# joesharratt1229/DT4Image_Restoration

Measured on AMD Instinct MI355X. Metric: pnp_admm_iterations_per_sec, higher is better.
Workload: dtype f32

## Files before the change

### dt4image_restoration_amd/_lib.py

```python
from __future__ import annotations

import ctypes as C
import os

_HERE = os.path.dirname(os.path.abspath(__file__))
LIB_PATH = os.environ.get("PNP_LIB_PATH") or os.path.join(_HERE, "csrc", "libpnpadmm.so")

PNP_FLAG_PROFILE = 1
PNP_FLAG_NO_DENOISER = 2
PNP_FLAG_KEEP_STAGES = 4
PNP_FLAG_BF16_CONVS = 8
PNP_FLAG_PROFILE_LAYERS = 16
PNP_SSIM_CLAMP_X = 1
PNP_RES_COLS = 6
PNP_RES_DELTA = 1
PNP_RES_DC = 2
RESIDUAL_COLUMNS = ("primal", "dx", "dz", "du", "delta", "dc")
PNP_MC_MAX_COILS = 32
PNP_MC_MAX_CG = 64
PNP_CC_MAX_COILS = 64
PNP_PW_MAX_COILS = 64
PNP_ESPIRIT_MAX_COILS = 16
PNP_ESPIRIT_MAX_KSIZE = 8
PNP_ESPIRIT_MAX_N = 512
PNP_GRAPPA_MAX_COILS = 32
PNP_GRAPPA_MAX_ACCEL = 8
PNP_GRAPPA_MAX_SRC = 512
PNP_TV_MAX_ITERS = 64
PNP_PRIOR_UNET = 0
PNP_PRIOR_TV = 1
PRIORS = {"unet": PNP_PRIOR_UNET, "tv": PNP_PRIOR_TV}
PNP_PRIOR_HAAR = 2
PRIOR_NAMES = {PNP_PRIOR_UNET: "unet", PNP_PRIOR_TV: "tv", PNP_PRIOR_HAAR: "haar"}
PNP_HAAR_TI = 0
PNP_HAAR_ORTHO = 1
PNP_HAAR_MAX_LEVELS = 4
HAAR_MODES = {"ti": PNP_HAAR_TI, "ortho": PNP_HAAR_ORTHO}
PNP_SENS_BOX = 0
PNP_SENS_HANN = 1
SENS_WINDOWS = {"box": PNP_SENS_BOX, "hann": PNP_SENS_HANN}
PROFILE_CLASSES = 6
PROFILE_CLASS_NAMES = ("conv3x3_mfma", "conv_first", "conv_last", "fft_rows", "fft_cols_prox", "other")
N_LAYERS = 28


class pnp_config(C.Structure):
    _fields_ = [("n", C.c_int32), ("h", C.c_int32), ("w", C.c_int32), ("device", C.c_int32), ("flags", C.c_int32)]


_vp, _fp, _u8p = C.c_void_p, C.c_void_p, C.c_void_p

SIGNATURES = {
    "pnp_create": (C.c_int, [C.POINTER(pnp_config), C.POINTER(C.c_void_p)]),
    "pnp_destroy": (C.c_int, [C.c_void_p]),
    "pnp_last_error": (C.c_char_p, []),
    "pnp_version": (C.c_char_p, []),
    "pnp_load_unet_weights": (C.c_int, [C.c_void_p, C.c_void_p, C.c_size_t]),
    "pnp_reset": (C.c_int, [C.c_void_p, _fp, _fp, _u8p, C.c_int, _fp, _fp, _fp, _vp]),
    "pnp_set_kspace": (C.c_int, [C.c_void_p, _fp, _u8p, C.c_int, _vp]),
    "pnp_step": (C.c_int, [C.c_void_p, _fp, _fp, _fp, _fp, _fp, _fp, _fp, _u8p, _vp]),
    "pnp_denoise": (C.c_int, [C.c_void_p, _fp, _fp, _fp, _vp]),
    "pnp_tv_denoise": (C.c_int, [C.c_void_p, _fp, _fp, C.c_int, _fp, _vp]),
    "pnp_set_prior": (C.c_int, [C.c_void_p, C.c_int, C.c_double, C.c_int]),
    "pnp_get_prior": (C.c_int, [C.c_void_p, C.POINTER(C.c_int), C.POINTER(C.c_double), C.POINTER(C.c_int)]),
    "pnp_haar_denoise": (C.c_int, [C.c_void_p, _fp, _fp, C.c_int, C.c_int, _fp, _vp]),
    "pnp_set_prior_haar": (C.c_int, [C.c_void_p, C.c_double, C.c_int, C.c_int]),
    "pnp_get_prior_haar": (C.c_int, [C.c_void_p, C.POINTER(C.c_double), C.POINTER(C.c_int), C.POINTER(C.c_int)]),
    "pnp_fft2c": (C.c_int, [C.c_void_p, _fp, _fp, C.c_int, C.c_int, C.c_int, C.c_int, _vp]),
    "pnp_prox_dual": (C.c_int, [C.c_void_p, _fp, _fp, _fp, _fp, _fp, _vp]),
    "pnp_psnr": (C.c_int, [C.c_void_p, _fp, _fp, _fp, _vp]),
    "pnp_ssim": (C.c_int, [C.c_void_p, _fp, _fp, C.c_float, C.c_float, C.c_float, C.c_int, C.c_int, _fp, _fp, _vp]),
    "pnp_residuals": (C.c_int, [C.c_void_p, _fp, _fp, _fp, _vp, C.c_int, _fp, _vp]),
    "pnp_acquire": (C.c_int, [C.c_void_p, _fp, _u8p, C.c_int, C.c_double, C.c_uint64, C.c_int, _fp, _fp, _fp, _vp]),
    "pnp_set_kspace_mc": (C.c_int, [C.c_void_p, _fp, _fp, C.c_int, C.c_int, _u8p, C.c_int, C.c_int, _vp]),
    "pnp_reset_mc": (C.c_int, [C.c_void_p, _fp, _fp, _fp, C.c_int, C.c_int, _u8p, C.c_int, C.c_int, _fp, _fp, _fp, _vp]),
    "pnp_mc_coils": (C.c_int, [C.c_void_p]),
    "pnp_mc_cg_residual": (C.c_int, [C.c_void_p, _fp, _vp]),
    "pnp_mc_normal": (C.c_int, [C.c_void_p, _fp, _fp, _fp, _vp]),
    "pnp_acquire_mc": (C.c_int, [C.c_void_p, _fp, _fp, C.c_int, C.c_int, _u8p, C.c_int, C.c_double, C.c_uint64, C.c_int, _fp, _fp, _fp, _vp]),
    "pnp_nufft_plan": (C.c_int, [C.c_void_p, C.c_void_p, C.c_int64, C.c_int, C.c_int, C.c_int, C.c_int]),
    "pnp_nufft_samples": (C.c_int64, [C.c_void_p]),
    "pnp_nufft_grid": (C.c_int, [C.c_void_p, C.POINTER(C.c_int), C.POINTER(C.c_int)]),
    "pnp_nufft_forward": (C.c_int, [C.c_void_p, _fp, C.c_int, _fp, _vp]),
    "pnp_nufft_adjoint": (C.c_int, [C.c_void_p, _fp, _fp, C.c_int, _fp, _vp]),
    "pnp_set_kspace_nc": (C.c_int, [C.c_void_p, _fp, _fp, C.c_int, _vp]),
    "pnp_reset_nc": (C.c_int, [C.c_void_p, _fp, _fp, _fp, C.c_int, _fp, _fp, _fp, _vp]),
    "pnp_nc_cg_residual": (C.c_int, [C.c_void_p, _fp, _vp]),
    "pnp_nc_normal": (C.c_int, [C.c_void_p, _fp, _fp, _fp, _vp]),
    "pnp_acquire_nc": (C.c_int, [C.c_void_p, _fp, _fp, C.c_double, C.c_uint64, C.c_int, _fp, _fp, _fp, _vp]),
    "pnp_estimate_sens": (C.c_int, [C.c_void_p, _fp, C.c_int, C.c_int, C.c_int, C.c_int, C.c_double, C.c_int, _fp, _fp, _vp]),
    "pnp_coil_compress_matrix": (C.c_int, [C.c_void_p, _fp, C.c_int, C.c_int, C.c_int, C.c_int, _fp, _fp, _fp, _vp]),
    "pnp_coil_compress_apply": (C.c_int, [C.c_void_p, _fp, C.c_int, _fp, C.c_int, C.c_int, _fp, _vp]),
    "pnp_noise_cov": (C.c_int, [C.c_void_p, _fp, C.c_int, C.c_int, C.c_int, C.c_int, _fp, _vp]),
    "pnp_whiten_matrix": (C.c_int, [C.c_void_p, _fp, C.c_int, C.c_int, C.c_int, _fp, _fp, _fp, _vp]),
    "pnp_whiten_apply": (C.c_int, [C.c_void_p, _fp, C.c_int, _fp, C.c_int, _fp, _vp]),
    "pnp_espirit_sens": (C.c_int, [C.c_void_p, _fp, C.c_int, C.c_int, C.c_int, C.c_int, C.c_double, C.c_double, C.c_int, C.c_int, C.c_double,
                                  C.c_int, _fp, _fp, _fp, _vp, _vp]),
    "pnp_grappa_weights": (C.c_int, [C.c_void_p, _fp, C.c_int, C.c_int, C.c_int, C.c_int, C.c_int, C.c_int, C.c_double, C.c_int, _fp, _vp, _fp,
                                    _vp]),
    "pnp_grappa_apply": (C.c_int, [C.c_void_p, _fp, C.c_int, _u8p, C.c_int, C.c_int, C.c_int, C.c_int, C.c_int, _fp, C.c_int, _fp, _vp]),
    "pnp_snapshot_bytes": (C.c_size_t, [C.c_void_p]),
    "pnp_snapshot": (C.c_int, [C.c_void_p, _fp, _fp, _fp, _fp, _vp, _vp]),
    "pnp_restore": (C.c_int, [C.c_void_p, _vp, _fp, _fp, _fp, _fp, _vp]),
    "pnp_unet_read_stage": (C.c_int, [C.c_void_p, C.c_int, _fp, C.POINTER(C.c_int), C.POINTER(C.c_int),
                                      C.POINTER(C.c_int), _vp]),
    "pnp_profile_reset": (C.c_int, [C.c_void_p]),
    "pnp_profile_collect": (C.c_int, [C.c_void_p, C.POINTER(C.c_double), C.POINTER(C.c_int64)]),
    "pnp_profile_layers": (C.c_int, [C.c_void_p, C.POINTER(C.c_double), C.POINTER(C.c_int64)]),
    "pnp_conv_algorithms": (C.c_int, [C.c_void_p, C.POINTER(C.c_int32)]),
    "pnp_conv_schedules": (C.c_int, [C.c_void_p, C.POINTER(C.c_int32)]),
    "pnp_bf16_weight_terms": (C.c_int, [C.c_void_p]),
    "pnp_workspace_bytes": (C.c_size_t, [C.c_void_p]),
}

SIGNATURES_NCSENSE = {
    "pnp_nufft_forward_mc": (C.c_int, [C.c_void_p, _fp, _fp, C.c_int, C.c_int, C.c_int, _fp, _vp]),
    "pnp_nufft_adjoint_mc": (C.c_int, [C.c_void_p, _fp, _fp, _fp, C.c_int, C.c_int, C.c_int, _fp, _vp]),
    "pnp_set_kspace_ncsense": (C.c_int, [C.c_void_p, _fp, _fp, C.c_int, C.c_int, _fp, C.c_int, _vp]),
    "pnp_reset_ncsense": (C.c_int, [C.c_void_p, _fp, _fp, _fp, C.c_int, C.c_int, _fp, C.c_int, _fp, _fp, _fp, _vp]),
    "pnp_ncsense_coils": (C.c_int, [C.c_void_p]),
    "pnp_ncsense_cg_residual": (C.c_int, [C.c_void_p, _fp, _vp]),
    "pnp_ncsense_normal": (C.c_int, [C.c_void_p, _fp, _fp, _fp, _vp]),
    "pnp_acquire_ncsense": (C.c_int, [C.c_void_p, _fp, _fp, C.c_int, C.c_int, _fp, C.c_double, C.c_uint64, C.c_int, _fp, _fp, _fp, _vp]),
}

SIGNATURES_TOEPLITZ = {
    "pnp_toeplitz_plan": (C.c_int, [C.c_void_p, _fp, C.c_int, _vp]),
    "pnp_toeplitz_planned": (C.c_int, [C.c_void_p]),
    "pnp_toeplitz_live": (C.c_int, [C.c_void_p]),
    "pnp_toeplitz_spectrum": (C.c_int, [C.c_void_p, _fp, _vp]),
    "pnp_toeplitz_apply": (C.c_int, [C.c_void_p, _fp, C.c_int, _fp, _vp]),
    "pnp_toeplitz_apply_mc": (C.c_int, [C.c_void_p, _fp, _fp, C.c_int, C.c_int, C.c_int, _fp, _vp]),
    "pnp_set_kspace_nc_tz": (C.c_int, [C.c_void_p, _fp, C.c_int, _vp]),
    "pnp_reset_nc_tz": (C.c_int, [C.c_void_p, _fp, _fp, C.c_int, _fp, _fp, _fp, _vp]),
    "pnp_set_kspace_ncsense_tz": (C.c_int, [C.c_void_p, _fp, _fp, C.c_int, C.c_int, C.c_int, _vp]),
    "pnp_reset_ncsense_tz": (C.c_int, [C.c_void_p, _fp, _fp, _fp, C.c_int, C.c_int, C.c_int, _fp, _fp, _fp, _vp]),
}
PNP_TOEPLITZ_MAX_SIDE = 512

SIGNATURES_DCF = {
    "pnp_nufft_psi": (C.c_int, [C.c_void_p, _fp, _fp, _vp]),
    "pnp_nufft_dcf": (C.c_int, [C.c_void_p, _fp, C.c_int, C.c_int, _fp, _fp, _vp]),
}
PNP_DCF_MAX_ITERS = 256

SIGNATURES_OFFRES = {
    "pnp_offres_plan": (C.c_int, [C.c_void_p, C.c_void_p, C.c_int, C.c_int]),
    "pnp_offres_segments": (C.c_int, [C.c_void_p]),
    "pnp_offres_maps": (C.c_int, [C.c_void_p, _fp, C.c_int, _fp, _vp]),
    "pnp_offres_forward": (C.c_int, [C.c_void_p, _fp, _fp, C.c_int, C.c_int, _fp, _vp]),
    "pnp_offres_adjoint": (C.c_int, [C.c_void_p, _fp, _fp, _fp, C.c_int, C.c_int, _fp, _vp]),
    "pnp_set_kspace_offres": (C.c_int, [C.c_void_p, _fp, _fp, C.c_int, _fp, C.c_int, _vp]),
    "pnp_reset_offres": (C.c_int, [C.c_void_p, _fp, _fp, _fp, C.c_int, _fp, C.c_int, _fp, _fp, _fp, _vp]),
    "pnp_offres_live": (C.c_int, [C.c_void_p]),
    "pnp_offres_cg_residual": (C.c_int, [C.c_void_p, _fp, _vp]),
    "pnp_offres_normal": (C.c_int, [C.c_void_p, _fp, _fp, _fp, _vp]),
    "pnp_acquire_offres": (C.c_int, [C.c_void_p, _fp, _fp, C.c_int, _fp, C.c_double, C.c_uint64, C.c_int, _fp, _fp, _fp, _vp]),
}


def toeplitz_size_error(fn: str, h: int, w: int):
    if h <= PNP_TOEPLITZ_MAX_SIDE and w <= PNP_TOEPLITZ_MAX_SIDE:
        return None
    return f"{fn}: the Toeplitz operator transforms a 2h x 2w grid, so it takes h, w up to {PNP_TOEPLITZ_MAX_SIDE} (got {int(h)}x{int(w)})"

_lib = None


class PnPError(RuntimeError):
    pass


def load() -> C.CDLL:
    global _lib
    if _lib is not None:
        return _lib
    if not os.path.exists(LIB_PATH):
        raise PnPError(f"{LIB_PATH} not found: build it with `python -c 'import __graft_entry__ as g; g.build()'` "
                       f"or `make -C {os.path.dirname(LIB_PATH)}`; there is no CPU fallback")
    lib = C.CDLL(LIB_PATH)
    for name, (res, args) in {**SIGNATURES, **SIGNATURES_NCSENSE, **SIGNATURES_TOEPLITZ, **SIGNATURES_DCF, **SIGNATURES_OFFRES}.items():
        fn = getattr(lib, name)
        fn.restype = res
        fn.argtypes = args
    _lib = lib
    return lib


def check(rc: int, what: str) -> None:
    if rc != 0:
        msg = load().pnp_last_error()
        raise PnPError(f"{what} failed ({rc}): {msg.decode() if msg else '?'}")
```

### dt4image_restoration_amd/csrc/conv_kernels.hip

```cpp
#include "pnp_internal.h"
#include "conv_staging.h"
#include <cstring>
#include <cstdlib>

namespace pnp {



const LayerSpec kLayers[N_LAYERS] = {
    {2, 32, 3, 0, SRC_SIGMA, 0},    {32, 32, 3, 0, SRC_PLAIN, 0},   {32, 32, 3, 0, SRC_PLAIN, 0},
    {32, 64, 3, 1, SRC_POOL, 0},    {64, 64, 3, 1, SRC_PLAIN, 0},   {64, 64, 3, 1, SRC_PLAIN, 0},
    {64, 128, 3, 2, SRC_POOL, 0},   {128, 128, 3, 2, SRC_PLAIN, 0}, {128, 128, 3, 2, SRC_PLAIN, 0},
    {128, 256, 3, 3, SRC_POOL, 0},  {256, 256, 3, 3, SRC_PLAIN, 0}, {256, 256, 3, 3, SRC_PLAIN, 0},
    {256, 512, 3, 4, SRC_POOL, 0},  {512, 512, 3, 4, SRC_PLAIN, 0}, {512, 512, 3, 4, SRC_PLAIN, 0},
    {768, 256, 3, 3, SRC_UPCAT, 256}, {256, 256, 3, 3, SRC_PLAIN, 0}, {256, 256, 3, 3, SRC_PLAIN, 0},
    {384, 128, 3, 2, SRC_UPCAT, 128}, {128, 128, 3, 2, SRC_PLAIN, 0}, {128, 128, 3, 2, SRC_PLAIN, 0},
    {192, 64, 3, 1, SRC_UPCAT, 64},  {64, 64, 3, 1, SRC_PLAIN, 0},   {64, 64, 3, 1, SRC_PLAIN, 0},
    {96, 32, 3, 0, SRC_UPCAT, 32},   {32, 32, 3, 0, SRC_PLAIN, 0},   {32, 32, 3, 0, SRC_PLAIN, 0},
    {32, 1, 1, 0, SRC_PLAIN, 0},
};

ConvPlan conv3x3_plan(int N, int H, int W, int Cin, int Cout, bool bf16, int src_mode, bool allow_ws) {
    ConvPlan p{};
    p.tw = W >= 32 ? 32 : (W >= 16 ? 16 : 8);
// ... 493 lines not shown
                    const float* o = &patch[((2 * qy) * TW + 2 * qx) * OSTR + 4 * c4];
                    const float4 m = f4max(f4max(*reinterpret_cast<const float4*>(o), *reinterpret_cast<const float4*>(o + OSTR)),
                                           f4max(*reinterpret_cast<const float4*>(o + TW * OSTR), *reinterpret_cast<const float4*>(o + TW * OSTR + OSTR)));
                    *reinterpret_cast<float4*>(a.pooled + (((size_t)n * Hp + gy) * Wp + gx) * a.Cout + cbase + 4 * c4) = m;
                }
            }
        }
    } else {
        const size_t plane = (size_t)a.N * a.H * a.W * a.Cout;
        float* const obuf = SPLITK ? a.partial + (size_t)blockIdx.z * plane : a.dst;
        const __amdgpu_buffer_rsrc_t orsrc = __builtin_amdgcn_make_buffer_rsrc((void*)obuf, 0, (int)(plane * sizeof(float)), 0x00020000);
#pragma unroll
        for (int nt = 0; nt < NT; ++nt) {
            const int co = (cbt * (WN * NT) + wn * NT + nt) * 32 + li;
            const unsigned obase = ((unsigned)(((size_t)n * a.H + ty0) * a.W + tx0 + 4 * hh) * (unsigned)a.Cout + (unsigned)co) * 4u;
#pragma unroll
            for (int mt = 0; mt < MT; ++mt)
#pragma unroll
                for (int r = 0; r < 16; ++r) {
                    const int qc = (wm * MT + mt) * 32 + (r & 3) + 8 * (r >> 2);
                    const int gy = ty0 + qc / TW, gx = tx0 + qc % TW + 4 * hh;
                    const int soff = __builtin_amdgcn_readfirstlane(((qc / TW) * a.W + qc % TW) * a.Cout * 4);
                    const float v = SPLITK ? acc[mt][nt][r] : fmaxf(acc[mt][nt][r], kLeaky * acc[mt][nt][r]);
                    if (gy < a.H && gx < a.W) __builtin_amdgcn_raw_buffer_store_b32(__builtin_bit_cast(unsigned, v), orsrc, obase, soff, 0);
                }
        }
    }
}

__global__ __launch_bounds__(256) void splitk_reduce_kernel(const float* __restrict__ partial, const float* __restrict__ bias,
                                                            float* __restrict__ dst, const float* __restrict__ tact,
                                                            size_t plane4, int splitk, int cout4, size_t slice4) {
    for (size_t i = (size_t)blockIdx.x * 256 + threadIdx.x; i < plane4; i += (size_t)gridDim.x * 256) {
        if (tact != nullptr && tact[i / slice4] > 0.5f) continue;
        float4 s = reinterpret_cast<const float4*>(bias)[i % cout4];
        for (int z0 = 0; z0 < splitk; z0 += 8) {
            float4 p[8];
#pragma unroll
            for (int k = 0; k < 8; ++k) p[k] = reinterpret_cast<const float4*>(partial)[(size_t)(z0 + k < splitk ? z0 + k : splitk - 1) * plane4 + i];
#pragma unroll
            for (int k = 0; k < 8; ++k)
                if (z0 + k < splitk) { s.x += p[k].x; s.y += p[k].y; s.z += p[k].z; s.w += p[k].w; }
        }
        s.x = fmaxf(s.x, kLeaky * s.x); s.y = fmaxf(s.y, kLeaky * s.y);
        s.z = fmaxf(s.z, kLeaky * s.z); s.w = fmaxf(s.w, kLeaky * s.w);
        reinterpret_cast<float4*>(dst)[i] = s;
    }
}

template <int TW, int MT, int NT, int WM, int WN, int CK, int SRC, bool SPLITK, int BF16>
static hipError_t launch_inst(const ConvArgs& a, const ConvPlan& p, hipStream_t s) {
    constexpr int WPS = (MT * NT <= 2 && SRC != SRC_UPCAT) ? 3 : (MT * NT <= 8 ? 2 : 1);
    constexpr int WPS16 = (MT * NT <= 2 && BF16 == 2) ? 3 : WPS;
    dim3 grid((unsigned)(p.tiles_x * p.tiles_y * a.N), (unsigned)(a.Cout / p.bn), (unsigned)p.splitk);
    constexpr bool CAN16 = BF16 != 0 && !SPLITK && MT == 2 && NT == 1 && WM == 4 && CK == 32 && SRC != SRC_POOL;
    if constexpr (CAN16) {
        if (a.act16 & 1) {
            hipLaunchKernelGGL((conv3x3_mfma_kernel<TW, MT, NT, WM, WN, CK, SRC, WPS16, SPLITK, BF16, true>), grid, dim3(256), 0, s, a);
            return hipGetLastError();
        }
    }
    if (a.act16 != 0) return hipErrorInvalidValue;
    hipLaunchKernelGGL((conv3x3_mfma_kernel<TW, MT, NT, WM, WN, CK, SRC, WPS, SPLITK, BF16, false>), grid, dim3(256), 0, s, a);
    return hipGetLastError();
}

template <int TW, int MT, int NT, int WM, int WN, int CK, bool SPLITK, int BF16>
static hipError_t launch_cfg(const ConvArgs& a, const ConvPlan& p, int src_mode, hipStream_t s) {
    switch (src_mode) {
        case SRC_PLAIN: return launch_inst<TW, MT, NT, WM, WN, CK, SRC_PLAIN, SPLITK, BF16>(a, p, s);
        case SRC_POOL:  return launch_inst<TW, MT, NT, WM, WN, CK, SRC_POOL, SPLITK, BF16>(a, p, s);
        case SRC_UPCAT: return launch_inst<TW, MT, NT, WM, WN, CK, SRC_UPCAT, SPLITK, BF16>(a, p, s);
        default: return hipErrorInvalidValue;
    }
}

template <int TW, int BF16>
static hipError_t launch_tw(const ConvArgs& a, const ConvPlan& p, int src_mode, hipStream_t s) {
    if constexpr (BF16 == 0) {
        if (p.mt == 1 && p.wn == 4) return launch_cfg<TW, 1, 1, 1, 4, 16, true, 0>(a, p, src_mode, s);
        if (p.mt == 1 && p.wn == 2) return launch_cfg<TW, 1, 1, 2, 2, 16, true, 0>(a, p, src_mode, s);
    }
    if (p.mt == 2 && p.wn == 4) return launch_cfg<TW, 2, 1, 1, 4, 32, true, BF16>(a, p, src_mode, s);
    if (p.mt == 2 && p.wn == 2) return launch_cfg<TW, 2, 1, 2, 2, 32, true, BF16>(a, p, src_mode, s);
    if constexpr (BF16 == 0) {
        if (p.nt == 1 && p.mt == 1) return launch_cfg<TW, 1, 1, 4, 1, 32, false, 0>(a, p, src_mode, s);
    }
    if (p.nt == 1) return launch_cfg<TW, 2, 1, 4, 1, 32, false, BF16>(a, p, src_mode, s);
    if (p.nt == 2 && p.wn == 1) return launch_cfg<TW, 4, 2, 4, 1, 16, false, BF16>(a, p, src_mode, s);
    if (p.nt == 2) return launch_cfg<TW, 4, 2, 2, 2, 32, false, BF16>(a, p, src_mode, s);
    if constexpr (BF16 != 0) return hipErrorInvalidValue;
    else return launch_cfg<TW, 4, 4, 2, 2, 32, false, 0>(a, p, src_mode, s);
}

hipError_t launch_conv3x3(const ConvArgs& a0, const ConvPlan& p, int src_mode, hipStream_t s) {
    if (a0.Cin % 32 != 0 || a0.Cout % 32 != 0 || (a0.Cout > 64 && a0.Cout % 128 != 0)) return hipErrorInvalidValue;
    if (!conv3x3_tensor_fits(a0.N, a0.H, a0.W, a0.Cin, a0.Cout)) return hipErrorInvalidValue;
    if (p.ws) return launch_conv3x3_bf16ws(a0, p, src_mode, s);
    ConvArgs a = a0;
    a.tilesX = p.tiles_x;
    a.tilesY = p.tiles_y;
    const bool split = p.mt <= 2 && p.wn >= 2;
    if (split && a.partial == nullptr) return hipErrorInvalidValue;
    hipError_t e;
    if (a.bf16 == 2) {
        if (p.tw == 32) e = launch_tw<32, 2>(a, p, src_mode, s);
        else if (p.tw == 16) e = launch_tw<16, 2>(a, p, src_mode, s);
        else e = launch_tw<8, 2>(a, p, src_mode, s);
    } else if (a.bf16 == 1) {
        if (p.tw == 32) e = launch_tw<32, 1>(a, p, src_mode, s);
        else if (p.tw == 16) e = launch_tw<16, 1>(a, p, src_mode, s);
        else e = launch_tw<8, 1>(a, p, src_mode, s);
    } else {
        if (p.tw == 32) e = launch_tw<32, 0>(a, p, src_mode, s);
        else if (p.tw == 16) e = launch_tw<16, 0>(a, p, src_mode, s);
        else e = launch_tw<8, 0>(a, p, src_mode, s);
    }
    if (e != hipSuccess || !split) return e;
    const size_t plane4 = (size_t)a.N * a.H * a.W * a.Cout / 4;
    unsigned blocks = (unsigned)((plane4 + 255) / 256);
    if (blocks > 2048u) blocks = 2048u;
    hipLaunchKernelGGL(splitk_reduce_kernel, dim3(blocks), dim3(256), 0, s, a.partial, a.bias, a.dst, a.tact, plane4,
                       p.splitk, a.Cout / 4, (size_t)a.H * a.W * a.Cout / 4);
    return hipGetLastError();
}

bool conv3x3_tensor_fits(int N, int H, int W, int Cin, int Cout) {
    (void)Cin;
    return (size_t)N * H * W * (size_t)Cout * 4 < ((size_t)1 << 31);
}

bool conv3x3_pooled_output_ok(const ConvPlan& p) {
    return p.splitk == 1 && p.mt <= 2 && p.nt == 1 && p.wm == 4;
}

size_t conv3x3_partial_floats(const ConvPlan& p, int N, int H, int W, int Cout) {
    return (p.mt <= 2 && p.wn >= 2) ? (size_t)p.splitk * N * H * W * Cout : 0;
}

Tuning tuning_from_env() {
    Tuning t;
    if (const char* v = getenv("PNP_WINO_MIN_CIN")) t.wino_min_cin = atoi(v);
    if (const char* v = getenv("PNP_WINO_MIN_BLOCKS")) t.wino_min_blocks = atol(v);
    t.wino_big = getenv("PNP_WINO_BIG_GROUPS") != nullptr;
    t.wino_small = getenv("PNP_WINO_SMALL_GROUPS") != nullptr;
    t.no_wino = getenv("PNP_NO_WINOGRAD") != nullptr;
    if (const char* v = getenv("PNP_WINO_F4_MIN_CIN")) t.f4_min_cin = atoi(v);
    t.no_f4 = getenv("PNP_NO_WINO_F4") != nullptr;
    t.no_f4_phased = getenv("PNP_NO_WINO_F4_PHASED") != nullptr;
    t.no_f4_fused_last = getenv("PNP_NO_F4_FUSED_LAST") != nullptr;
    t.no_f4_fused_first = getenv("PNP_NO_F4_FUSED_FIRST") != nullptr;
    if (const char* v = getenv("PNP_WINO_F4_MT16")) t.f4_mt16 = atoi(v);
    if (const char* v = getenv("PNP_WINO_F4_CS")) t.f4_cs = atoi(v);
    if (const char* v = getenv("PNP_WINO_F4_ORDER")) t.f4_order = atoi(v) != 0;
    t.bf16_f32_acts = getenv("PNP_BF16_F32_ACTS") != nullptr;
    t.bf16_no_ws = getenv("PNP_BF16_NO_WS") != nullptr;
    t.bf16_w1 = getenv("PNP_BF16_W1") != nullptr;
    t.bf16_no_holdhi = getenv("PNP_BF16_NO_HOLDHI") != nullptr;
    if (const char* v = getenv("PNP_SLICE128_MIN_N")) t.slice128_min_n = atoi(v);
    if (const char* v = getenv("PNP_TV_NAIVE")) t.tv_naive = atoi(v) != 0;
    if (const char* v = getenv("PNP_HAAR_NAIVE")) t.haar_naive = atoi(v) != 0;
    if (const char* v = getenv("PNP_NCSENSE_COIL_BLOCK")) t.ncsense_block = atoi(v);
    if (const char* v = getenv("PNP_NCSENSE_NAIVE")) t.ncsense_naive = atoi(v) != 0 ? 1 : 0;
    if (const char* v = getenv("PNP_TOEPLITZ_NAIVE")) t.toeplitz_naive = atoi(v) != 0;
    if (const char* v = getenv("PNP_OFFRES_SEG_BLOCK")) t.offres_block = atoi(v);
    if (const char* v = getenv("PNP_OFFRES_GRID_FILTER")) t.offres_grid_filter = atoi(v) != 0;
    if (const char* v = getenv("PNP_OFFRES_NAIVE")) t.offres_naive = atoi(v) != 0 ? 1 : 0;
    return t;
}

hipError_t raise_lds_cap(const void* fn, int bytes, DeviceOnce& once) {
    int dev = 0;
    hipError_t e = hipGetDevice(&dev);
    if (e != hipSuccess) return e;
    const uint64_t bit = 1ull << (dev & 63);
    if (once.mask.load(std::memory_order_relaxed) & bit) return hipSuccess;
    e = hipFuncSetAttribute(fn, hipFuncAttributeMaxDynamicSharedMemorySize, bytes);
    if (e != hipSuccess) return e;
    once.mask.fetch_or(bit, std::memory_order_relaxed);
    return hipSuccess;
}

__global__ __launch_bounds__(256) void conv_first_kernel(const float* __restrict__ ximg, const float2* __restrict__ z,
                                                         const float2* __restrict__ u, const float* __restrict__ sigma,
                                                         const float* __restrict__ tact, const float* __restrict__ w,
                                                         const float* __restrict__ bias, float* __restrict__ dst,
                                                         int N, int H, int W, int tilesX, int tilesY, int TYG, int dst16) {
    constexpr int TH = 8, TW = 32, PW = TW + 2, PH = TH + 2;
    __shared__ float dt[2][PH][PW + 1];
    __shared__ float mt[2][PH][PW + 1];
    const int groupsY = (tilesY + TYG - 1) / TYG;
    int bt = blockIdx.x;
    const int tx0 = (bt % tilesX) * TW;
    bt /= tilesX;
    const int tyg = bt % groupsY;
    const int n = bt / groupsY;
    if (tact != nullptr && tact[n] > 0.5f) return;
    auto stage = [&](int buf, int ty0) {
        for (int i = threadIdx.x; i < PH * PW; i += 256) {
            const int py = i / PW, px = i % PW;
            const int gy = ty0 + py - 1, gx = tx0 + px - 1;
            float d = 0.f, m = 0.f;
            if (gy >= 0 && gy < H && gx >= 0 && gx < W) {
                const size_t q = ((size_t)n * H + gy) * W + gx;
                d = ximg != nullptr ? ximg[q] : (z[q].x - u[q].x);
                m = 1.f;
            }
            dt[buf][py][px] = d;
            mt[buf][py][px] = m;
        }
    };
    const int t_first = tyg * TYG, t_last = min(t_first + TYG, tilesY);
    stage(0, t_first * TH);
    const int cg = threadIdx.x & 7, col = threadIdx.x >> 3;
    float wd[4][9], ws[4][9], br[4], brs[4];
    const float sg = sigma[n];
#pragma unroll
    for (int j = 0; j < 4; ++j) {
        br[j] = bias[cg * 4 + j];
        brs[j] = br[j];
#pragma unroll
        for (int k = 0; k < 9; ++k) {
            wd[j][k] = w[(cg * 4 + j) * 18 + k];
            ws[j][k] = w[(cg * 4 + j) * 18 + 9 + k] * sg;
            brs[j] += ws[j][k];
        }
    }
    const int gx = tx0 + col;
    for (int t = t_first; t < t_last; ++t) {
        const int buf = (t - t_first) & 1, ty0 = t * TH;
        const bool interior = tx0 > 0 && tx0 + TW < W && ty0 > 0 && ty0 + TH < H;
        __syncthreads();
        if (t + 1 < t_last) stage(buf ^ 1, ty0 + TH);
        float d[3][3], m[3][3];
#pragma unroll
        for (int r = 0; r < 2; ++r)
#pragma unroll
            for (int c = 0; c < 3; ++c) { d[r + 1][c] = dt[buf][r][col + c]; m[r + 1][c] = mt[buf][r][col + c]; }
#pragma unroll
        for (int row = 0; row < TH; ++row) {
#pragma unroll
            for (int c = 0; c < 3; ++c) {
                d[0][c] = d[1][c]; d[1][c] = d[2][c]; d[2][c] = dt[buf][row + 2][col + c];
                m[0][c] = m[1][c]; m[1][c] = m[2][c]; m[2][c] = mt[buf][row + 2][col + c];
            }
            float acc[4];
            if (interior) {
#pragma unroll
                for (int j = 0; j < 4; ++j) acc[j] = brs[j];
#pragma unroll
                for (int ky = 0; ky < 3; ++ky)
#pragma unroll
                    for (int kx = 0; kx < 3; ++kx)
#pragma unroll
                        for (int j = 0; j < 4; ++j) acc[j] = fmaf(wd[j][ky * 3 + kx], d[ky][kx], acc[j]);
            } else {
#pragma unroll
                for (int j = 0; j < 4; ++j) acc[j] = br[j];
#pragma unroll
                for (int ky = 0; ky < 3; ++ky)
#pragma unroll
                    for (int kx = 0; kx < 3; ++kx)
#pragma unroll
                        for (int j = 0; j < 4; ++j) {
                            acc[j] = fmaf(wd[j][ky * 3 + kx], d[ky][kx], acc[j]);
                            acc[j] = fmaf(ws[j][ky * 3 + kx], m[ky][kx], acc[j]);
                        }
            }
            const int gy = ty0 + row;
            if (gy < H && gx < W) {
                float4 o;
                o.x = fmaxf(acc[0], kLeaky * acc[0]);
                o.y = fmaxf(acc[1], kLeaky * acc[1]);
                o.z = fmaxf(acc[2], kLeaky * acc[2]);
                o.w = fmaxf(acc[3], kLeaky * acc[3]);
                if (dst16) {
                    uint2 o16;
                    o16.x = __builtin_bit_cast(unsigned, __builtin_convertvector((f32x2){o.x, o.y}, bf16x2));
                    o16.y = __builtin_bit_cast(unsigned, __builtin_convertvector((f32x2){o.z, o.w}, bf16x2));
                    *reinterpret_cast<uint2*>(reinterpret_cast<uint16_t*>(dst) + (((size_t)n * H + gy) * W + gx) * 32 + cg * 4) = o16;
                } else {
                    *reinterpret_cast<float4*>(dst + (((size_t)n * H + gy) * W + gx) * 32 + cg * 4) = o;
                }
            }
        }
    }
}

hipError_t launch_conv_first(const float* ximg, const float2* z, const float2* u, const float* sigma,
                             const float* tact, const float* w, const float* bias, float* dst, int N, int H, int W,
                             hipStream_t s, bool dst_bf16) {
    const int tilesX = (W + 31) / 32, tilesY = (H + 7) / 8;
    int tyg = 8;
    while (tyg > 1 && (long)tilesX * ((tilesY + tyg - 1) / tyg) * N < 512) tyg >>= 1;
    const int groupsY = (tilesY + tyg - 1) / tyg;
    hipLaunchKernelGGL(conv_first_kernel, dim3((unsigned)(tilesX * groupsY * N)), dim3(256), 0, s, ximg, z, u, sigma, tact, w,
                       bias, dst, N, H, W, tilesX, tilesY, tyg, dst_bf16 ? 1 : 0);
    return hipGetLastError();
}

__global__ __launch_bounds__(256) void conv_last_kernel(const float* __restrict__ act, const float* __restrict__ ximg,
                                                        const float2* __restrict__ z, const float2* __restrict__ u,
                                                        const float* __restrict__ tact, const float* __restrict__ w,
                                                        const float* __restrict__ bias, float* __restrict__ out,
                                                        int N, int H, int W) {
    const int cg = threadIdx.x & 7;
// ... 51 lines not shown
```

### dt4image_restoration_amd/csrc/pnp_capi.hip

```cpp
#include "../../include/pnpadmm.h"
#include "../../include/pnpadmm_ncsense.h"
#include "../../include/pnpadmm_toeplitz.h"
#include "../../include/pnpadmm_dcf.h"
#include "../../include/pnpadmm_offres.h"
#include "pnp_internal.h"
#include "denoiser_plan.h"
#include "nufft_plan.h"
#include "offres_plan.h"
#include "block_reduce.h"

#include <cmath>
#include <cstdarg>
#include <cstdio>
#include <cstring>
#include <cstdlib>
#include <initializer_list>
#include <new>
#include <string>
#include <vector>

using namespace pnp;

namespace {

thread_local std::string g_err;

int fail(int code, const char* fmt, ...) {
    char buf[512];
    va_list ap;
    va_start(ap, fmt);
    vsnprintf(buf, sizeof buf, fmt, ap);
    va_end(ap);
    g_err = buf;
    return code;
}

#define HIP_TRY(expr)                                                                              \
    do {                                                                                           \
        hipError_t e_ = (expr);                                                                    \
        if (e_ != hipSuccess) return fail(PNP_ERR_HIP, "%s failed: %s", #expr, hipGetErrorString(e_)); \
    } while (0)

#define PNP_API_BEGIN try {
#define PNP_API_END(name)                                                                          \
    } catch (const std::bad_alloc&) { return fail(PNP_ERR_NOMEM, name ": out of host memory");     \
    } catch (const std::exception& ex_) { return fail(PNP_ERR_INTERNAL, name ": %s", ex_.what());  \
    } catch (...) { return fail(PNP_ERR_INTERNAL, name ": unknown C++ exception"); }

struct DeviceGuard {
    int prev = -1;
    bool switched = false;
    hipError_t err = hipSuccess;
    explicit DeviceGuard(int dev) {
        err = hipGetDevice(&prev);
        if (err == hipSuccess && prev != dev) { err = hipSetDevice(dev); switched = err == hipSuccess; }
    }
    ~DeviceGuard() { if (switched) (void)hipSetDevice(prev); }
};
#define PNP_ON_DEVICE(e)                                                                                  \
    DeviceGuard dev_guard_((e)->cfg.device);                                                              \
    if (dev_guard_.err != hipSuccess) return fail(PNP_ERR_HIP, "hipSetDevice(%d): %s", (e)->cfg.device, hipGetErrorString(dev_guard_.err))

constexpr size_t kNParams = 11773857;

enum ProfClass : int { PROF_CONV3X3 = 0, PROF_CONV_FIRST = 1, PROF_CONV_LAST = 2, PROF_FFT_ROWS = 3, PROF_FFT_COLS = 4, PROF_OTHER = 5 };
static_assert(PROF_OTHER + 1 == PNP_PROFILE_CLASSES, "one enumerator per profile class");

struct EventPair {
    hipEvent_t a, b;
    int cls, layer;
    int count;
};

enum StageKind { STAGE_NONE, STAGE_CART, STAGE_MC, STAGE_NC, STAGE_NS, STAGE_OR };
struct LiveStage {
    StageKind kind = STAGE_NONE;
    bool toeplitz = false;
    int coils = 0;
    int sens_n = 1;
    int cg = 0;
    bool has_w = false;
};

}

struct pnp_engine {
    pnp_config cfg;
    bool weights_loaded = false;
    LiveStage stage;
    float* d_wpack[N_LAYERS] = {};
    float* d_bias[N_LAYERS] = {};
    float* plane[N_LEVELS][N_SLOTS] = {};
    float* d_partial = nullptr;
    Tuning tune;
    DenoiserPlan dplan;
    ConvArgs largs[N_LAYERS] = {};
    FftPlan plan = {};
    float2* d_work = nullptr;
    float2* d_y0s = nullptr;
    uint8_t* d_masks = nullptr;
    double* d_ssim_part = nullptr;
    double* d_res_part = nullptr;
    int mask_n = 1;
    size_t ws_bytes = 0;
    float2* mc_y = nullptr;
    float2* mc_work = nullptr;
    float2* mc_sens = nullptr;
    size_t mc_y_cap = 0, mc_work_cap = 0, mc_sens_cap = 0;
    float2* mc_vec = nullptr;
    double* mc_part = nullptr;
    double* mc_sc = nullptr;
    float* cm_max = nullptr;
    float* cm_rss = nullptr;
    double2* cc_part = nullptr;
    double2* cc_gram = nullptr;
    size_t cc_part_cap = 0, cc_gram_cap = 0;
    double2* pw_part = nullptr;
    size_t pw_part_cap = 0;
    void* es_ws = nullptr;
    size_t es_cap = 0;
    double2* gr_ws = nullptr;
    size_t gr_cap = 0;
    NufftDev nc;
    size_t nc_i0_cap = 0, nc_wts_cap = 0, nc_cy_cap = 0, nc_cx_cap = 0, nc_off_cap = 0, nc_idx_cap = 0, nc_twh_cap = 0, nc_tww_cap = 0;
    float2* nc_grid = nullptr;
    float2* nc_samp = nullptr;
    float2* nc_y = nullptr;
    float* nc_w = nullptr;
    double* nc_mpart = nullptr;
    size_t nc_grid_cap = 0, nc_samp_cap = 0, nc_y_cap = 0, nc_w_cap = 0, nc_mpart_cap = 0;
    int ns_block = kNcsenseBlock;
    int ns_naive = kNcsenseNaiveSteps;
    float2* ns_img = nullptr;
    size_t ns_img_cap = 0;
    float2* ns_grid = nullptr;
    float2* ns_samp = nullptr;
    float2* ns_y = nullptr;
    float2* ns_sens = nullptr;
    float* ns_w = nullptr;
    double* ns_mpart = nullptr;
    size_t ns_grid_cap = 0, ns_samp_cap = 0, ns_y_cap = 0, ns_sens_cap = 0, ns_w_cap = 0, ns_mpart_cap = 0;
    std::vector<int32_t> nc_bin_off_h, nc_bin_idx_h;
    OffresDev orp;
    size_t or_tau_cap = 0, or_seg_cap = 0, or_b0_cap = 0, or_b1_cap = 0, or_loff_cap = 0, or_lidx_cap = 0;
    int or_block = kOffresBlock;
    int or_naive = kOffresNaiveSteps;
    float2* or_maps = nullptr;
    float2* or_y = nullptr;
    float* or_w = nullptr;
    double* or_mpart = nullptr;
    float2* or_amaps = nullptr;
    size_t or_maps_cap = 0, or_y_cap = 0, or_w_cap = 0, or_mpart_cap = 0, or_amaps_cap = 0;
    std::vector<double> nc_traj;
    double* tz_traj = nullptr;
    float* tz_k = nullptr;
    float* tz_w = nullptr;
    float2* tz_tw_h = nullptr;
// ... 2383 lines not shown
                       float* wts, int32_t* info, double* gram, void* stream) {
    PNP_API_BEGIN
    const char* fn = "pnp_grappa_weights";
    if (flags != 0) return fail(PNP_ERR_INVALID, "%s: flags must be 0 (got 0x%x)", fn, (unsigned)flags);
    if (!(lam >= 0.0) || !(lam <= 1.0)) return fail(PNP_ERR_INVALID, "%s: lam must be finite and in [0, 1] (got %g)", fn, lam);
    if (int rc = grappa_check_kernel(fn, coils, accel, by, bx)) return rc;
    const int span = (bx - 1) * accel + 1;
    if (acs_h < by || (acs_h & 1)) return fail(PNP_ERR_INVALID, "%s: acs_h must be even and >= by=%d (got %d)", fn, by, acs_h);
    if (acs_w < span || (acs_w & 1)) return fail(PNP_ERR_INVALID, "%s: acs_w must be even and >= (bx - 1) accel + 1 = %d (got %d)", fn, span, acs_w);
    if (!y0) return fail(PNP_ERR_INVALID, "%s: null y0", fn);
    if (!wts) return fail(PNP_ERR_INVALID, "%s: null wts", fn);
    if (!info) return fail(PNP_ERR_INVALID, "%s: null info", fn);
    {
        const void* q[4] = {y0, wts, info, gram};
        for (int i = 0; i < 4; ++i)
            for (int j = i + 1; j < 4; ++j)
                if (q[j] && q[i] == q[j]) return fail(PNP_ERR_INVALID, "%s: y0, wts, info and gram must not alias", fn);
    }
    if (!e) return fail(PNP_ERR_INVALID, "%s: null handle", fn);
    const int N = e->cfg.n, H = e->cfg.h, W = e->cfg.w;
    if (W % accel) return fail(PNP_ERR_INVALID, "%s: accel must divide w=%d (got %d)", fn, W, accel);
    if (acs_h > H) return fail(PNP_ERR_INVALID, "%s: acs_h must be <= h=%d (got %d)", fn, H, acs_h);
    if (acs_w > W) return fail(PNP_ERR_INVALID, "%s: acs_w must be <= w=%d (got %d)", fn, W, acs_w);
    if ((long long)N * coils > 65535) return fail(PNP_ERR_INVALID, "%s: n * coils must be <= 65535 (got %d * %d)", fn, N, coils);
    const int ns = coils * by * bx, nt = coils * (accel - 1);
    {
        const void* q[4] = {y0, wts, info, gram};
        const size_t len[4] = {(size_t)N * coils * H * W * sizeof(float2), (size_t)N * nt * ns * sizeof(float2), (size_t)N * sizeof(int32_t),
                               (size_t)N * ns * (ns + nt) * sizeof(double2)};
        for (int i = 0; i < 4; ++i)
            for (int j = i + 1; j < 4; ++j)
                if (q[j] && ranges_overlap(q[i], len[i], q[j], len[j])) return fail(PNP_ERR_INVALID, "%s: y0, wts, info and gram must not alias", fn);
    }
    PNP_ON_DEVICE(e);
    hipStream_t s = (hipStream_t)stream;
    if (int rc = gr_ensure(e, (size_t)N * ns * (ns + nt))) return rc;
    Prof p(e, s, PROF_OTHER, -1);
    HIP_TRY(launch_grappa_gram((const float2*)y0, coils, acs_h, acs_w, accel, by, bx, e->gr_ws, (double2*)gram, N, H, W, s));
    HIP_TRY(launch_grappa_solve(e->gr_ws, ns, nt, lam, (float2*)wts, (int*)info, N, s));
    p.end(2);
    return PNP_OK;
    PNP_API_END("pnp_grappa_weights")
}

int pnp_grappa_apply(pnp_handle e, const float* y0, int coils, const uint8_t* mask, int mask_n, int accel, int offset, int by, int bx,
                     const float* wts, int wts_n, float* out, void* stream) {
    PNP_API_BEGIN
    const char* fn = "pnp_grappa_apply";
    if (int rc = grappa_check_kernel(fn, coils, accel, by, bx)) return rc;
    if (offset < 0 || offset >= accel) return fail(PNP_ERR_INVALID, "%s: offset must be 0..accel-1 = %d (got %d)", fn, accel - 1, offset);
    if (mask_n < 1) return fail(PNP_ERR_INVALID, "%s: mask_n must be 1 or the handle's n (got %d)", fn, mask_n);
    if (wts_n < 1) return fail(PNP_ERR_INVALID, "%s: wts_n must be 1 or the handle's n (got %d)", fn, wts_n);
    if (!y0) return fail(PNP_ERR_INVALID, "%s: null y0", fn);
    if (!mask) return fail(PNP_ERR_INVALID, "%s: null mask", fn);
    if (!wts) return fail(PNP_ERR_INVALID, "%s: null wts", fn);
    if (!out) return fail(PNP_ERR_INVALID, "%s: null out", fn);
    if (out == wts || (const void*)out == (const void*)mask || ranges_overlap(out, (size_t)2048 * coils, y0, (size_t)2048 * coils))
        return fail(PNP_ERR_INVALID, "%s: out must not overlap y0, wts or mask", fn);
    if (!e) return fail(PNP_ERR_INVALID, "%s: null handle", fn);
    const int N = e->cfg.n, H = e->cfg.h, W = e->cfg.w;
    if (W % accel) return fail(PNP_ERR_INVALID, "%s: accel must divide w=%d (got %d)", fn, W, accel);
    if (mask_n != 1 && mask_n != N) return fail(PNP_ERR_INVALID, "%s: mask_n must be 1 or the handle's n=%d (got %d)", fn, N, mask_n);
    if (wts_n != 1 && wts_n != N) return fail(PNP_ERR_INVALID, "%s: wts_n must be 1 or the handle's n=%d (got %d)", fn, N, wts_n);
    if ((long long)N * coils > 65535) return fail(PNP_ERR_INVALID, "%s: n * coils must be <= 65535 (got %d * %d)", fn, N, coils);
    const size_t ns = (size_t)coils * by * bx, nt = (size_t)coils * (accel - 1);
    const size_t bytes = (size_t)N * coils * H * W * sizeof(float2), wbytes = (size_t)wts_n * nt * ns * sizeof(float2), mbytes = (size_t)mask_n * H * W;
    if (ranges_overlap(out, bytes, y0, bytes) || ranges_overlap(out, bytes, wts, wbytes) || ranges_overlap(out, bytes, mask, mbytes))
        return fail(PNP_ERR_INVALID, "%s: out must not overlap y0, wts or mask", fn);
    PNP_ON_DEVICE(e);
    hipStream_t s = (hipStream_t)stream;
    Prof p(e, s, PROF_OTHER, -1);
    HIP_TRY(launch_grappa_apply((const float2*)y0, mask, mask_n, (const float2*)wts, wts_n, (float2*)out, coils, accel, offset, by, bx, N, H, W, s));
    return PNP_OK;
    PNP_API_END("pnp_grappa_apply")
}

size_t pnp_snapshot_bytes(pnp_handle e) {
    return e ? SnapLayout(e).bytes() : 0;
}

int pnp_snapshot(pnp_handle e, const float* x, const float* z, const float* u, const float* t_state, void* dst,
                 void* stream) {
    PNP_API_BEGIN
    if (!e || !x || !z || !u || !dst) return fail(PNP_ERR_INVALID, "pnp_snapshot: null argument");
    PNP_ON_DEVICE(e);
    const SnapLayout snap(e);
    char* d = static_cast<char*>(dst);
    hipStream_t s = (hipStream_t)stream;
    HIP_TRY(hipMemcpyAsync(d, x, snap.x_bytes(), hipMemcpyDeviceToDevice, s));
    HIP_TRY(hipMemcpyAsync(d + snap.z_off(), z, snap.zu_bytes(), hipMemcpyDeviceToDevice, s));
    HIP_TRY(hipMemcpyAsync(d + snap.u_off(), u, snap.zu_bytes(), hipMemcpyDeviceToDevice, s));
    if (t_state) HIP_TRY(hipMemcpyAsync(d + snap.t_off(), t_state, snap.t_bytes(), hipMemcpyDeviceToDevice, s));
    else HIP_TRY(hipMemsetAsync(d + snap.t_off(), 0, snap.t_bytes(), s));
    return PNP_OK;
    PNP_API_END("pnp_snapshot")
}

int pnp_restore(pnp_handle e, const void* src, float* x, float* z, float* u, float* t_state, void* stream) {
    PNP_API_BEGIN
    if (!e || !x || !z || !u || !src) return fail(PNP_ERR_INVALID, "pnp_restore: null argument");
    PNP_ON_DEVICE(e);
    const SnapLayout snap(e);
    const char* d = static_cast<const char*>(src);
    hipStream_t s = (hipStream_t)stream;
    HIP_TRY(hipMemcpyAsync(x, d, snap.x_bytes(), hipMemcpyDeviceToDevice, s));
    HIP_TRY(hipMemcpyAsync(z, d + snap.z_off(), snap.zu_bytes(), hipMemcpyDeviceToDevice, s));
    HIP_TRY(hipMemcpyAsync(u, d + snap.u_off(), snap.zu_bytes(), hipMemcpyDeviceToDevice, s));
    if (t_state) HIP_TRY(hipMemcpyAsync(t_state, d + snap.t_off(), snap.t_bytes(), hipMemcpyDeviceToDevice, s));
    return PNP_OK;
    PNP_API_END("pnp_restore")
}

int pnp_unet_read_stage(pnp_handle e, int which, float* dst, int* c, int* hh, int* ww, void* stream) {
    PNP_API_BEGIN
    if (!e || which < 0 || which > 8) return fail(PNP_ERR_INVALID, "pnp_unet_read_stage: which must be 0..8");
    if (e->cfg.flags & PNP_FLAG_NO_DENOISER) return fail(PNP_ERR_STATE, "pnp_unet_read_stage: handle has no denoiser");
    const StagePlan& st = e->dplan.stage[which];
    if (st.fused_away) return fail(PNP_ERR_STATE, "pnp_unet_read_stage: stage 8 is fused away; create the handle with PNP_FLAG_KEEP_STAGES");
    if (st.bf16) return fail(PNP_ERR_STATE, "pnp_unet_read_stage: this stage is held as bf16 on this handle; create it with PNP_FLAG_KEEP_STAGES");
    PNP_ON_DEVICE(e);
    const float* src = e->plane[st.plane.level][st.plane.slot];
    if (c) *c = st.c;
    if (hh) *hh = st.h;
    if (ww) *ww = st.w;
    if (dst) HIP_TRY(launch_nhwc_to_nchw(src, dst, e->cfg.n, st.c, st.h, st.w, (hipStream_t)stream));
    return PNP_OK;
    PNP_API_END("pnp_unet_read_stage")
}

int pnp_conv_algorithms(pnp_handle e, int32_t* algo28) {
    PNP_API_BEGIN
    if (!e || !algo28) return fail(PNP_ERR_INVALID, "pnp_conv_algorithms: null argument");
    if (e->cfg.flags & PNP_FLAG_NO_DENOISER) return fail(PNP_ERR_STATE, "pnp_conv_algorithms: handle has no denoiser");
    for (int i = 0; i < N_LAYERS; ++i) algo28[i] = e->dplan.family[i];
    return PNP_OK;
    PNP_API_END("pnp_conv_algorithms")
}

int pnp_conv_schedules(pnp_handle e, int32_t* sched28) {
    PNP_API_BEGIN
    if (!e || !sched28) return fail(PNP_ERR_INVALID, "pnp_conv_schedules: null argument");
    if (e->cfg.flags & PNP_FLAG_NO_DENOISER) return fail(PNP_ERR_STATE, "pnp_conv_schedules: handle has no denoiser");
    for (int i = 0; i < N_LAYERS; ++i) {
        const int at = e->dplan.launch_of[i];
        sched28[i] = 0;
        if (at < 0 || e->dplan.family[i] != FAM_WINO4) continue;
        const WinoPlan& w = e->dplan.launch[at].wino;
        sched28[i] = w.cs ? 4 : (w.mt == 16 ? 3 : (w.phased ? 2 : 1));
    }
    return PNP_OK;
    PNP_API_END("pnp_conv_schedules")
}

int pnp_profile_reset(pnp_handle e) {
    PNP_API_BEGIN
    if (!e) return fail(PNP_ERR_INVALID, "null handle");
    e->ev_used = 0;
    memset(e->cls_ms, 0, sizeof e->cls_ms); memset(e->cls_n, 0, sizeof e->cls_n);
    memset(e->layer_ms, 0, sizeof e->layer_ms); memset(e->layer_n, 0, sizeof e->layer_n);
    return PNP_OK;
    PNP_API_END("pnp_profile_reset")
}

int pnp_profile_collect(pnp_handle e, double* total_ms, int64_t* launches) {
    PNP_API_BEGIN
    if (!e) return fail(PNP_ERR_INVALID, "null handle");
    PNP_ON_DEVICE(e);
    for (size_t i = 0; i < e->ev_used; ++i) {
        float ms = 0.f;
        HIP_TRY(hipEventElapsedTime(&ms, e->events[i].a, e->events[i].b));
        const EventPair& p = e->events[i];
        e->cls_ms[p.cls] += ms; e->cls_n[p.cls] += p.count;
        if (p.layer >= 0) { e->layer_ms[p.layer] += ms; e->layer_n[p.layer] += 1; }
    }
    e->ev_used = 0;
    for (int i = 0; i < PNP_PROFILE_CLASSES; ++i) {
        if (total_ms) total_ms[i] = e->cls_ms[i];
        if (launches) launches[i] = e->cls_n[i];
    }
    return PNP_OK;
    PNP_API_END("pnp_profile_collect")
}

int pnp_profile_layers(pnp_handle e, double* layer_ms, int64_t* layer_launches) {
    PNP_API_BEGIN
    if (!e) return fail(PNP_ERR_INVALID, "null handle");
    for (int i = 0; i < N_LAYERS; ++i) {
        if (layer_ms) layer_ms[i] = e->layer_ms[i];
        if (layer_launches) layer_launches[i] = e->layer_n[i];
    }
    return PNP_OK;
    PNP_API_END("pnp_profile_layers")
}

}
```

### dt4image_restoration_amd/csrc/pnp_internal.h

```cpp
#pragma once
#include <hip/hip_runtime.h>
#include <stdint.h>
#include <stddef.h>
#include <atomic>
#include <vector>

namespace pnp {

struct Tuning {
    int wino_min_cin = 32;
    long wino_min_blocks = 192;
    bool wino_big = false;
    bool wino_small = false;
    bool no_wino = false;
    int f4_min_cin = 32;
    bool no_f4 = false;
    bool no_f4_fused_first = false;
    bool no_f4_fused_last = false;
    bool no_f4_phased = false;
    int f4_mt16 = 0;
    bool bf16_no_ws = false;
    bool bf16_f32_acts = false;
    bool bf16_no_holdhi = false;
    bool bf16_w1 = false;
    int f4_cs = 1;
    int f4_order = 1;
    int slice128_min_n = 192;
    bool tv_naive = false;
    bool haar_naive = false;
    int ncsense_block = 0;
    int ncsense_naive = -1;
    bool toeplitz_naive = false;
    int offres_block = 0;
    bool offres_grid_filter = false;
    int offres_naive = -1;
};
Tuning tuning_from_env();

struct DeviceOnce { std::atomic<uint64_t> mask{0}; };
hipError_t raise_lds_cap(const void* fn, int bytes, DeviceOnce& once);

enum SrcMode : int { SRC_PLAIN = 0, SRC_SIGMA = 1, SRC_POOL = 2, SRC_UPCAT = 3, SRC_FIRST = 4 };

struct LayerSpec {
    int cin, cout, ksize, level, src, cskip;
};
static constexpr int N_LAYERS = 28;
extern const LayerSpec kLayers[N_LAYERS];

struct ConvArgs {
    const float* src0;
    const float* src1;
    const float* wpack;
    const float* bias;
    float* dst;
    float* pooled;
    const float* last_w; const float* last_b; const float* last_ximg; const float2* last_z; const float2* last_u; float* last_out;
    const float* first_w; const float* first_b; const float* first_sigma;
    float* partial;
    const float* tact;
    int N, H, W;
    int Cin, Cskip, Cout;
    int tilesX, tilesY;
    float rh, rw;
    int bf16;
    int act16;
    int order;
#ifdef PNP_STAMPS
    int stamp_slot;
#endif
#ifdef PNP_DIAG
    int diag;
#endif
};

struct ConvPlan {
    int tw, th;
    int bm, bn;
    int mt, nt, wm, wn;
    int ck;
    int splitk;
    int ws;
    int holdhi = 1;
    int tiles_x, tiles_y;
};
ConvPlan conv3x3_plan(int N, int H, int W, int Cin, int Cout, bool bf16 = false, int src_mode = SRC_PLAIN, bool allow_ws = true);
hipError_t launch_conv3x3_bf16ws(const ConvArgs& a, const ConvPlan& p, int src_mode, hipStream_t s);
size_t conv3x3_partial_floats(const ConvPlan& p, int N, int H, int W, int Cout);
bool conv3x3_pooled_output_ok(const ConvPlan& p);
bool conv3x3_tensor_fits(int N, int H, int W, int Cin, int Cout);
hipError_t launch_conv3x3(const ConvArgs& a, const ConvPlan& p, int src_mode, hipStream_t s);

size_t conv3x3_pack_floats(int cin, int cout);
void pack_conv3x3_weights(const float* oihw, int cin, int cout, int ck, float* dst);
size_t conv3x3_pack_floats_bf16(int cin, int cout, int terms);
void pack_conv3x3_weights_bf16(const float* oihw, int cin, int cout, int ck, int terms, float* dst);

struct WinoPlan {
    bool use;
    int algo;
    int tw, th, bn, wm, wn, ck, tiles_x, tiles_y;
    int stack;
    int mt;
    int phased;
    int cs;
    int order;
};
WinoPlan winograd_plan(int N, int H, int W, int Cin, int Cout, int src_mode, const Tuning& t, int Cskip = 0);
bool upsample_lines_regular(int H);
size_t winograd4_pack_floats(int cin, int cout);
void pack_winograd4_weights(const float* oihw, int cin, int cout, int ck, float* dst);
hipError_t launch_conv3x3_winograd4(const ConvArgs& a, const WinoPlan& p, int src_mode, hipStream_t s);
size_t winograd_pack_floats(int cin, int cout);
void pack_winograd_weights(const float* oihw, int cin, int cout, int ck, float* dst);
hipError_t launch_conv3x3_winograd(const ConvArgs& a, const WinoPlan& p, int src_mode, hipStream_t s);

hipError_t launch_conv_first(const float* ximg, const float2* z, const float2* u, const float* sigma,
                             const float* tact, const float* w, const float* bias, float* dst,
                             int N, int H, int W, hipStream_t s, bool dst_bf16 = false);
hipError_t launch_conv_last(const float* act, const float* ximg, const float2* z, const float2* u,
                            const float* tact, const float* w, const float* bias, float* out,
                            int N, int H, int W, hipStream_t s);
hipError_t launch_nhwc_to_nchw(const float* src, float* dst, int N, int C, int H, int W, hipStream_t s);

struct FftPlan {
    int h, w;
    float2* tw_h;
    float2* tw_w;
};

bool kspace_len_ok(int L);
hipError_t launch_fft_rows(const float2* in, float2* out, const float2* tw, int batch, int H, int W, int inverse, int shift, hipStream_t s);
hipError_t launch_fft_cols(float2* data, const float2* tw, int batch, int H, int W, int inverse, int shift, hipStream_t s);
hipError_t launch_fft_rows_real(const float* x, float2* work, const float2* tw, int N, int H, int W, hipStream_t s);
hipError_t launch_fft_rows_fwd_admm(const float* x, const float2* u, float2* work, const float2* tw, const float* tact, int N, int H, int W,
                                    hipStream_t s);
hipError_t launch_fft_cols_prox(float2* work, const float2* tw, const float2* y0s, const uint8_t* masks, int mask_n, const float* mu,
                                const float* tact, int N, int H, int W, hipStream_t s);
hipError_t launch_fft_rows_inv_admm(const float2* work, const float* x, float2* z, float2* u, const float2* tw, const float* tact, int N,
                                    int H, int W, hipStream_t s);
namespace mixed {
hipError_t launch_fft_rows(const float2* in, float2* out, const float2* tw, int batch, int H, int W, int inverse, int shift, hipStream_t s);
hipError_t launch_fft_cols(float2* data, const float2* tw, int batch, int H, int W, int inverse, int shift, hipStream_t s);
hipError_t launch_fft_rows_real(const float* x, float2* work, const float2* tw, int N, int H, int W, hipStream_t s);
hipError_t launch_fft_rows_fwd_admm(const float* x, const float2* u, float2* work, const float2* tw, const float* tact, int N, int H, int W,
                                    hipStream_t s);
hipError_t launch_fft_cols_prox(float2* work, const float2* tw, const float2* y0s, const uint8_t* masks, int mask_n, const float* mu,
                                const float* tact, int N, int H, int W, hipStream_t s);
hipError_t launch_fft_rows_inv_admm(const float2* work, const float* x, float2* z, float2* u, const float2* tw, const float* tact, int N,
                                    int H, int W, hipStream_t s);
}

hipError_t launch_admm_slice128(const float* x, float2* z, float2* u, const float2* tw, const float2* y0s,
                                const uint8_t* masks, int mask_n, const float* mu, const float* tact, int N, hipStream_t s);

hipError_t launch_reset(const float2* x0, const float2* y0, const uint8_t* mask, int mask_n, float* x, float2* z,
                        float2* u, float2* y0s, uint8_t* masks, int N, int H, int W, hipStream_t s);
hipError_t launch_finish(const float* tact, float* tstate, uint8_t* done, int N, hipStream_t s);
hipError_t launch_psnr(const float* x, const float* gt, float* out, int N, int HW, hipStream_t s);

static constexpr int kSsimMaxRadius = 16;
struct SsimArgs {
    const float* x;
    const float* gt;
    float* map;
    double* partial;
    float* out;
    int H, W;
    int radius;
    int clamp_x;
    float c1, c2;
    float w[2 * kSsimMaxRadius + 1];
};
int ssim_tiles(int H, int W);
hipError_t launch_ssim(const SsimArgs& a, int N, hipStream_t s);

hipError_t launch_residual_tiles(const float* x, const float2* z, const float2* u, const float* xp, const float2* zp, const float2* up,
                                 double* partial, int N, int H, int W, hipStream_t s);
hipError_t launch_misfit_tiles(const float2* fx, const float2* y0s, const uint8_t* masks, int mask_n, double* dcpartial, int N, int H, int W,
                               hipStream_t s);
hipError_t launch_residual_reduce(const double* partial, const double* dcpartial, int has_delta, int has_dc, float* out, int N, int H, int W,
                                  hipStream_t s);

hipError_t launch_acquire_epilogue(float2* work, const uint8_t* mask, int mask_n, float2* y0, double sigma, uint64_t seed, int N, int H, int W,
                                   hipStream_t s, int coils = 1);
hipError_t launch_acquire_clamp(const float2* aty0, float2* x0, int N, int H, int W, hipStream_t s);

hipError_t launch_sense_expand(const float2* src, const float* src_real, const float2* sens, int sens_n, int C, const float* tact, float2* work,
                               int N, int H, int W, hipStream_t s);
hipError_t launch_sense_mask(float2* work, const uint8_t* masks, int mask_n, int C, int N, int H, int W, hipStream_t s);
hipError_t launch_sense_combine(const float2* work, const float2* sens, int sens_n, int C, const float2* pv, const float* mu, const float* tact,
                                float2* q, double* partial, int N, int H, int W, hipStream_t s);
hipError_t launch_sense_cg_init(const float2* aty, const float* x, const float2* u, const float2* q, const float* mu, const float* tact, float2* r,
                                float2* pv, double* partial, int N, int H, int W, hipStream_t s);
hipError_t launch_sense_scalar(const double* partial, int mode, const float* tact, double* sc, int N, int H, int W, hipStream_t s);
hipError_t launch_sense_cg_update(float2* z, float2* r, const float2* pv, const float2* q, const double* sc, const float* tact, double* partial,
                                  int N, int H, int W, hipStream_t s);
hipError_t launch_sense_cg_dir(const float2* r, float2* pv, const double* sc, const float* tact, int N, int H, int W, hipStream_t s);
hipError_t launch_sense_dual(const float* x, const float2* z, float2* u, const float* tact, int N, int H, int W, hipStream_t s);
hipError_t launch_sense_cgres(const double* sc, float* out, int N, hipStream_t s);
hipError_t launch_sense_misfit(const float2* fx, const float2* ys, const uint8_t* masks, int mask_n, int C, double* dcpartial, int N, int H, int W,
                               hipStream_t s);
hipError_t launch_sense_install(const float2* y, const uint8_t* mask, int mask_n, int C, float2* ys, float2* work, uint8_t* masks, int N, int H,
                                int W, hipStream_t s);
hipError_t launch_sense_iterate(const float2* x0, float* x, float2* z, float2* u, int N, int H, int W, hipStream_t s);

hipError_t launch_coilmap_window(const float2* y, float2* sens, int acs_h, int acs_w, int hann, int N, int C, int H, int W, hipStream_t s);
hipError_t launch_coilmap_rss(const float2* l, int C, float* rss, float* partial, int N, int H, int W, hipStream_t s);
hipError_t launch_coilmap_max(const float* partial, float* smax, int N, int H, int W, hipStream_t s);
hipError_t launch_coilmap_normalise(float2* l, int C, const float* rss, const float* smax, float thresh, int N, int H, int W, hipStream_t s);

static constexpr int kGramMinBins = 1024, kGramMaxChunks = 64;
inline int gram_chunk_len(long long count) {
    const long long per = ((count + kGramMaxChunks - 1) / kGramMaxChunks + 31) / 32 * 32;
    return per < kGramMinBins ? kGramMinBins : (int)per;
}
inline int gram_chunks(long long count) { return (int)((count + gram_chunk_len(count) - 1) / gram_chunk_len(count)); }
hipError_t launch_coilcomp_gram(const float2* y, int C, int acs_h, int acs_w, double2* partial, double2* gram, int N, int H, int W, hipStream_t s);
hipError_t launch_coilcomp_eig(const double2* gram, int C, float2* cmat, float* eig, int N, hipStream_t s);
hipError_t launch_coilcomp_apply(const float2* in, const float2* cmat, int cmat_n, int C, int V, float2* out, int N, int H, int W, hipStream_t s);

hipError_t launch_prewhiten_cov(const float2* noise, int noise_n, int C, int S, double2* partial, double2* psi, hipStream_t s);
hipError_t launch_prewhiten_chol(const double2* psi, int psi_n, int C, float2* wmat, float2* lmat, int* info, hipStream_t s);
hipError_t launch_prewhiten_apply(const float2* in, const float2* wmat, int wmat_n, int C, float2* out, int N, int H, int W, hipStream_t s);

hipError_t launch_grappa_gram(const float2* y, int C, int acs_h, int acs_w, int R, int by, int bx, double2* ws, double2* gram, int N, int H, int W,
                              hipStream_t s);
hipError_t launch_grappa_solve(double2* ws, int ns, int nt, double lam, float2* wts, int* info, int N, hipStream_t s);
hipError_t launch_grappa_apply(const float2* y0, const uint8_t* mask, int mask_n, const float2* wts, int wts_n, float2* out, int C, int R,
                               int offset, int by, int bx, int N, int H, int W, hipStream_t s);

inline int espirit_padded(int C, int k) { return (C * k * k + 1) & ~1; }
hipError_t launch_espirit_gram(const float2* y, int C, int acs_h, int acs_w, int k, double2* ws, int N, int H, int W, hipStream_t s);
hipError_t launch_espirit_eig(double2* ws, int C, int k, int N, hipStream_t s);
hipError_t launch_espirit_kern(const double2* ws, int C, int k, double sv_thresh, float2* kern, int* nkept, int N, hipStream_t s);
hipError_t launch_espirit_pixels(float2* sens, const float2* kern, const float* rss, const float* smax, int C, int k, int iters, float crop,
                                 float thresh, float* eval, int N, int H, int W, hipStream_t s);

static constexpr int kTvT = 10, kTvRegion = 128, kTvTile = kTvRegion - 2 * kTvT - 1;
struct TvArgs {
    const float* v;
    const float2* z;
    const float2* u;
    const float* lam;
    float scale;
    const float* tact;
    const float2* p_in;
    float2* p_out;
    float* out;
    int H, W;
    int iters;
    int tiles_x, tiles_y;
};
hipError_t launch_tv_fused(TvArgs a, int N, hipStream_t s);
hipError_t launch_tv_iter(TvArgs a, int N, hipStream_t s);
hipError_t launch_tv_close(TvArgs a, int N, hipStream_t s);

static constexpr int kHaarRegion = 128, kHaarMaxLevels = 4;
inline int haar_tile(int levels) { return kHaarRegion - 2 * ((1 << levels) - 1); }
struct HaarArgs {
// ... 103 lines not shown
```

### dt4image_restoration_amd/csrc/winograd4_kernels.hip

```cpp
#include "pnp_internal.h"
#include "conv_staging.h"
#include <type_traits>

namespace pnp {

#ifdef PNP_STAMPS
#define W4_SLOTS 32
#define W4_WGS 1024
#define W4_N 16
__device__ unsigned long long g_w4_stamps[W4_SLOTS * W4_WGS * W4_N];
static int g_w4_slot = 0;
#define W4T() __builtin_amdgcn_s_memtime()
#endif

namespace {
constexpr double kA = 0.75, kB = 1.5;
constexpr float fA = 0.75f, fB = 1.5f, fA2 = 0.5625f, fB2 = 2.25f, fA3 = 0.421875f, fB3 = 3.375f;
constexpr float fK0 = 1.265625f;
constexpr float fK1 = 2.8125f;

__device__ __forceinline__ float4 f4add(float4 a, float4 b) { return make_float4(a.x + b.x, a.y + b.y, a.z + b.z, a.w + b.w); }
typedef float v2f __attribute__((ext_vector_type(2)));
typedef float f32x4 __attribute__((ext_vector_type(4)));

template <int G>
__device__ __forceinline__ void bt3(const v2f* d, v2f* o) {
    if constexpr (G == 0) {
        o[0] = fK0 * d[0] + (d[4] - fK1 * d[2]);
        const v2f e = d[4] - fB2 * d[2];
        const v2f od = fA * (d[3] - fB2 * d[1]);
        o[1] = e + od;
        o[2] = e - od;
    } else {
        const v2f e = d[4] - fA2 * d[2];
        const v2f od = fB * (d[3] - fA2 * d[1]);
        o[0] = e + od;
        o[1] = e - od;
        o[2] = fK0 * d[1] + (d[5] - fK1 * d[3]);
    }
}

template <int QJ, int PW, int CKP, int PLANE>
__device__ __forceinline__ void wino4_input_transform(const float* w, float* v) {
    constexpr int X0 = QJ == 0 ? 0 : 1;
    v2f c[6][3];
#pragma unroll
    for (int y = 0; y < 6; ++y) {
        v2f d[6];
        __builtin_amdgcn_sched_barrier(0);
#pragma unroll
        for (int x = 0; x < 5; ++x) d[X0 + x] = *reinterpret_cast<const v2f*>(w + (y * PW + X0 + x) * CKP);
        bt3<QJ>(d, c[y]);
    }
#pragma unroll
    for (int j = 0; j < 3; ++j) {
        const v2f r0 = c[0][j], r1 = c[1][j], r2 = c[2][j], r3 = c[3][j], r4 = c[4][j], r5 = c[5][j];
        float* vj = v + (3 * QJ + j) * PLANE;
        *reinterpret_cast<v2f*>(vj + 0 * 6 * PLANE) = fK0 * r0 + (r4 - fK1 * r2);
        const v2f e1 = r4 - fB2 * r2, o1 = fA * (r3 - fB2 * r1);
        *reinterpret_cast<v2f*>(vj + 1 * 6 * PLANE) = e1 + o1;
        *reinterpret_cast<v2f*>(vj + 2 * 6 * PLANE) = e1 - o1;
        const v2f e2 = r4 - fA2 * r2, o2 = fB * (r3 - fA2 * r1);
        *reinterpret_cast<v2f*>(vj + 3 * 6 * PLANE) = e2 + o2;
        *reinterpret_cast<v2f*>(vj + 4 * 6 * PLANE) = e2 - o2;
        *reinterpret_cast<v2f*>(vj + 5 * 6 * PLANE) = fK0 * r1 + (r5 - fK1 * r3);
    }
}
}

constexpr int kW4Tail = 8 * 64 * 4;
size_t winograd4_pack_floats(int cin, int cout) { return (size_t)cout * cin * 36 + (size_t)(cout / 16) * kW4Tail; }

void pack_winograd4_weights(const float* oihw, int cin, int cout, int ck, float* dst) {
    const int CK = ck, S = CK / 4;
    const double pts[5] = {0.0, kA, -kA, kB, -kB};
    double G[6][3];
    for (int j = 0; j < 5; ++j) {
        double nrm = 1.0;
        for (int l = 0; l < 5; ++l) if (l != j) nrm *= pts[j] - pts[l];
        G[j][0] = 1.0 / nrm; G[j][1] = pts[j] / nrm; G[j][2] = pts[j] * pts[j] / nrm;
    }
    G[5][0] = 0.0; G[5][1] = 0.0; G[5][2] = 1.0;
    std::vector<float> U((size_t)cout * cin * 36);
    for (int co = 0; co < cout; ++co)
        for (int ci = 0; ci < cin; ++ci) {
            const float* g = oihw + ((size_t)co * cin + ci) * 9;
            double t[6][3];
            for (int i = 0; i < 6; ++i)
                for (int kx = 0; kx < 3; ++kx) t[i][kx] = G[i][0] * g[kx] + G[i][1] * g[3 + kx] + G[i][2] * g[6 + kx];
            for (int i = 0; i < 6; ++i)
                for (int j = 0; j < 6; ++j)
                    U[((size_t)co * cin + ci) * 36 + 6 * i + j] = (float)(t[i][0] * G[j][0] + t[i][1] * G[j][1] + t[i][2] * G[j][2]);
        }
    size_t o = 0;
    for (int cb = 0; cb < cout / 16; ++cb) {
        for (int ch = 0; ch < cin / CK; ++ch)
            for (int xi = 0; xi < 36; ++xi)
                for (int l = 0; l < 64; ++l)
                    for (int sidx = 0; sidx < S; ++sidx) {
                        const int co = 16 * cb + (l & 15);
                        const int ci = CK * ch + S * (l >> 4) + sidx;
                        dst[o++] = U[((size_t)co * cin + ci) * 36 + xi];
                    }
        for (int i = 0; i < kW4Tail; ++i) dst[o++] = 0.f;
    }
}

bool upsample_lines_regular(int H) {
    if (H < 2 || H % 2) return false;
    const int Hs = H / 2;
    const float rh = (float)(Hs - 1) / (float)(H - 1);
    for (int g = 0; g < H; ++g) {
        const float sc = rh * (float)g;
        const int i0 = (int)sc;
        const int i1 = i0 + (i0 < Hs - 1 ? 1 : 0);
        const float l = sc - (float)i0;
        const int s0 = g >= 1 ? (g - 1) / 2 : -1;
        if (l < 1.f && i0 != s0 && i0 != s0 + 1) return false;
        if (l > 0.f && i1 != s0 && i1 != s0 + 1) return false;
    }
    return true;
}

__device__ __forceinline__ void wino4_decode(int bid, int ny, int ntiles, int order, int& cby, int& bt) {
    if (order == 0) {
        const int grp = bid / (8 * ny), rem = bid % (8 * ny);
        cby = rem >> 3;
        bt = grp * 8 + (rem & 7);
    } else {
        const int xcd = bid & 7, slot = bid >> 3;
        const int tpx = (ntiles + 7) >> 3;
        const int lt = slot / ny;
        cby = slot - lt * ny;
        bt = lt < tpx ? xcd * tpx + lt : ntiles;
    }
}

template <int PH, int PW, int PPP, int NW>
struct Wino4Interp {
    static constexpr int IPAIRS = PW * PPP, IWPG = (IPAIRS + 63) / 64, ING = NW / IWPG;
    static constexpr int IRG = (((PH + (ING > 0 ? ING : 1) - 1) / (ING > 0 ? ING : 1)) + 1) & ~1;
    static constexpr int IK = IRG / 2 + 1;
};
template <int PH, int PW, int PPP, int LH, int LW, int LP, int NW, int ROWSTEP, class Slot, class Put>
__device__ __forceinline__ void wino4_interpolate(const float* lowres, const float* rowT, const float* colT, int w, int t, Slot slot, Put put) {
    typedef Wino4Interp<PH, PW, PPP, NW> G;
    constexpr int IPAIRS = G::IPAIRS, IWPG = G::IWPG, ING = G::ING, IRG = G::IRG, IK = G::IK;
    const int ig = w / IWPG;
    const int it = t - ig * (IWPG * 64);
    if (ig >= ING || it >= IPAIRS) return;
    const int x = it / PPP, part = it % PPP;
    const int yb = ig * IRG;
    const float4 ct = *reinterpret_cast<const float4*>(&colT[4 * x]);
    const float* const l0 = &lowres[__float_as_int(ct.x) + part * 4 + (yb / 2) * (LW * LP)];
    const float* const l1 = &lowres[__float_as_int(ct.y) + part * 4 + (yb / 2) * (LW * LP)];
    const v2f wx0 = v2f{ct.z, ct.z}, wx1 = v2f{ct.w, ct.w};
    v2f tl[IK], th_[IK];
#pragma unroll
    for (int k = 0; k < IK; ++k) {
        if ((yb / 2 + k) < LH) {
            const float4 pa = *reinterpret_cast<const float4*>(l0 + k * (LW * LP)), pb = *reinterpret_cast<const float4*>(l1 + k * (LW * LP));
            tl[k] = __builtin_elementwise_fma(wx0, v2f{pa.x, pa.y}, wx1 * v2f{pb.x, pb.y});
            th_[k] = __builtin_elementwise_fma(wx0, v2f{pa.z, pa.w}, wx1 * v2f{pb.z, pb.w});
        } else { tl[k] = v2f{0.f, 0.f}; th_[k] = v2f{0.f, 0.f}; }
    }
    const int pdst = slot(yb, x, part);
#pragma unroll
    for (int j = 0; j < IRG; ++j) {
        if (yb + j < PH) {
            const float4 rw = *reinterpret_cast<const float4*>(&rowT[4 * (yb + j)]);
            const v2f wa = v2f{rw.x, rw.x}, wb = v2f{rw.y, rw.y};
            const int k = j >> 1;
            const v2f olo = __builtin_elementwise_fma(wa, tl[k], wb * tl[k + 1]);
            const v2f ohi = __builtin_elementwise_fma(wa, th_[k], wb * th_[k + 1]);
            put(pdst + j * ROWSTEP, make_float4(olo.x, olo.y, ohi.x, ohi.y));
        }
    }
}
template <int PH, int PW, int LP>
__device__ __forceinline__ void wino4_upsample_tables(const ConvArgs& a, int tid, int ty0, int tx0, int ylo, int xlo, float* rowT, float* colT) {
    if (tid >= PH + PW) return;
    const int Hs = a.H >> 1, Ws = a.W >> 1;
    const bool isrow = tid < PH;
    const int pq = isrow ? tid : tid - PH;
    const int g = (isrow ? ty0 : tx0) + pq - 1;
    float4 e = make_float4(0.f, 0.f, 0.f, 0.f);
    if (g >= 0 && g < (isrow ? a.H : a.W)) {
        const float sc = (isrow ? a.rh : a.rw) * (float)g;
        const int i0 = (int)sc;
        const int i1 = i0 + (i0 < (isrow ? Hs : Ws) - 1 ? 1 : 0);
        const float l = fminf(fmaxf(sc - (float)i0, 0.f), 1.f);
        if (isrow) {
            const int s0 = ylo + (pq >> 1);
            const float w0 = 1.f - l, w1 = l;
            e.x = (i0 == s0 ? w0 : 0.f) + (i1 == s0 ? w1 : 0.f);
            e.y = (i0 == s0 + 1 ? w0 : 0.f) + (i1 == s0 + 1 ? w1 : 0.f);
        } else {
            e = make_float4(__int_as_float((i0 - xlo) * LP), __int_as_float((i1 - xlo) * LP), 1.f - l, l);
        }
    }
    *reinterpret_cast<float4*>(&(isrow ? rowT : colT)[4 * pq]) = e;
}

template <int CTRL>
__device__ __forceinline__ float dpp_xchg(float v) {
    return __builtin_bit_cast(float, __builtin_amdgcn_update_dpp(0, __builtin_bit_cast(int, v), CTRL, 0xF, 0xF, false));
}
template <int H, int CTRL>
__device__ __forceinline__ void row_reduce_scatter_step(v2f* P, bool bit) {
#pragma unroll
    for (int i = 0; i < H; ++i) {
        const v2f lo = P[i], hi = P[i + H];
        const v2f keep = bit ? hi : lo, send = bit ? lo : hi;
        P[i] = v2f{keep.x + dpp_xchg<CTRL>(send.x), keep.y + dpp_xchg<CTRL>(send.y)};
    }
}

template <int TW, bool STK, int MT = 32, bool FUSE = false>
__device__ __forceinline__ void wino4_epilogue(const ConvArgs& a, const f32x4 (&acc)[36], int n, int th, int tg, int cl, int cb,
                                               int tx0, int ty0, bool live, float* xch = nullptr) {
    constexpr int TC = TW / 4, TR = MT / TC;
    constexpr unsigned OOB = 0x80000000u;
    const int cout0 = cb * 16 + cl;
    const float bias = a.bias[cout0];
    const int Hp = a.H >> 1, Wp = a.W >> 1;
    auto at6 = [&](v2f m0, v2f m1, v2f m2, v2f m3, v2f m4, v2f m5, v2f* t) {
        const v2f s1 = m1 + m2, d1 = m1 - m2, s2 = m3 + m4, d2 = m3 - m4;
        t[0] = m0 + s1 + s2;
        t[1] = fA * d1 + fB * d2;
        t[2] = fA2 * s1 + fB2 * s2;
        t[3] = fA3 * d1 + fB3 * d2 + m5;
    };
    if (!live) return;
    const bool fused = FUSE && a.last_w != nullptr;
#ifdef PNP_DIAG
    const bool nostore = (a.diag & 1) != 0;
#else
    constexpr bool nostore = false;
#endif
    v2f part[2];
    const __amdgpu_buffer_rsrc_t rdst = __builtin_amdgcn_make_buffer_rsrc(
        (void*)(a.dst + (size_t)(n + (STK ? th : 0)) * a.H * a.W * a.Cout), 0, nostore ? 0 : a.H * a.W * a.Cout * 4, 0x00020000);
    const __amdgpu_buffer_rsrc_t rpool = __builtin_amdgcn_make_buffer_rsrc(
        (void*)(a.pooled != nullptr ? a.pooled + (size_t)(n + (STK ? th : 0)) * Hp * Wp * a.Cout : a.dst), 0,
        (a.pooled != nullptr && !nostore) ? Hp * Wp * a.Cout * 4 : 0, 0x00020000);
#pragma unroll
    for (int rp = 0; rp < 2; ++rp) {
        v2f T[4][6];
#pragma unroll
        for (int j = 0; j < 6; ++j) {
            v2f m[6];
#pragma unroll
            for (int i = 0; i < 6; ++i) m[i] = v2f{acc[6 * i + j][2 * rp], acc[6 * i + j][2 * rp + 1]};
            v2f t[4];
            at6(m[0], m[1], m[2], m[3], m[4], m[5], t);
#pragma unroll
            for (int ay = 0; ay < 4; ++ay) T[ay][j] = t[ay];
        }
        v2f Y[4][4];
#pragma unroll
        for (int ay = 0; ay < 4; ++ay) {
            at6(T[ay][0], T[ay][1], T[ay][2], T[ay][3], T[ay][4], T[ay][5], Y[ay]);
#pragma unroll
            for (int ax = 0; ax < 4; ++ax) {
                const v2f sv = Y[ay][ax] + bias;
                Y[ay][ax] = v2f{fmaxf(sv.x, kLeaky * sv.x), fmaxf(sv.y, kLeaky * sv.y)};
            }
        }
        if constexpr (FUSE) {
            if (fused) {
                const float wl = a.last_w[cout0];
                v2f P[16];
#pragma unroll
                for (int i = 0; i < 16; ++i) P[i] = Y[i >> 2][i & 3] * wl;
                row_reduce_scatter_step<8, 0x140>(P, (cl & 8) != 0);
                row_reduce_scatter_step<4, 0x141>(P, (cl & 4) != 0);
                row_reduce_scatter_step<2, 0x1B>(P, (cl & 2) != 0);
                row_reduce_scatter_step<1, 0xB1>(P, (cl & 1) != 0);
                part[rp] = P[0];
                continue;
            }
        }
#pragma unroll
        for (int e = 0; e < 2; ++e) {
            const int t = 16 * th + 4 * tg + 2 * rp + e;
            const int tr = t / TC;
            const int py = STK ? 4 * (tr % (TR / 2)) : 4 * tr, px = 4 * (t % TC);
            const int gy = ty0 + py, gx = tx0 + px;
            const unsigned base = (gx < a.W) ? (unsigned)(((gy * a.W + gx) * a.Cout + cout0) * 4) : OOB;
            const unsigned rowb = (unsigned)(a.W * a.Cout * 4);
#pragma unroll
            for (int ay = 0; ay < 4; ++ay)
#pragma unroll
                for (int ax = 0; ax < 4; ++ax) {
                    const float val = e == 0 ? Y[ay][ax].x : Y[ay][ax].y;
                    __builtin_amdgcn_raw_buffer_store_b32(__builtin_bit_cast(unsigned, val), rdst, base + ay * rowb, ax * a.Cout * 4, 0);
                }
            if (a.pooled != nullptr) {
                const int qy = gy >> 1, qx = gx >> 1;
                const unsigned pbase = (qx < Wp) ? (unsigned)(((qy * Wp + qx) * a.Cout + cout0) * 4) : OOB;
                const unsigned prowb = (unsigned)(Wp * a.Cout * 4);
#pragma unroll
                for (int wy = 0; wy < 2; ++wy)
#pragma unroll
                    for (int wx = 0; wx < 2; ++wx) {
                        const v2f mx = __builtin_elementwise_max(__builtin_elementwise_max(Y[2 * wy][2 * wx], Y[2 * wy][2 * wx + 1]),
                                                                 __builtin_elementwise_max(Y[2 * wy + 1][2 * wx], Y[2 * wy + 1][2 * wx + 1]));
                        const float val = e == 0 ? mx.x : mx.y;
                        __builtin_amdgcn_raw_buffer_store_b32(__builtin_bit_cast(unsigned, val), rpool, pbase + wy * prowb, wx * a.Cout * 4, 0);
                    }
            }
        }
    }
    if constexpr (FUSE) {
        if (fused) {
            const int cq = cb & 1, lane = 16 * tg + cl;
            float4* const x4 = reinterpret_cast<float4*>(xch) + th * 64 + lane;
            if (cq == 1) *x4 = make_float4(part[0].x, part[0].y, part[1].x, part[1].y);
            __syncthreads();
            if (cq == 0) {
                const float4 o = *x4;
                const float sum[4] = {part[0].x + o.x, part[0].y + o.y, part[1].x + o.z, part[1].y + o.w};
                const float lb = a.last_b[0];
#pragma unroll
                for (int r = 0; r < 4; ++r) {
                    const int t = 16 * th + 4 * tg + r;
                    const int gy = ty0 + 4 * (t / TC) + (cl >> 2), gx = tx0 + 4 * (t % TC) + (cl & 3);
                    if (gy < a.H && gx < a.W && !nostore) {
                        const size_t qx = ((size_t)n * a.H + gy) * a.W + gx;
                        const float img = a.last_ximg != nullptr ? a.last_ximg[qx] : (a.last_z[qx].x - a.last_u[qx].x);
                        a.last_out[qx] = fminf(fmaxf(img + sum[r] + lb, 0.f), 1.f);
                    }
                }
            }
        }
    }
}

template <int TW, int SRC, bool STK = false, int WN = 2, int MT = 32>
__global__ __launch_bounds__(8 * MT * WN, 2) void conv3x3_wino4_kernel(const ConvArgs a) {
    constexpr int CK = 8 * WN, CKP = CK, LP = CK, PPP = CK / 4, NT_ = 8 * MT * WN;
    constexpr int CKQ = WN == 2 ? CK + 4 : CK + 2;
    constexpr int HCN = CK / 2;
    constexpr int TC = TW / 4, TR = MT / TC;
    constexpr int TH = 4 * TR;
    constexpr int SUBH = STK ? TH / 2 + 2 : 0;
    constexpr int PH = STK ? 2 * SUBH : TH + 2, PW = TW + 2;
    constexpr int ITEMS = PH * PW * PPP;
    static_assert(!STK || (TW == 16 && SRC == SRC_PLAIN && WN == 2 && MT == 32), "stacked slices: 16-wide tiles, plain source");
    static_assert(MT == 32 || (MT == 16 && WN == 2), "16-tile M-blocks: 64-channel workgroups only");
    constexpr int NIT = (ITEMS + NT_ - 1) / NT_;
    constexpr bool UP2 = SRC == SRC_UPCAT;
    constexpr bool FIRST = SRC == SRC_FIRST;
    constexpr int LH = TH / 2 + 3, LW = TW / 2 + 3;
    constexpr int LITEMS = LH * LW * PPP;
    constexpr int NITL = (LITEMS + NT_ - 1) / NT_;
    constexpr bool SPLIT = UP2 && WN == 2;
    constexpr int NH0 = SPLIT ? (NIT + 1) / 2 : NIT;
    constexpr int NRAW = SPLIT ? (NH0 > NITL ? NH0 : NITL) : ((UP2 && NITL > NIT) ? NITL : NIT);
    constexpr int S = CK / 4;
    constexpr int PF = WN == 2 ? 9 : 12;
    constexpr int KEEP = WN == 1 ? 6 : 3;
    constexpr int PLANE = MT * CKP;
    static_assert(SRC == SRC_PLAIN || SRC == SRC_UPCAT || SRC == SRC_FIRST, "pooled sources go through the pooled copy");
    static_assert(!FIRST || (WN == 1 && MT == 32), "fused first layer: the 32-channel variant");
    static_assert(36 % PF == 0 && MT * HCN * 2 == NT_, "one (tile, 2-channel, column group) transform item per thread");

    extern __shared__ __attribute__((aligned(16))) float smem[];
    float* const patch = smem;
    float* const V = smem + ((PH * PW * CKQ + 3) & ~3);
    float* const lowres = V + 36 * PLANE;
    float* const rowT = lowres + LH * LW * LP;
    float* const colT = rowT + 4 * PH;
    constexpr int IW = PW + 3;
    float* const dimg = V + 36 * PLANE;
    float* const mimg = dimg + (PH + 2) * IW;
    float* const wl = mimg + (PH + 2) * IW;
    float* const bl = wl + 18 * 32;
#ifdef PNP_STAMPS
    unsigned long long st_t0 = W4T(), st_setup = 0, st_loop0 = 0, st_commit = 0, st_trans = 0, st_mfma = 0, st_loop1 = 0, st_ew = 0, st_er = 0, st_tmp = 0;
#endif
    const int tid = threadIdx.x, lane = tid & 63;
    const int wid = __builtin_amdgcn_readfirstlane(tid >> 6);
    const int cq = wid / (MT / 16), th = wid % (MT / 16);
    const int tg = lane >> 4, cl = lane & 15;

    const int ny = a.Cout / (32 * WN);
    const int bid = blockIdx.x;
    const int ntl = a.tilesX * a.tilesY * (STK ? (a.N + 1) / 2 : a.N);
    int cby, bt;
    wino4_decode(bid, ny, ntl, a.order, cby, bt);
    if (bt >= ntl) return;
    const int tx0 = (bt % a.tilesX) * TW;
    bt /= a.tilesX;
    const int ty0 = (bt % a.tilesY) * TH;
    const int n = STK ? 2 * (bt / a.tilesY) : bt / a.tilesY;
    const int nsl = STK ? (n + 1 < a.N ? 2 : 1) : 1;
    const bool live0 = !(a.tact != nullptr && a.tact[n] > 0.5f);
    const bool live1 = STK && nsl == 2 && !(a.tact != nullptr && a.tact[n + 1] > 0.5f);
    if (!live0 && !live1) return;
    const int cb = cby * (2 * WN) + cq;
    const int nchunks = a.Cin / CK;

    const int Hs = a.H >> 1, Ws = a.W >> 1;
    const int ylo = UP2 ? ty0 / 2 - 1 : 0;
    const int xlo = UP2 ? (int)(a.rw * (float)(tx0 > 0 ? tx0 - 1 : 0)) : 0;
    const int nskip = UP2 ? a.Cskip / CK : 0;

    constexpr unsigned OOB = 0x80000000u;
    const int cs = UP2 ? a.Cskip : a.Cin;
#ifdef PNP_DIAG
    const bool hot = (a.diag & 2) != 0;
#else
    constexpr bool hot = false;
#endif
    const int ly0 = hot ? 0 : ty0, lx0 = hot ? 0 : tx0, ln = hot ? 0 : n;
    const __amdgpu_buffer_rsrc_t rsrc0 = __builtin_amdgcn_make_buffer_rsrc(
        (void*)(a.src0 + (size_t)ln * a.H * a.W * cs), 0, nsl * a.H * a.W * cs * 4, 0x00020000);
    unsigned voff[NIT];
#pragma unroll
    for (int k = 0; k < NIT; ++k) {
        const int idx = tid + k * NT_;
        const int part = idx % PPP, pp = idx / PPP;
        const int py = pp / PW, px = pp % PW;
        const int sub = STK ? py / SUBH : 0;
        const int gy = STK ? py % SUBH - 1 : ly0 + py - 1, gx = lx0 + px - 1;
        voff[k] = (idx < ITEMS && sub < nsl && gy >= 0 && gy < a.H && gx >= 0 && gx < a.W)
                      ? (unsigned)((((sub * a.H + gy) * a.W + gx) * cs + part * 4) * 4) : OOB;
    }
    const int Cup = a.Cin - a.Cskip;
    const __amdgpu_buffer_rsrc_t rsrc1 = __builtin_amdgcn_make_buffer_rsrc(
        (void*)(UP2 ? a.src1 + (size_t)ln * Hs * Ws * Cup : a.src0), 0, UP2 ? Hs * Ws * Cup * 4 : 0, 0x00020000);
    unsigned voffL[UP2 ? NITL : 1];
    if constexpr (UP2) {
#pragma unroll
        for (int k = 0; k < NITL; ++k) {
            const int idx = tid + k * NT_;
            const int part = idx % PPP, pp = idx / PPP;
            const int sy = (hot ? -1 : ylo) + pp / LW, sx = (hot ? 0 : xlo) + pp % LW;
            voffL[k] = (idx < LITEMS && sy >= 0 && sy < Hs && sx < Ws) ? (unsigned)(((sy * Ws + sx) * Cup + part * 4) * 4) : OOB;
        }
    }
    const int ldst = ((tid / PPP) * CKQ + (tid % PPP) * 4);
    const int ldstL = ((tid / PPP) * LP + (tid % PPP) * 4);
    auto put_patch = [&](int off, float4 v) {
        if constexpr (CKQ % 4 == 0) *reinterpret_cast<float4*>(&patch[off]) = v;
        else { *reinterpret_cast<float2*>(&patch[off]) = make_float2(v.x, v.y); *reinterpret_cast<float2*>(&patch[off + 2]) = make_float2(v.z, v.w); }
    };

    float4 raw[NRAW];
    auto issue = [&](int c, int half = 0) {
        if (UP2 && c >= nskip) {
            if (half != 0) return;
            const int soff = (c * CK - a.Cskip) * 4;
#pragma unroll
            for (int k = 0; k < NITL; ++k)
                raw[k] = __builtin_bit_cast(float4, __builtin_amdgcn_raw_buffer_load_b128(rsrc1, voffL[k], soff, 0));
            return;
        }
        const int soff = c * CK * 4;
        if (half == 0) {
#pragma unroll
            for (int k = 0; k < NH0; ++k)
                raw[k] = __builtin_bit_cast(float4, __builtin_amdgcn_raw_buffer_load_b128(rsrc0, voff[k], soff, 0));
        } else {
#pragma unroll
            for (int k = NH0; k < NIT; ++k)
                raw[k - NH0] = __builtin_bit_cast(float4, __builtin_amdgcn_raw_buffer_load_b128(rsrc0, voff[k], soff, 0));
        }
    };
    auto park = [&](int c, int half = 0) {
        if (UP2 && c >= nskip) {
            if (half != 0) return;
#pragma unroll
            for (int k = 0; k < NITL; ++k) {
                const int idx = tid + k * NT_;
                if (idx < LITEMS) *reinterpret_cast<float4*>(&lowres[ldstL + k * (NT_ / PPP) * LP]) = raw[k];
            }
            return;
        }
        if (half == 0) {
#pragma unroll
            for (int k = 0; k < NH0; ++k) {
                const int idx = tid + k * NT_;
                if (idx < ITEMS) put_patch(ldst + k * (NT_ / PPP) * CKQ, raw[k]);
            }
        } else {
#pragma unroll
            for (int k = NH0; k < NIT; ++k) {
                const int idx = tid + k * NT_;
                if (idx < ITEMS) put_patch(ldst + k * (NT_ / PPP) * CKQ, raw[k - NH0]);
            }
        }
    };
    typedef Wino4Interp<PH, PW, PPP, NT_ / 64> IG;
    static_assert(!UP2 || (IG::ING >= 1 && (PPP & (PPP - 1)) == 0 && TH % 2 == 0), "row groups of whole waves; even tile origin");
    static_assert(!UP2 || ((PH - 1) / 2 + 1 < LH), "the parked region holds every candidate line");
    auto interpolate = [&]() {
        wino4_interpolate<PH, PW, PPP, LH, LW, LP, NT_ / 64, PW * CKQ>(lowres, rowT, colT, wid, tid,
            [](int y, int x, int part) { return ((y * PW + x) * CKQ) + part * 4; }, [&](int off, float4 v) { put_patch(off, v); });
    };
    bool first_interior = false;
    int fbase[FIRST ? NIT : 1];
    if constexpr (FIRST) {
        first_interior = ty0 >= 2 && ty0 + TH + 2 <= a.H && tx0 >= 2 && tx0 + TW + 2 <= a.W;
        const float sg = a.first_sigma[n];
        for (int i = tid; i < (PH + 2) * (PW + 2); i += NT_) {
            const int r = i / (PW + 2), q = i % (PW + 2);
            const int gy = ty0 - 2 + r, gx = tx0 - 2 + q;
            float d = 0.f, m = 0.f;
            if (gy >= 0 && gy < a.H && gx >= 0 && gx < a.W) {
                const size_t qx = ((size_t)n * a.H + gy) * a.W + gx;
                d = a.last_ximg != nullptr ? a.last_ximg[qx] : (a.last_z[qx].x - a.last_u[qx].x);
                m = 1.f;
            }
            dimg[r * IW + q] = d;
            mimg[r * IW + q] = m;
        }
        for (int i = tid; i < 32 * 18; i += NT_) {
            const int ch = i / 18, t = i % 18;
            wl[t * 32 + ch] = a.first_w[i] * (t >= 9 ? sg : 1.f);
        }
        if (tid < 32) {
            float sc = 0.f;
#pragma unroll
            for (int t = 9; t < 18; ++t) sc += a.first_w[tid * 18 + t] * sg;
            bl[tid] = a.first_b[tid];
            bl[32 + tid] = a.first_b[tid] + sc;
        }
#pragma unroll
        for (int k = 0; k < NIT; ++k) {
            const int pp = (tid + k * NT_) / PPP;
            fbase[k] = (tid + k * NT_ < ITEMS) ? (pp / PW) * IW + pp % PW : 0;
        }
        __syncthreads();
    }
    auto first_patch = [&](int c) {
        if constexpr (FIRST) {
            const int part = tid % PPP;
            const float* const wq = wl + CK * c + 4 * part;
            const f32x4 b4 = *reinterpret_cast<const f32x4*>(bl + (first_interior ? 32 : 0) + CK * c + 4 * part);
            f32x4 acc[NIT];
#pragma unroll
            for (int k = 0; k < NIT; ++k) acc[k] = b4;
#pragma unroll
            for (int t = 0; t < 9; ++t) {
                const f32x4 w4 = *reinterpret_cast<const f32x4*>(wq + t * 32);
#pragma unroll
                for (int k = 0; k < NIT; ++k) acc[k] = __builtin_elementwise_fma(w4, f32x4(dimg[fbase[k] + (t / 3) * IW + t % 3]), acc[k]);
            }
            if (!first_interior) {
#pragma unroll
                for (int t = 0; t < 9; ++t) {
                    const f32x4 w4 = *reinterpret_cast<const f32x4*>(wq + (9 + t) * 32);
#pragma unroll
                    for (int k = 0; k < NIT; ++k) acc[k] = __builtin_elementwise_fma(w4, f32x4(mimg[fbase[k] + (t / 3) * IW + t % 3]), acc[k]);
                }
            }
#pragma unroll
            for (int k = 0; k < NIT; ++k) {
                const int idx = tid + k * NT_;
                if (idx < ITEMS) {
                    const float in = first_interior ? 1.f : mimg[fbase[k] + IW + 1];
                    const f32x4 v = in * __builtin_elementwise_max(acc[k], kLeaky * acc[k]);
                    put_patch((idx / PPP) * CKQ + part * 4, make_float4(v[0], v[1], v[2], v[3]));
                }
            }
        }
    };
    if constexpr (UP2) {
        wino4_upsample_tables<PH, PW, LP>(a, tid, ty0, tx0, ylo, xlo, rowT, colT);
    }
    if constexpr (FIRST) first_patch(0);
    else {
        issue(0); park(0);
        if constexpr (SPLIT) { issue(0, 1); park(0, 1); }
    }

    auto swz = [](int t16, int g) { return WN == 2 ? (g ^ ((4 - (t16 >> 2)) & 3)) : (g ^ ((t16 >> 3) << 1)); };
    const int hc = tid % HCN, tq = (tid / HCN) % MT;
    const int tj = wid / (NT_ / 128);
    const int trow = tq / TC;
    const int wrow = STK ? (trow / (TR / 2)) * SUBH + 4 * (trow % (TR / 2)) : 4 * trow;
    const int win = (wrow * PW + 4 * (tq % TC)) * CKQ + 2 * hc;
    const int vout = WN == 2 ? tq * CKP + 4 * swz(tq & 15, hc >> 1) + 2 * (hc & 1)
                             : tq * CKP + 2 * swz(tq & 15, hc);

    f32x4 acc[36];
#pragma unroll
    for (int k = 0; k < 36; ++k) acc[k] = f32x4{0.f, 0.f, 0.f, 0.f};

    typedef typename std::conditional<WN == 2, float4, float2>::type frag_t;
    const size_t stream = (size_t)nchunks * 36 * 64 + kW4Tail / S;
    const __amdgpu_buffer_rsrc_t rB = __builtin_amdgcn_make_buffer_rsrc(
        (void*)(reinterpret_cast<const frag_t*>(a.wpack) + (size_t)cb * stream), 0, (int)(stream * sizeof(frag_t)), 0x00020000);
    const int boff = lane * (int)sizeof(frag_t);
    const frag_t* const bptr = reinterpret_cast<const frag_t*>(a.wpack) + (size_t)cb * stream + lane;
    auto bfrag = [&](const frag_t* bp, int f0, int i) -> frag_t {
        if constexpr (!UP2) return bp[i * 64];
        else if constexpr (WN == 2) return __builtin_bit_cast(frag_t, __builtin_amdgcn_raw_buffer_load_b128(rB, boff, (f0 + i) * (64 * 16), 0));
        else return __builtin_bit_cast(frag_t, __builtin_amdgcn_raw_buffer_load_b64(rB, boff, (f0 + i) * (64 * 8), 0));
    };
    frag_t bq[PF];
#pragma unroll
    for (int p = 0; p < KEEP; ++p) bq[p] = bfrag(bptr, 0, p);
    const int aoff = (16 * th + cl) * CKP + S * swz(cl, tg);

#ifdef PNP_STAMPS
    st_setup = W4T();
    st_loop0 = st_setup;
#endif
    for (int c = 0; c < nchunks; ++c) {
#ifdef PNP_STAMPS
        st_tmp = W4T();
#endif
        __syncthreads();
        if (UP2 && c >= nskip) {
            if constexpr (NT_ == 256) __builtin_amdgcn_s_setprio(3);
            interpolate();
            if constexpr (NT_ == 256) __builtin_amdgcn_s_setprio(0);
            __syncthreads();
        }
#ifdef PNP_STAMPS
        { const unsigned long long t = W4T(); st_commit += t - st_tmp; st_tmp = t; }
#endif

        if constexpr (WN == 1 && !FIRST) { if (c + 1 < nchunks) issue(c + 1); }
        __builtin_amdgcn_sched_barrier(0);
        if constexpr (NT_ == 256) __builtin_amdgcn_s_setprio(3);
        if (tj == 0) wino4_input_transform<0, PW, CKQ, PLANE>(patch + win, V + vout);
        else wino4_input_transform<1, PW, CKQ, PLANE>(patch + win, V + vout);
        if constexpr (NT_ == 256) __builtin_amdgcn_s_setprio(0);
        __builtin_amdgcn_sched_barrier(0);
        const frag_t* bp = bptr + (size_t)c * 36 * 64;
        const int bf0 = c * 36;
#pragma unroll
        for (int p = KEEP; p < PF; ++p) bq[p] = bfrag(bp, bf0, p);
        if constexpr (WN == 2) { if (c + 1 < nchunks) issue(c + 1); }
        __syncthreads();
#ifdef PNP_STAMPS
        { const unsigned long long t = W4T(); st_trans += t - st_tmp; st_tmp = t; }
#endif

        frag_t ar[3];
        ar[0] = *reinterpret_cast<const frag_t*>(&V[aoff]);
        ar[1] = *reinterpret_cast<const frag_t*>(&V[PLANE + aoff]);
#pragma unroll
        for (int xi = 0; xi < 36; ++xi) {
            if (xi + 2 < 36) ar[(xi + 2) % 3] = *reinterpret_cast<const frag_t*>(&V[(xi + 2) * PLANE + aoff]);
            __builtin_amdgcn_sched_barrier(0);
            const frag_t a0 = ar[xi % 3], b0 = bq[xi % PF];
            acc[xi] = __builtin_amdgcn_mfma_f32_16x16x4f32(a0.x, b0.x, acc[xi], 0, 0, 0);
            acc[xi] = __builtin_amdgcn_mfma_f32_16x16x4f32(a0.y, b0.y, acc[xi], 0, 0, 0);
            if constexpr (WN == 2) {
                acc[xi] = __builtin_amdgcn_mfma_f32_16x16x4f32(a0.z, b0.z, acc[xi], 0, 0, 0);
                acc[xi] = __builtin_amdgcn_mfma_f32_16x16x4f32(a0.w, b0.w, acc[xi], 0, 0, 0);
            }
            __builtin_amdgcn_sched_barrier(0);
            if constexpr (SPLIT) {
                if (xi == 17 && c + 1 < nchunks) { park(c + 1, 0); issue(c + 1, 1); }
            }
#ifdef PNP_DIAG
            if ((a.diag & 4) && (xi & 1)) continue;
#endif
            if (xi + PF < 36 + KEEP) bq[xi % PF] = bfrag(bp, bf0, xi + PF);
        }
#ifdef PNP_STAMPS
        { const unsigned long long t = W4T(); st_mfma += t - st_tmp; }
#endif
        if (c + 1 < nchunks) {
            if constexpr (FIRST) first_patch(c + 1);
            else park(c + 1, SPLIT ? 1 : 0);
        }
    }
#ifdef PNP_STAMPS
    st_loop1 = W4T();
    st_tmp = st_loop1;
#endif

    wino4_epilogue<TW, STK, MT, WN == 1 && MT == 32 && SRC == SRC_PLAIN>(a, acc, n, th, tg, cl, cb, tx0, ty0, STK ? (th == 0 ? live0 : live1) : true, smem);
#ifdef PNP_STAMPS
    {
        const int w = (int)blockIdx.x - (int)(gridDim.x / 2);
        if (tid == 0 && w >= 0 && w < W4_WGS && a.stamp_slot < W4_SLOTS) {
            unsigned long long* o = g_w4_stamps + ((size_t)a.stamp_slot * W4_WGS + w) * W4_N;
            const unsigned long long te = W4T();
            o[0] = 1; o[1] = st_setup - st_t0; o[2] = st_commit; o[3] = st_trans; o[4] = st_mfma; o[5] = st_loop1 - st_loop0;
            o[6] = te - st_tmp; o[7] = 0; o[8] = te - st_loop1; o[9] = te - st_t0; o[10] = (unsigned long long)nchunks;
        }
    }
#endif
}

template <int TW, bool STK>
__global__ __launch_bounds__(512, 2) void conv3x3_wino4p_kernel(const ConvArgs a) {
    constexpr int CK = 16, CKP = 16, PPP = 4, NT_ = 512, S = 4;
    constexpr int TC = TW / 4, TR = 32 / TC;
    constexpr int TH = 4 * TR;
    constexpr int SUBH = STK ? TH / 2 + 2 : 0;
    constexpr int PH = STK ? 2 * SUBH : TH + 2, PW = TW + 2;
    constexpr int NPIX = PH * PW, ITEMS = NPIX * PPP;
    constexpr int NIT = (ITEMS + NT_ - 1) / NT_;
    constexpr int PLSZ = ((NPIX * 4 + 15) / 16) * 16 + 4;
    constexpr int PATCH = 4 * PLSZ;
    constexpr int PF = 12, KEEP = 3;
    constexpr int PLANE = 32 * CKP;
    constexpr unsigned OOB = 0x80000000u;
    static_assert(!STK || TW == 16, "stacked slices: 16-wide tiles");
    static_assert((2 * PATCH + 36 * PLANE) * 4 <= 160 * 1024, "two patch copies + V in one CU's LDS");

    extern __shared__ __attribute__((aligned(16))) float smem[];
    float* const patch = smem;
    float* const V = smem + 2 * PATCH;
#ifdef PNP_STAMPS
    unsigned long long st_t0 = W4T(), st_setup = 0, st_loop0 = 0, st_commit = 0, st_trans = 0, st_mfma = 0, st_loop1 = 0, st_tmp = 0;
#endif
    const int tid = threadIdx.x, lane = tid & 63;
    const int wid = __builtin_amdgcn_readfirstlane(tid >> 6);
    const int grp = wid >> 2, cq = wid & 3;
    const int th = grp;
    const int tg = lane >> 4, cl = lane & 15;

    const int ny = a.Cout / 64;
    const int bid = blockIdx.x;
    const int ntl = a.tilesX * a.tilesY * (STK ? (a.N + 1) / 2 : a.N);
    int cby, bt;
    wino4_decode(bid, ny, ntl, a.order, cby, bt);
    if (bt >= ntl) return;
    const int tx0 = (bt % a.tilesX) * TW;
    bt /= a.tilesX;
    const int ty0 = (bt % a.tilesY) * TH;
    const int n = STK ? 2 * (bt / a.tilesY) : bt / a.tilesY;
    const int nsl = STK ? (n + 1 < a.N ? 2 : 1) : 1;
    const bool live0 = !(a.tact != nullptr && a.tact[n] > 0.5f);
    const bool live1 = STK && nsl == 2 && !(a.tact != nullptr && a.tact[n + 1] > 0.5f);
    if (!live0 && !live1) return;
    const int cb = cby * 4 + cq;
    const int nchunks = a.Cin / CK;

    const __amdgpu_buffer_rsrc_t rsrc0 = __builtin_amdgcn_make_buffer_rsrc(
        (void*)(a.src0 + (size_t)n * a.H * a.W * a.Cin), 0, nsl * a.H * a.W * a.Cin * 4, 0x00020000);
    unsigned voff[NIT];
#pragma unroll
    for (int k = 0; k < NIT; ++k) {
        const int idx = tid + k * NT_;
        const int part = idx % PPP, pp = idx / PPP;
        const int py = pp / PW, px = pp % PW;
        const int sub = STK ? py / SUBH : 0;
        const int gy = STK ? py % SUBH - 1 : ty0 + py - 1, gx = tx0 + px - 1;
        voff[k] = (idx < ITEMS && sub < nsl && gy >= 0 && gy < a.H && gx >= 0 && gx < a.W)
                      ? (unsigned)((((sub * a.H + gy) * a.W + gx) * a.Cin + part * 4) * 4) : OOB;
    }
    const int ldst = (tid & 3) * PLSZ + (tid >> 2) * 4;
    float4 raw[NIT];
    auto issue = [&](int c) {
        const int soff = c * CK * 4;
#pragma unroll
        for (int k = 0; k < NIT; ++k)
            raw[k] = __builtin_bit_cast(float4, __builtin_amdgcn_raw_buffer_load_b128(rsrc0, voff[k], soff, 0));
    };
    auto park = [&](int c) {
        float* const dst = patch + (c & 1) * PATCH + ldst;
#pragma unroll
        for (int k = 0; k < NIT; ++k)
            if (tid + k * NT_ < ITEMS) *reinterpret_cast<float4*>(&dst[k * (NT_ / PPP) * 4]) = raw[k];
    };

    auto swz = [](int t16, int g) { return g ^ ((4 - (t16 >> 2)) & 3); };
    const int tgi = tid & 255;
    const int hc = tgi & 7, t16 = (tgi >> 3) & 15;
    const int tj = (wid >> 1) & 1;
    const int tq = 16 * grp + t16;
    const int trow = tq / TC;
    const int wrow = STK ? (trow / (TR / 2)) * SUBH + 4 * (trow % (TR / 2)) : 4 * trow;
    const int win = (hc >> 1) * PLSZ + (wrow * PW + 4 * (tq % TC)) * 4 + 2 * (hc & 1);
    const int vout = tq * CKP + 4 * swz(t16, hc >> 1) + 2 * (hc & 1);

    f32x4 acc[36];
#pragma unroll
    for (int k = 0; k < 36; ++k) acc[k] = f32x4{0.f, 0.f, 0.f, 0.f};

    const size_t stream = (size_t)nchunks * 36 * 64 + kW4Tail / S;
    const float4* const bptr = reinterpret_cast<const float4*>(a.wpack) + (size_t)cb * stream + lane;
    float4 bq[PF];
#pragma unroll
    for (int p = 0; p < KEEP; ++p) bq[p] = bptr[p * 64];
    const int aoff = (16 * th + cl) * CKP + 4 * swz(cl, tg);

    constexpr bool PARK_T = !STK;
    issue(0);
    park(0);
    if constexpr (!PARK_T) { if (grp == 1 && nchunks > 1) { issue(1); park(1); } }
#ifdef PNP_STAMPS
    st_setup = W4T();
    st_loop0 = st_setup;
#endif
    if (grp == 1) __syncthreads();
    for (int c = 0; c < nchunks; ++c) {
#ifdef PNP_STAMPS
        st_tmp = W4T();
#endif
        __syncthreads();
#ifdef PNP_STAMPS
        { const unsigned long long t = W4T(); st_commit += t - st_tmp; st_tmp = t; }
#endif
        if constexpr (PARK_T) { if (c + 1 < nchunks) issue(c + 1); }
        __builtin_amdgcn_s_setprio(3);
        {
            const float* const w = patch + (c & 1) * PATCH + win;
            if (tj == 0) wino4_input_transform<0, PW, 4, PLANE>(w, V + vout);
            else wino4_input_transform<1, PW, 4, PLANE>(w, V + vout);
        }
        __builtin_amdgcn_s_setprio(0);
        __builtin_amdgcn_sched_barrier(0);
        const float4* bp = bptr + (size_t)c * 36 * 64;
#pragma unroll
        for (int p = KEEP; p < PF; ++p) bq[p] = bp[p * 64];
        const int nx = c + 1 + grp;
        if constexpr (PARK_T) { if (c + 1 < nchunks) park(c + 1); }
        else { if (nx < nchunks) issue(nx); }
        __syncthreads();
#ifdef PNP_STAMPS
        { const unsigned long long t = W4T(); st_trans += t - st_tmp; st_tmp = t; }
#endif

        float4 ar[3];
        ar[0] = *reinterpret_cast<const float4*>(&V[aoff]);
        ar[1] = *reinterpret_cast<const float4*>(&V[PLANE + aoff]);
#pragma unroll
        for (int xi = 0; xi < 36; ++xi) {
            if (xi + 2 < 36) ar[(xi + 2) % 3] = *reinterpret_cast<const float4*>(&V[(xi + 2) * PLANE + aoff]);
            __builtin_amdgcn_sched_barrier(0);
            const float4 a0 = ar[xi % 3], b0 = bq[xi % PF];
            acc[xi] = __builtin_amdgcn_mfma_f32_16x16x4f32(a0.x, b0.x, acc[xi], 0, 0, 0);
            acc[xi] = __builtin_amdgcn_mfma_f32_16x16x4f32(a0.y, b0.y, acc[xi], 0, 0, 0);
            acc[xi] = __builtin_amdgcn_mfma_f32_16x16x4f32(a0.z, b0.z, acc[xi], 0, 0, 0);
            acc[xi] = __builtin_amdgcn_mfma_f32_16x16x4f32(a0.w, b0.w, acc[xi], 0, 0, 0);
            __builtin_amdgcn_sched_barrier(0);
#ifdef PNP_DIAG
            if ((a.diag & 4) && (xi & 1)) continue;
#endif
            if (xi + PF < 36 + KEEP) bq[xi % PF] = bp[(xi + PF) * 64];
        }
#ifdef PNP_STAMPS
        { const unsigned long long t = W4T(); st_mfma += t - st_tmp; }
#endif
        if constexpr (!PARK_T) { if (nx < nchunks) park(nx); }
    }
    if (grp == 0) __syncthreads();
#ifdef PNP_STAMPS
    st_loop1 = W4T();
    st_tmp = st_loop1;
#endif

    wino4_epilogue<TW, STK>(a, acc, n, th, tg, cl, cb, tx0, ty0, STK ? (th == 0 ? live0 : live1) : true);
#ifdef PNP_STAMPS
    {
        const int w = (int)blockIdx.x - (int)(gridDim.x / 2);
        if (tid == 0 && w >= 0 && w < W4_WGS && a.stamp_slot < W4_SLOTS) {
            unsigned long long* o = g_w4_stamps + ((size_t)a.stamp_slot * W4_WGS + w) * W4_N;
            const unsigned long long te = W4T();
            o[0] = 1; o[1] = st_setup - st_t0; o[2] = st_commit; o[3] = st_trans; o[4] = st_mfma; o[5] = st_loop1 - st_loop0;
            o[6] = te - st_tmp; o[7] = 0; o[8] = te - st_loop1; o[9] = te - st_t0; o[10] = (unsigned long long)nchunks;
        }
    }
#endif
}

template <int TW, int SRC>
__global__ __launch_bounds__(512, 2) void conv3x3_wino4c_kernel(const ConvArgs a) {
    constexpr int CK = 16, CKP = 16, PPP = 4, NT_ = 512, S = 4, MT = 16;
    constexpr bool UP2 = SRC == SRC_UPCAT;
    static_assert(SRC == SRC_PLAIN || SRC == SRC_UPCAT, "plain or upsample + concat source");
    constexpr int TC = TW / 4, TR = MT / TC;
    constexpr int TH = 4 * TR;
    constexpr int PH = TH + 2, PW = TW + 2;
    constexpr int NPIX = PH * PW, ITEMS = NPIX * PPP;
    constexpr int NIT = (ITEMS + NT_ - 1) / NT_;
    constexpr int PLSZ = ((NPIX * 4 + 15) / 16) * 16 + 4;
    constexpr int PATCH = 4 * PLSZ;
    constexpr int PF = 12, KEEP = 3;
    constexpr int PLANE = MT * CKP;
    constexpr int VSZ = 36 * PLANE;
    constexpr unsigned OOB = 0x80000000u;
    static_assert(NIT == 3 && ITEMS <= NIT * NT_, "three staging items per thread");
    constexpr int LP = CK;
    constexpr int LH = TH / 2 + 3, LW = TW / 2 + 3;
    constexpr int LITEMS = LH * LW * PPP, NITL = (LITEMS + NT_ - 1) / NT_;
    constexpr int LOWRES = LH * LW * LP;
    static_assert((2 * PATCH + 2 * VSZ + (UP2 ? 2 * LOWRES + 4 * (PH + PW) : 0)) * 4 <= 160 * 1024, "everything in one CU's LDS");

    extern __shared__ __attribute__((aligned(16))) float smem[];
    float* const patch = smem;
    float* const V = smem + 2 * PATCH;
    float* const lowres = V + 2 * VSZ;
    float* const rowT = lowres + 2 * LOWRES;
    float* const colT = rowT + 4 * PH;
#ifdef PNP_STAMPS
    unsigned long long st_t0 = W4T(), st_setup = 0, st_loop0 = 0, st_commit = 0, st_trans = 0, st_mfma = 0, st_loop1 = 0, st_tmp = 0;
#endif
    const int tid = threadIdx.x, lane = tid & 63;
    const int wid = __builtin_amdgcn_readfirstlane(tid >> 6);
    const int half = wid >> 2;
    const int tg = lane >> 4, cl = lane & 15;

    const int ny = a.Cout / 128;
    const int bid = blockIdx.x;
    const int ntl = a.tilesX * a.tilesY * a.N;
    int cby, bt;
    wino4_decode(bid, ny, ntl, a.order, cby, bt);
    if (bt >= ntl) return;
    const int tx0 = (bt % a.tilesX) * TW;
    bt /= a.tilesX;
    const int ty0 = (bt % a.tilesY) * TH;
    const int n = bt / a.tilesY;
    if (a.tact != nullptr && a.tact[n] > 0.5f) return;
    const int cb = cby * 8 + wid;
    const int nchunks = a.Cin / CK;
    const int cs = UP2 ? a.Cskip : a.Cin;
    const int nskip = UP2 ? a.Cskip / CK : nchunks;
    const int Hs = a.H >> 1, Ws = a.W >> 1;
    const int ylo = UP2 ? ty0 / 2 - 1 : 0;
    const int xlo = UP2 ? (int)(a.rw * (float)(tx0 > 0 ? tx0 - 1 : 0)) : 0;

    const __amdgpu_buffer_rsrc_t rsrc0 = __builtin_amdgcn_make_buffer_rsrc(
        (void*)(a.src0 + (size_t)n * a.H * a.W * cs), 0, a.H * a.W * cs * 4, 0x00020000);
    unsigned voff[NIT];
#pragma unroll
    for (int k = 0; k < NIT; ++k) {
        const int idx = tid + k * NT_;
        const int part = idx % PPP, pp = idx / PPP;
        const int gy = ty0 + pp / PW - 1, gx = tx0 + pp % PW - 1;
        voff[k] = (idx < ITEMS && gy >= 0 && gy < a.H && gx >= 0 && gx < a.W) ? (unsigned)(((gy * a.W + gx) * cs + part * 4) * 4) : OOB;
    }
    const int ldst = (tid & 3) * PLSZ + (tid >> 2) * 4;
    float4 raw[NIT];
    const int Cup = a.Cin - a.Cskip;
    const __amdgpu_buffer_rsrc_t rsrc1 = __builtin_amdgcn_make_buffer_rsrc(
        (void*)(UP2 ? a.src1 + (size_t)n * Hs * Ws * Cup : a.src0), 0, UP2 ? Hs * Ws * Cup * 4 : 0, 0x00020000);
    unsigned voffL[UP2 ? NITL : 1];
    float4 rawL[UP2 ? NITL : 1];
    if constexpr (UP2) {
#pragma unroll
        for (int k = 0; k < NITL; ++k) {
            const int idx = tid + k * NT_;
            const int part = idx % PPP, pp = idx / PPP;
            const int sy = ylo + pp / LW, sx = xlo + pp % LW;
            voffL[k] = (idx < LITEMS && sy >= 0 && sy < Hs && sx < Ws) ? (unsigned)(((sy * Ws + sx) * Cup + part * 4) * 4) : OOB;
        }
    }
    const int ldstL = (tid >> 2) * LP + (tid & 3) * 4;
    auto issueL = [&](int c) {
        if constexpr (UP2) {
            const int soff = (c * CK - a.Cskip) * 4;
#pragma unroll
            for (int k = 0; k < NITL; ++k)
                rawL[k] = __builtin_bit_cast(float4, __builtin_amdgcn_raw_buffer_load_b128(rsrc1, voffL[k], soff, 0));
        }
    };
    auto parkL = [&](int c) {
        if constexpr (UP2) {
            float* const dst = lowres + (c & 1) * LOWRES + ldstL;
#pragma unroll
            for (int k = 0; k < NITL; ++k)
                if (tid + k * NT_ < LITEMS) *reinterpret_cast<float4*>(&dst[k * (NT_ / PPP) * LP]) = rawL[k];
        }
    };
    static_assert(Wino4Interp<PH, PW, PPP, 4>::ING >= 1 && TH % 2 == 0 && (PH - 1) / 2 + 1 < LH, "row groups of whole waves; even tile origin; every candidate line parked");
    auto interpolate = [&](int c) {
        if constexpr (UP2) {
            float* const pdst = patch + (c & 1) * PATCH;
            wino4_interpolate<PH, PW, PPP, LH, LW, LP, 4, PW * 4>(lowres + (c & 1) * LOWRES, rowT, colT, wid & 3, tid & 255,
                [](int y, int x, int part) { return part * PLSZ + (y * PW + x) * 4; }, [&](int off, float4 v) { *reinterpret_cast<float4*>(&pdst[off]) = v; });
        }
    };
    if constexpr (UP2) {
        wino4_upsample_tables<PH, PW, LP>(a, tid, ty0, tx0, ylo, xlo, rowT, colT);
    }
    auto issue = [&](int c) {
        const int soff = c * CK * 4;
#pragma unroll
        for (int k = 0; k < NIT; ++k)
            raw[k] = __builtin_bit_cast(float4, __builtin_amdgcn_raw_buffer_load_b128(rsrc0, voff[k], soff, 0));
    };
    auto park = [&](int c) {
        float* const dst = patch + (c & 1) * PATCH + ldst;
#pragma unroll
        for (int k = 0; k < NIT; ++k)
            if (tid + k * NT_ < ITEMS) *reinterpret_cast<float4*>(&dst[k * (NT_ / PPP) * 4]) = raw[k];
    };

    auto swz = [](int t16, int g) { return g ^ ((4 - (t16 >> 2)) & 3); };
    const int tgi = tid & 255;
    const int hc = tgi & 7, t16 = (tgi >> 3) & 15;
    const int tj = (wid >> 1) & 1;
    const int win = (hc >> 1) * PLSZ + (4 * (t16 / TC) * PW + 4 * (t16 % TC)) * 4 + 2 * (hc & 1);
    const int vout = t16 * CKP + 4 * swz(t16, hc >> 1) + 2 * (hc & 1);
    auto transform = [&](int c) {
        const float* const w = patch + (c & 1) * PATCH + win;
        float* const v = V + (c & 1) * VSZ + vout;
        if (tj == 0) wino4_input_transform<0, PW, 4, PLANE>(w, v);
        else wino4_input_transform<1, PW, 4, PLANE>(w, v);
    };

    f32x4 acc[36];
#pragma unroll
    for (int k = 0; k < 36; ++k) acc[k] = f32x4{0.f, 0.f, 0.f, 0.f};

    const size_t stream = (size_t)nchunks * 36 * 64 + kW4Tail / S;
    const __amdgpu_buffer_rsrc_t rB = __builtin_amdgcn_make_buffer_rsrc(
        (void*)(reinterpret_cast<const float4*>(a.wpack) + (size_t)cb * stream), 0, (int)(stream * sizeof(float4)), 0x00020000);
    const int boff = lane * (int)sizeof(float4);
    const float4* const bptr = reinterpret_cast<const float4*>(a.wpack) + (size_t)cb * stream + lane;
    auto bfrag = [&](const float4* bp, int f0, int i) -> float4 {
        if constexpr (!UP2) return bp[i * 64];
        else return __builtin_bit_cast(float4, __builtin_amdgcn_raw_buffer_load_b128(rB, boff, (f0 + i) * (64 * 16), 0));
    };
    float4 bq[PF];
#pragma unroll
    for (int p = 0; p < KEEP; ++p) bq[p] = bfrag(bptr, 0, p);
    const int aoff = cl * CKP + 4 * swz(cl, tg);

    issue(0);
    park(0);
    if (nchunks > 1) issue(1);
    __syncthreads();
    if (half == 1) transform(0);
    if (nchunks > 1) park(1);
#ifdef PNP_STAMPS
    st_setup = W4T();
    st_loop0 = st_setup;
#endif
    for (int c = 0; c < nchunks; ++c) {
#ifdef PNP_STAMPS
        st_tmp = W4T();
#endif
        __syncthreads();
#ifdef PNP_STAMPS
        { const unsigned long long t = W4T(); st_commit += t - st_tmp; st_tmp = t; }
#endif
        if (half == (c & 1)) {
            if (c + 1 < nchunks) {
                __builtin_amdgcn_s_setprio(3);
                transform(c + 1);
                __builtin_amdgcn_s_setprio(0);
            }
        } else if (UP2 && c + 2 >= nskip && c + 2 < nchunks) {
            __builtin_amdgcn_s_setprio(3);
            interpolate(c + 2);
            __builtin_amdgcn_s_setprio(0);
        }
        __builtin_amdgcn_sched_barrier(0);
        const float4* bp = bptr + (size_t)c * 36 * 64;
        const int bf0 = c * 36;
#pragma unroll
        for (int p = KEEP; p < PF; ++p) bq[p] = bfrag(bp, bf0, p);
        if (c + 2 < nskip) issue(c + 2);
        if (UP2 && c + 3 >= nskip && c + 3 < nchunks) issueL(c + 3);
#ifdef PNP_STAMPS
        { const unsigned long long t = W4T(); st_trans += t - st_tmp; st_tmp = t; }
#endif

        const float* const Vc = V + (c & 1) * VSZ + aoff;
        float4 ar[3];
        ar[0] = *reinterpret_cast<const float4*>(&Vc[0]);
        ar[1] = *reinterpret_cast<const float4*>(&Vc[PLANE]);
#pragma unroll
        for (int xi = 0; xi < 36; ++xi) {
            if (xi + 2 < 36) ar[(xi + 2) % 3] = *reinterpret_cast<const float4*>(&Vc[(xi + 2) * PLANE]);
            __builtin_amdgcn_sched_barrier(0);
            const float4 a0 = ar[xi % 3], b0 = bq[xi % PF];
            acc[xi] = __builtin_amdgcn_mfma_f32_16x16x4f32(a0.x, b0.x, acc[xi], 0, 0, 0);
            acc[xi] = __builtin_amdgcn_mfma_f32_16x16x4f32(a0.y, b0.y, acc[xi], 0, 0, 0);
            acc[xi] = __builtin_amdgcn_mfma_f32_16x16x4f32(a0.z, b0.z, acc[xi], 0, 0, 0);
            acc[xi] = __builtin_amdgcn_mfma_f32_16x16x4f32(a0.w, b0.w, acc[xi], 0, 0, 0);
            __builtin_amdgcn_sched_barrier(0);
            if (xi + PF < 36 + KEEP) bq[xi % PF] = bfrag(bp, bf0, xi + PF);
        }
#ifdef PNP_STAMPS
        { const unsigned long long t = W4T(); st_mfma += t - st_tmp; }
#endif
        if (c + 2 < nskip) park(c + 2);
        if (UP2 && c + 3 >= nskip && c + 3 < nchunks) parkL(c + 3);
    }
#ifdef PNP_STAMPS
    st_loop1 = W4T();
    st_tmp = st_loop1;
#endif

    wino4_epilogue<TW, false, 16>(a, acc, n, 0, tg, cl, cb, tx0, ty0, true);
#ifdef PNP_STAMPS
    {
        const int w = (int)blockIdx.x - (int)(gridDim.x / 2);
        if (tid == 0 && w >= 0 && w < W4_WGS && a.stamp_slot < W4_SLOTS) {
            unsigned long long* o = g_w4_stamps + ((size_t)a.stamp_slot * W4_WGS + w) * W4_N;
            const unsigned long long te = W4T();
            o[0] = 1; o[1] = st_setup - st_t0; o[2] = st_commit; o[3] = st_trans; o[4] = st_mfma; o[5] = st_loop1 - st_loop0;
            o[6] = te - st_tmp; o[7] = 0; o[8] = te - st_loop1; o[9] = te - st_t0; o[10] = (unsigned long long)nchunks;
        }
    }
#endif
}

template <int TW, int SRC>
static hipError_t launch_wino4c_inst(const ConvArgs& a, const WinoPlan& p, hipStream_t s) {
    constexpr int TC = TW / 4, TR = 16 / TC, TH = 4 * TR;
    constexpr int NPIX = (TH + 2) * (TW + 2);
    constexpr int PLSZ = ((NPIX * 4 + 15) / 16) * 16 + 4;
    constexpr size_t lowres_f = SRC == SRC_UPCAT ? (size_t)2 * (TH / 2 + 3) * (TW / 2 + 3) * 16 + 4 * (TH + 2 + TW + 2) : 0;
    constexpr size_t lds = ((size_t)2 * 4 * PLSZ + (size_t)2 * 36 * 16 * 16 + lowres_f) * sizeof(float);
    if (p.th != TH || p.tw != TW) return hipErrorInvalidValue;
    if (SRC == SRC_UPCAT && a.Cskip < 3 * 16) return hipErrorInvalidValue;
    auto kern = conv3x3_wino4c_kernel<TW, SRC>;
    static DeviceOnce cap;
    if (hipError_t e = raise_lds_cap((const void*)kern, (int)lds, cap); e != hipSuccess) return e;
    const int ntiles = p.tiles_x * p.tiles_y * a.N, ny = a.Cout / 128;
    dim3 grid((unsigned)(((ntiles + 7) / 8) * 8 * ny));
    hipLaunchKernelGGL(kern, grid, dim3(512), lds, s, a);
    return hipGetLastError();
}

template <int TW, bool STK>
static hipError_t launch_wino4p_inst(const ConvArgs& a, const WinoPlan& p, hipStream_t s) {
    constexpr int TC = TW / 4, TR = 32 / TC, TH = 4 * TR;
    constexpr int NPIX = (STK ? TH + 4 : TH + 2) * (TW + 2);
    constexpr int PLSZ = ((NPIX * 4 + 15) / 16) * 16 + 4;
    constexpr size_t lds = ((size_t)2 * 4 * PLSZ + (size_t)36 * 32 * 16) * sizeof(float);
    auto kern = conv3x3_wino4p_kernel<TW, STK>;
    static DeviceOnce cap;
    if (hipError_t e = raise_lds_cap((const void*)kern, (int)lds, cap); e != hipSuccess) return e;
    const int ntiles = p.tiles_x * p.tiles_y * (STK ? (a.N + 1) / 2 : a.N), ny = a.Cout / 64;
    dim3 grid((unsigned)(((ntiles + 7) / 8) * 8 * ny));
    hipLaunchKernelGGL(kern, grid, dim3(512), lds, s, a);
    return hipGetLastError();
}

template <int TW, int SRC, bool STK = false, int WN = 2, int MT = 32>
static hipError_t launch_wino4_inst(const ConvArgs& a, const WinoPlan& p, hipStream_t s) {
    constexpr int CK = 8 * WN, CKP = CK, CKQ = WN == 2 ? CK + 4 : CK + 2, TC = TW / 4, TR = MT / TC, TH = 4 * TR;
    constexpr size_t patch_f = (((size_t)(STK ? TH + 4 : TH + 2) * (TW + 2) * CKQ + 3) / 4) * 4;
    constexpr size_t lowres_f = SRC == SRC_UPCAT ? (size_t)(TH / 2 + 3) * (TW / 2 + 3) * CK + 4 * (TH + 2 + TW + 2) : 0;
    constexpr size_t first_f = SRC == SRC_FIRST ? (size_t)2 * (TH + 4) * (TW + 5) + 18 * 32 + 64 : 0;
    constexpr size_t lds = (patch_f + (size_t)36 * MT * CKP + lowres_f + first_f) * sizeof(float);
    static_assert(lds <= (WN == 2 && MT == 32 ? 160 : 80) * 1024, "one (8 waves) / two (4 waves) workgroups per CU");
    if (p.th != TH || p.tw != TW) return hipErrorInvalidValue;
    auto kern = conv3x3_wino4_kernel<TW, SRC, STK, WN, MT>;
    static DeviceOnce cap;
    if (hipError_t e = raise_lds_cap((const void*)kern, (int)lds, cap); e != hipSuccess) return e;
    const int ntiles = p.tiles_x * p.tiles_y * (STK ? (a.N + 1) / 2 : a.N), ny = a.Cout / (32 * WN);
    dim3 grid((unsigned)(((ntiles + 7) / 8) * 8 * ny));
    hipLaunchKernelGGL(kern, grid, dim3(8 * MT * WN), lds, s, a);
    return hipGetLastError();
}

hipError_t launch_conv3x3_winograd4(const ConvArgs& a0, const WinoPlan& p, int src_mode, hipStream_t s) {
    if (!p.use || p.algo != 4 || a0.Cout % p.bn || a0.Cin % p.ck || (src_mode == SRC_UPCAT && a0.Cskip % p.ck) || a0.W % 4) return hipErrorInvalidValue;
    if (a0.last_w != nullptr && !(p.bn == 32 && p.mt == 32 && src_mode == SRC_PLAIN)) return hipErrorInvalidValue;
    ConvArgs a = a0;
    a.tilesX = p.tiles_x;
    a.tilesY = p.tiles_y;
    a.order = p.order;
#ifdef PNP_STAMPS
    a.stamp_slot = g_w4_slot++;
#endif
    if (p.bn == 32) {
        if (p.ck != 8 || p.stack) return hipErrorInvalidValue;
        if (p.tw == 32 && src_mode == SRC_PLAIN) return launch_wino4_inst<32, SRC_PLAIN, false, 1>(a, p, s);
        if (p.tw == 32 && src_mode == SRC_UPCAT) return launch_wino4_inst<32, SRC_UPCAT, false, 1>(a, p, s);
        if (p.tw == 32 && src_mode == SRC_FIRST) return launch_wino4_inst<32, SRC_FIRST, false, 1>(a, p, s);
        if (p.tw == 16 && src_mode == SRC_FIRST) return launch_wino4_inst<16, SRC_FIRST, false, 1>(a, p, s);
        if (p.tw == 16 && src_mode == SRC_PLAIN) return launch_wino4_inst<16, SRC_PLAIN, false, 1>(a, p, s);
        if (p.tw == 16 && src_mode == SRC_UPCAT) return launch_wino4_inst<16, SRC_UPCAT, false, 1>(a, p, s);
        return hipErrorInvalidValue;
    }
    if (p.ck != 16) return hipErrorInvalidValue;
    if (p.cs) {
        if (p.bn != 128 || p.mt != 16 || p.stack) return hipErrorInvalidValue;
        if (p.tw == 32 && src_mode == SRC_PLAIN) return launch_wino4c_inst<32, SRC_PLAIN>(a, p, s);
        if (p.tw == 32 && src_mode == SRC_UPCAT) return launch_wino4c_inst<32, SRC_UPCAT>(a, p, s);
        if (p.tw == 16 && src_mode == SRC_PLAIN) return launch_wino4c_inst<16, SRC_PLAIN>(a, p, s);
        if (p.tw == 16 && src_mode == SRC_UPCAT) return launch_wino4c_inst<16, SRC_UPCAT>(a, p, s);
        return hipErrorInvalidValue;
    }
    if (p.mt == 16) {
        if (p.stack) return hipErrorInvalidValue;
        if (p.tw == 32 && src_mode == SRC_PLAIN) return launch_wino4_inst<32, SRC_PLAIN, false, 2, 16>(a, p, s);
        if (p.tw == 32 && src_mode == SRC_UPCAT) return launch_wino4_inst<32, SRC_UPCAT, false, 2, 16>(a, p, s);
        if (p.tw == 16 && src_mode == SRC_PLAIN) return launch_wino4_inst<16, SRC_PLAIN, false, 2, 16>(a, p, s);
        if (p.tw == 16 && src_mode == SRC_UPCAT) return launch_wino4_inst<16, SRC_UPCAT, false, 2, 16>(a, p, s);
        return hipErrorInvalidValue;
    }
    if (p.phased && src_mode == SRC_PLAIN) {
        if (p.tw == 32 && !p.stack) return launch_wino4p_inst<32, false>(a, p, s);
        if (p.tw == 16) {
            if (p.stack) return a.H == 16 && a.W == 16 ? launch_wino4p_inst<16, true>(a, p, s) : hipErrorInvalidValue;
            return launch_wino4p_inst<16, false>(a, p, s);
        }
        return hipErrorInvalidValue;
    }
    if (p.tw == 32) {
        if (src_mode == SRC_PLAIN) return launch_wino4_inst<32, SRC_PLAIN>(a, p, s);
        if (src_mode == SRC_UPCAT) return launch_wino4_inst<32, SRC_UPCAT>(a, p, s);
    } else if (p.tw == 16) {
        if (p.stack) return src_mode == SRC_PLAIN && a.H == 16 && a.W == 16 ? launch_wino4_inst<16, SRC_PLAIN, true>(a, p, s) : hipErrorInvalidValue;
        if (src_mode == SRC_PLAIN) return launch_wino4_inst<16, SRC_PLAIN>(a, p, s);
        if (src_mode == SRC_UPCAT) return launch_wino4_inst<16, SRC_UPCAT>(a, p, s);
    }
    return hipErrorInvalidValue;
}

}

#ifdef PNP_STAMPS
extern "C" int pnp_debug_stamps4_reset(void) { pnp::g_w4_slot = 0; return 0; }
extern "C" int pnp_debug_stamps4_read(unsigned long long* dst, int slots) {
    return (int)hipMemcpyFromSymbol(dst, HIP_SYMBOL(pnp::g_w4_stamps), (size_t)slots * W4_WGS * W4_N * sizeof(unsigned long long));
}
#endif
```

### dt4image_restoration_amd/csrc/winograd_kernels.hip

```cpp
#include "pnp_internal.h"
#include "conv_staging.h"
#include <cstdlib>

namespace pnp {

#ifdef PNP_STAMPS
#define PNP_STAMP_SLOTS 32
#define PNP_STAMP_WGS 1024
#define PNP_STAMP_N 112
__device__ unsigned long long g_wino_stamps[PNP_STAMP_SLOTS * PNP_STAMP_WGS * PNP_STAMP_N];
static int g_stamp_slot = 0;
#define STAMP() do { if (ns < PNP_STAMP_N) st[ns] = __builtin_amdgcn_s_memtime(); ++ns; } while (0)
#else
#define STAMP() do { } while (0)
#endif

size_t winograd_pack_floats(int cin, int cout) { return (size_t)(cout / 32) * ((size_t)(cin / 8) * 16 * 256 + 2 * 4 * 256); }

void pack_winograd_weights(const float* oihw, int cin, int cout, int ck, float* dst) {
    static const double G[4][3] = {{1, 0, 0}, {0.5, 0.5, 0.5}, {0.5, -0.5, 0.5}, {0, 0, 1}};
    std::vector<float> U((size_t)cout * cin * 16);
    for (int co = 0; co < cout; ++co)
        for (int ci = 0; ci < cin; ++ci) {
            const float* g = oihw + ((size_t)co * cin + ci) * 9;
            double t[4][3];
            for (int i = 0; i < 4; ++i)
                for (int kx = 0; kx < 3; ++kx) t[i][kx] = G[i][0] * g[kx] + G[i][1] * g[3 + kx] + G[i][2] * g[6 + kx];
            for (int i = 0; i < 4; ++i)
                for (int j = 0; j < 4; ++j)
                    U[((size_t)co * cin + ci) * 16 + 4 * i + j] = (float)(t[i][0] * G[j][0] + t[i][1] * G[j][1] + t[i][2] * G[j][2]);
        }
    size_t o = 0;
    for (int cb = 0; cb < cout / 32; ++cb)
        for (int half = 0; half < 2; ++half) {
            for (int ch = 0; ch < cin / ck; ++ch)
                for (int ks = 0; ks < ck / 8; ++ks)
                    for (int k = 0; k < 8; ++k)
                        for (int l = 0; l < 64; ++l)
                            for (int j = 0; j < 4; ++j) {
                                const int co = 32 * cb + (l & 31);
                                const int ci = ck * ch + 8 * ks + 4 * (l >> 5) + j;
                                dst[o++] = U[((size_t)co * cin + ci) * 16 + 8 * half + k];
                            }
            for (int i = 0; i < 4 * 256; ++i) dst[o++] = 0.f;
        }
}


WinoPlan winograd_plan(int N, int H, int W, int Cin, int Cout, int src_mode, const Tuning& t, int Cskip) {
    constexpr long kCsMinBlocks = 256;
    WinoPlan p{};
    p.use = false;
    p.algo = 1;
    if (t.no_wino || Cin < t.wino_min_cin || Cin % 32 || Cout % 32) return p;
    if (!t.no_f4 && Cin >= t.f4_min_cin && (Cout % 64 == 0 || Cout == 32) && Cin % 16 == 0 && (src_mode == SRC_PLAIN || src_mode == SRC_UPCAT) &&
        W >= 16 && H >= 16 && (W >= 32 || H >= 32 || (W == 16 && H == 16 && src_mode == SRC_PLAIN && N >= 2)) &&
        W % 4 == 0 &&
        (src_mode != SRC_UPCAT || upsample_lines_regular(H))) {
        WinoPlan f{};
        f.algo = 4;
        f.order = (t.f4_order && (long)H * W >= 32 * 32) ? 1 : 0;
        f.tw = W >= 32 ? 32 : 16;
        f.th = f.tw == 32 ? 16 : 32;
        f.bn = 64; f.wm = 1; f.wn = 2; f.ck = 16;
        if (Cout == 32) { f.bn = 32; f.wn = 1; f.ck = 8; }
        f.tiles_x = (W + f.tw - 1) / f.tw;
        f.tiles_y = (H + f.th - 1) / f.th;
        f.stack = (W == 16 && H == 16) ? 1 : 0;
        if (!(f.stack && Cout == 32)) {
            f.mt = 32;
            const bool mt16 = t.f4_mt16 == 0 ? (src_mode == SRC_UPCAT || Cin <= 64) : (t.f4_mt16 == 1 ? false : (t.f4_mt16 == 2 ? src_mode == SRC_UPCAT : true));
            if (f.bn == 64 && mt16 && (f.tw == 32 ? H >= 8 : H >= 16)) {
                f.mt = 16;
                f.th = f.tw == 32 ? 8 : 16;
                f.tiles_y = (H + f.th - 1) / f.th;
                f.stack = 0;
            }
            f.phased = (f.mt == 32 && f.bn == 64 && src_mode == SRC_PLAIN && !t.no_f4_phased) ? 1 : 0;
            const bool cs_can = f.bn == 64 && Cout % 128 == 0 && (src_mode == SRC_PLAIN || (Cskip % 16 == 0 && Cskip >= 48));
            const int cs_th = f.tw == 32 ? 8 : 16;
            const long cs_blocks = (long)f.tiles_x * ((H + cs_th - 1) / cs_th) * N * (Cout / 128);
            const bool cs_rule = src_mode == SRC_UPCAT && cs_blocks >= kCsMinBlocks;
            if (cs_can && cs_blocks >= t.wino_min_blocks && (t.f4_cs == 2 || (t.f4_cs == 1 && t.f4_mt16 == 0 && !t.no_f4_phased && cs_rule))) {
                f.cs = 1;
                f.bn = 128;
                f.mt = 16;
                f.th = cs_th;
                f.tiles_y = (H + f.th - 1) / f.th;
                f.stack = 0;
                f.phased = 0;
            }
            const long blocks = (long)f.tiles_x * f.tiles_y * (f.stack ? (N + 1) / 2 : N) * (Cout / f.bn);
            f.use = blocks >= t.wino_min_blocks;
            if (f.use) return f;
        }
    }
    p.tw = W >= 32 ? 32 : (W >= 16 ? 16 : 8);
    const bool big = t.wino_big;
    if (Cout % 128 == 0 && !t.wino_small) { p.wm = 1; p.wn = 4; p.ck = 32; }
    else if (Cout % 64 == 0) { if (big) { p.wm = 2; p.wn = 2; } else { p.wm = 1; p.wn = 2; } p.ck = 16; }
    else { if (big) { p.wm = 4; p.wn = 1; } else { p.wm = 2; p.wn = 1; } p.ck = 8; }
    const int tc = p.tw / 2, tr = 32 / tc;
    p.th = p.wm * 2 * tr;
    p.bn = p.wn * 32;
    p.tiles_x = (W + p.tw - 1) / p.tw;
    p.tiles_y = (H + p.th - 1) / p.th;
    const long blocks = (long)p.tiles_x * p.tiles_y * N * (Cout / p.bn);
    p.use = blocks >= t.wino_min_blocks;
    return p;
}

template <int TW, int WM, int WN, int CK, int SRC>
__global__ __launch_bounds__(WM * WN * 128, 2) void conv3x3_winograd_kernel(const ConvArgs a) {
    constexpr int GW = WM * WN;
    constexpr int NT_ = GW * 128;
    constexpr int CKP = CK + 4;
    constexpr int PPP = CK / 4;
    constexpr int TC = TW / 2, TR = 32 / TC;
    constexpr int TH = WM * 2 * TR;
    constexpr int NTILES = WM * 32;
    constexpr int PWL = TW + 2, PH = TH + 2, PW = PWL;
    constexpr int ITEMS = PH * PWL * PPP;
    constexpr int NIT = (ITEMS + NT_ - 1) / NT_;
    constexpr bool UP2 = SRC == SRC_UPCAT;
    constexpr bool PREFETCH = SRC == SRC_PLAIN || UP2;
    constexpr int LH = TH / 2 + 3, LW = TW / 2 + 3;
    constexpr int LITEMS = LH * LW * PPP;
    constexpr int NITL = (LITEMS + NT_ - 1) / NT_;
    constexpr int NRAW = PREFETCH ? (UP2 && NITL > NIT ? NITL : NIT) : (NIT < 3 ? NIT : 3);
    constexpr int LB = PREFETCH ? NIT : (NIT < 3 ? NIT : 3);
    constexpr int KSC = CK / 8;
    constexpr int PAIRS = 8 * KSC;
    constexpr int PF = 4;
    static_assert((GW == 4 || GW == 2) && NTILES * PPP * 2 == NT_, "one (tile, 4-channel, frequency-half) transform item per thread");

#ifdef PNP_STAMPS
    unsigned long long st[PNP_STAMP_N];
    int ns = 0;
    STAMP();
#endif
    extern __shared__ __attribute__((aligned(16))) float smem[];
    float* const patch = smem;
    float* const V = smem + PH * PW * CKP;
    float* const lowres = V + 16 * NTILES * CKP;

    const int tid = threadIdx.x, lane = tid & 63, wid = tid >> 6;
    const int xh = wid / GW;
    const int wm = (wid % GW) / WN, wn = (wid % GW) % WN;
    const int hh = lane >> 5, li = lane & 31;

    int bt = blockIdx.x;
    const int tx0 = (bt % a.tilesX) * TW;
    bt /= a.tilesX;
    const int ty0 = (bt % a.tilesY) * TH;
    const int n = bt / a.tilesY;
    const int cb = blockIdx.y * WN + wn;
    if (a.tact != nullptr && a.tact[n] > 0.5f) return;
    const int nchunks = a.Cin / CK;

    const int Hs = a.H >> 1, Ws = a.W >> 1;
    const int ylo = UP2 ? (int)(a.rh * (float)(ty0 > 0 ? ty0 - 1 : 0)) : 0;
    const int xlo = UP2 ? (int)(a.rw * (float)(tx0 > 0 ? tx0 - 1 : 0)) : 0;
    const int nskip = UP2 ? a.Cskip / CK : 0;

    float4 raw[NRAW][(SRC == SRC_POOL) ? 4 : 1];
    auto issue = [&](int c, int it0, int cnt) {
        if (UP2 && c >= nskip) {
            const int Cup = a.Cin - a.Cskip;
            const float* base = a.src1 + (size_t)n * Hs * Ws * Cup + (c * CK - a.Cskip);
#pragma unroll
            for (int k = 0; k < NITL; ++k) {
                const int idx = tid + k * NT_;
                const int part = idx % PPP, pp = idx / PPP;
                const int sy = ylo + pp / LW, sx = xlo + pp % LW;
                if (idx < LITEMS && sy < Hs && sx < Ws)
                    raw[k][0] = *reinterpret_cast<const float4*>(base + ((size_t)sy * Ws + sx) * Cup + part * 4);
            }
            return;
        }
#pragma unroll
        for (int k = 0; k < cnt; ++k) {
            const int idx = tid + (it0 + k) * NT_;
            const int part = idx % PPP, pp = idx / PPP;
            const int py = pp / PWL, px = pp % PWL;
            const int gy = ty0 + py - 1, gx = tx0 + px - 1;
            if (idx < ITEMS && gy >= 0 && gy < a.H && gx >= 0 && gx < a.W) {
                if constexpr (SRC == SRC_POOL) {
                    RawPiece<SRC_POOL> r;
                    issue_piece<SRC_POOL>(a, n, gy, gx, c * CK + part * 4, r);
                    raw[k][0] = r.v[0]; raw[k][1] = r.v[1]; raw[k][2] = r.v[2]; raw[k][3] = r.v[3];
                } else {
                    const int cs = UP2 ? a.Cskip : a.Cin;
                    raw[k][0] = *reinterpret_cast<const float4*>(a.src0 + (((size_t)n * a.H + gy) * a.W + gx) * cs + c * CK + part * 4);
                }
            }
        }
    };
    auto commit = [&](int c, int it0, int cnt) {
        if (UP2 && c >= nskip) {
#pragma unroll
            for (int k = 0; k < NITL; ++k) {
                const int idx = tid + k * NT_;
                if (idx < LITEMS) *reinterpret_cast<float4*>(&lowres[(idx / PPP) * CKP + (idx % PPP) * 4]) = raw[k][0];
            }
            __syncthreads();
#pragma unroll
            for (int k = 0; k < NIT; ++k) {
                const int idx = tid + k * NT_;
                const int part = idx % PPP, pp = idx / PPP;
                const int py = pp / PWL, px = pp % PWL;
                const int gy = ty0 + py - 1, gx = tx0 + px - 1;
                if (idx < ITEMS) {
                    float4 v = make_float4(0.f, 0.f, 0.f, 0.f);
                    if (gy >= 0 && gy < a.H && gx >= 0 && gx < a.W) {
                        const float sy = a.rh * (float)gy, sx = a.rw * (float)gx;
                        const int y0 = (int)sy, x0 = (int)sx;
                        const int y1 = y0 + (y0 < Hs - 1 ? 1 : 0), x1 = x0 + (x0 < Ws - 1 ? 1 : 0);
                        const float ly = fminf(fmaxf(sy - (float)y0, 0.f), 1.f), lx = fminf(fmaxf(sx - (float)x0, 0.f), 1.f);
                        const float* r0 = &lowres[((y0 - ylo) * LW - xlo) * CKP + part * 4];
                        const float* r1 = &lowres[((y1 - ylo) * LW - xlo) * CKP + part * 4];
                        v = f4lerp2(*reinterpret_cast<const float4*>(r0 + x0 * CKP), *reinterpret_cast<const float4*>(r0 + x1 * CKP),
                                    *reinterpret_cast<const float4*>(r1 + x0 * CKP), *reinterpret_cast<const float4*>(r1 + x1 * CKP),
                                    1.f - lx, lx, 1.f - ly, ly);
                    }
                    *reinterpret_cast<float4*>(&patch[(py * PW + px) * CKP + part * 4]) = v;
                }
            }
            return;
        }
#pragma unroll
        for (int k = 0; k < cnt; ++k) {
            const int idx = tid + (it0 + k) * NT_;
            const int part = idx % PPP, pp = idx / PPP;
            const int py = pp / PWL, px = pp % PWL;
            const int gy = ty0 + py - 1, gx = tx0 + px - 1;
            if (idx < ITEMS) {
                float4 v = make_float4(0.f, 0.f, 0.f, 0.f);
                if (gy >= 0 && gy < a.H && gx >= 0 && gx < a.W) {
                    if constexpr (SRC == SRC_POOL) v = f4max(f4max(raw[k][0], raw[k][1]), f4max(raw[k][2], raw[k][3]));
                    else v = raw[k][0];
                }
                *reinterpret_cast<float4*>(&patch[(py * PW + px) * CKP + part * 4]) = v;
            }
        }
    };
// ... 248 lines not shown
```

### dt4image_restoration_amd/engine.py

```python
from __future__ import annotations

import ctypes as C
from typing import Dict, Mapping, Optional, Tuple

import numpy as np
import torch

from . import _lib
from .weights import flatten_state_dict

RESIDUAL_COLUMNS = _lib.RESIDUAL_COLUMNS


def _ptr(t: Optional[torch.Tensor]) -> Optional[int]:
    return None if t is None else t.data_ptr()


_episode_counter = 0


def _next_episode() -> int:
    global _episode_counter
    _episode_counter += 1
    return _episode_counter
# ... 745 lines not shown
                                                     _ptr(gram), self._stream()), "pnp_coil_compress_matrix")
        return (cmat, eig, gram) if return_gram else (cmat, eig)

    def coil_compress_apply(self, planes: torch.Tensor, cmat: torch.Tensor, out_coils: int) -> torch.Tensor:
        if planes.dim() != 4 or planes.shape[0] != self.n or tuple(planes.shape[-2:]) != (self.h, self.w):
            raise ValueError(f"planes: expected [{self.n},C,{self.h},{self.w}], got {tuple(planes.shape)}")
        coils = int(planes.shape[1])
        planes = self._chk(planes, torch.complex64, self.n * coils * self.h * self.w, "planes")
        if tuple(cmat.shape) not in ((coils, coils), (1, coils, coils), (self.n, coils, coils)):
            raise ValueError(f"cmat: expected [{coils},{coils}] or [{self.n},{coils},{coils}], got {tuple(cmat.shape)}")
        cmat_n = 1 if cmat.numel() == coils * coils else self.n
        cmat = self._chk(cmat, torch.complex64, cmat_n * coils * coils, "cmat")
        out_coils = int(out_coils)
        if not 1 <= out_coils <= min(coils, _lib.PNP_MC_MAX_COILS):
            raise ValueError(f"out_coils must be 1..{min(coils, _lib.PNP_MC_MAX_COILS)}, got {out_coils}")
        out = torch.empty((self.n, out_coils, self.h, self.w), dtype=torch.complex64, device=self.device)
        _lib.check(self.lib.pnp_coil_compress_apply(self._h, planes.data_ptr(), coils, cmat.data_ptr(), cmat_n, out_coils, out.data_ptr(),
                                                    self._stream()), "pnp_coil_compress_apply")
        return out

    def noise_cov(self, noise: torch.Tensor) -> torch.Tensor:
        if noise.dim() not in (2, 3):
            raise ValueError(f"noise: expected [C,S] or [M,C,S], got {tuple(noise.shape)}")
        m = 1 if noise.dim() == 2 else int(noise.shape[0])
        coils, samples = int(noise.shape[-2]), int(noise.shape[-1])
        noise = self._chk(noise, torch.complex64, m * coils * samples, "noise")
        psi = torch.empty((m, coils, coils), dtype=torch.complex128, device=self.device)
        _lib.check(self.lib.pnp_noise_cov(self._h, noise.data_ptr(), m, coils, samples, 0, psi.data_ptr(), self._stream()), "pnp_noise_cov")
        return psi[0] if noise.dim() == 2 else psi

    def whiten_matrix(self, psi: torch.Tensor) -> Tuple[torch.Tensor, torch.Tensor, torch.Tensor]:
        if psi.dim() not in (2, 3) or psi.shape[-1] != psi.shape[-2]:
            raise ValueError(f"psi: expected [C,C] or [M,C,C], got {tuple(psi.shape)}")
        m = 1 if psi.dim() == 2 else int(psi.shape[0])
        coils = int(psi.shape[-1])
        psi = self._chk(psi, torch.complex128, m * coils * coils, "psi")
        wmat = torch.empty(tuple(psi.shape), dtype=torch.complex64, device=self.device)
        lmat = torch.empty_like(wmat)
        info = torch.empty((m,), dtype=torch.int32, device=self.device)
        _lib.check(self.lib.pnp_whiten_matrix(self._h, psi.data_ptr(), m, coils, 0, wmat.data_ptr(), lmat.data_ptr(), info.data_ptr(),
                                              self._stream()), "pnp_whiten_matrix")
        return wmat, lmat, info

    def whiten_apply(self, planes: torch.Tensor, wmat: torch.Tensor, out: Optional[torch.Tensor] = None) -> torch.Tensor:
        if planes.dim() != 4 or planes.shape[0] != self.n or tuple(planes.shape[-2:]) != (self.h, self.w):
            raise ValueError(f"planes: expected [{self.n},C,{self.h},{self.w}], got {tuple(planes.shape)}")
        coils = int(planes.shape[1])
        planes = self._chk(planes, torch.complex64, self.n * coils * self.h * self.w, "planes")
        if tuple(wmat.shape) not in ((coils, coils), (1, coils, coils), (self.n, coils, coils)):
            raise ValueError(f"wmat: expected [{coils},{coils}] or [{self.n},{coils},{coils}], got {tuple(wmat.shape)}")
        wmat_n = 1 if wmat.numel() == coils * coils else self.n
        wmat = self._chk(wmat, torch.complex64, wmat_n * coils * coils, "wmat")
        if out is None:
            out = torch.empty_like(planes)
        elif tuple(out.shape) != tuple(planes.shape):
            raise ValueError(f"out: expected {tuple(planes.shape)}, got {tuple(out.shape)}")
        out = self._chk(out, torch.complex64, planes.numel(), "out")
        _lib.check(self.lib.pnp_whiten_apply(self._h, planes.data_ptr(), coils, wmat.data_ptr(), wmat_n, out.data_ptr(), self._stream()),
                   "pnp_whiten_apply")
        return out

    @staticmethod
    def _grappa_kernel(coils: int, accel: int, kernel) -> Tuple[int, int, int, int]:
        by, bx = (int(v) for v in kernel)
        if not 1 <= coils <= _lib.PNP_GRAPPA_MAX_COILS:
            raise ValueError(f"grappa takes 1..{_lib.PNP_GRAPPA_MAX_COILS} coils, got {coils}: compress the channels first")
        if not 2 <= accel <= _lib.PNP_GRAPPA_MAX_ACCEL:
            raise ValueError(f"accel must be 2..{_lib.PNP_GRAPPA_MAX_ACCEL}, got {accel}")
        if by not in (1, 3, 5, 7) or bx not in (2, 4) or coils * by * bx > _lib.PNP_GRAPPA_MAX_SRC:
            raise ValueError(f"kernel must be (1|3|5|7, 2|4) with coils * by * bx <= {_lib.PNP_GRAPPA_MAX_SRC}, got {(by, bx)} at {coils} coils")
        return by, bx, coils * by * bx, coils * (accel - 1)

    def grappa_weights(self, y0: torch.Tensor, acs: Tuple[int, int], accel: int, kernel: Tuple[int, int] = (5, 4), lam: float = 1e-2,
                       return_gram: bool = False):
        if y0.dim() != 4 or y0.shape[0] != self.n or tuple(y0.shape[-2:]) != (self.h, self.w):
            raise ValueError(f"y0: expected [{self.n},C,{self.h},{self.w}], got {tuple(y0.shape)}")
        coils, accel = int(y0.shape[1]), int(accel)
        y0 = self._chk(y0, torch.complex64, self.n * coils * self.h * self.w, "y0")
        by, bx, ns, nt = self._grappa_kernel(coils, accel, kernel)
        acs_h, acs_w = (int(v) for v in acs)
        wts = torch.empty((self.n, nt, ns), dtype=torch.complex64, device=self.device)
        info = torch.empty((self.n,), dtype=torch.int32, device=self.device)
        gram = torch.empty((self.n, ns, ns + nt), dtype=torch.complex128, device=self.device) if return_gram else None
        _lib.check(self.lib.pnp_grappa_weights(self._h, y0.data_ptr(), coils, acs_h, acs_w, accel, by, bx, float(lam), 0, wts.data_ptr(),
                                               info.data_ptr(), _ptr(gram), self._stream()), "pnp_grappa_weights")
        return (wts, info, gram) if return_gram else (wts, info)

    def grappa_apply(self, y0: torch.Tensor, wts: torch.Tensor, mask: torch.Tensor, accel: int, offset: int, kernel: Tuple[int, int] = (5, 4),
                     out: Optional[torch.Tensor] = None) -> torch.Tensor:
        if y0.dim() != 4 or y0.shape[0] != self.n or tuple(y0.shape[-2:]) != (self.h, self.w):
            raise ValueError(f"y0: expected [{self.n},C,{self.h},{self.w}], got {tuple(y0.shape)}")
        coils, accel, offset = int(y0.shape[1]), int(accel), int(offset)
        y0 = self._chk(y0, torch.complex64, self.n * coils * self.h * self.w, "y0")
        by, bx, ns, nt = self._grappa_kernel(coils, accel, kernel)
        if tuple(wts.shape) not in ((nt, ns), (1, nt, ns), (self.n, nt, ns)):
            raise ValueError(f"wts: expected [{nt},{ns}] or [{self.n},{nt},{ns}], got {tuple(wts.shape)}")
        wts_n = 1 if wts.numel() == nt * ns else self.n
        wts = self._chk(wts, torch.complex64, wts_n * nt * ns, "wts")
        m, mask_n = self._mask(mask)
        if out is None:
            out = torch.empty_like(y0)
        elif tuple(out.shape) != tuple(y0.shape):
            raise ValueError(f"out: expected {tuple(y0.shape)}, got {tuple(out.shape)}")
        out = self._chk(out, torch.complex64, y0.numel(), "out")
        _lib.check(self.lib.pnp_grappa_apply(self._h, y0.data_ptr(), coils, m.data_ptr(), mask_n, accel, offset, by, bx, wts.data_ptr(), wts_n,
                                             out.data_ptr(), self._stream()), "pnp_grappa_apply")
        return out

    def snapshot(self, x: torch.Tensor, z: torch.Tensor, u: torch.Tensor, t_state: Optional[torch.Tensor] = None,
                 out: Optional[torch.Tensor] = None) -> torch.Tensor:
        nhw = self.n * self.h * self.w
        self._chk(x, torch.float32, nhw, "x"); self._chk(z, torch.complex64, nhw, "z"); self._chk(u, torch.complex64, nhw, "u")
        if t_state is not None:
            self._chk(t_state, torch.float32, self.n, "t_state")
        nbytes = self.lib.pnp_snapshot_bytes(self._h)
        if out is None:
            out = torch.empty(nbytes, dtype=torch.uint8, device=self.device)
        elif out.numel() * out.element_size() != nbytes or not out.is_contiguous() or out.device != self.device:
            raise ValueError(f"snapshot buffer must be {nbytes} contiguous bytes on {self.device}")
        _lib.check(self.lib.pnp_snapshot(self._h, x.data_ptr(), z.data_ptr(), u.data_ptr(), _ptr(t_state), out.data_ptr(),
                                         self._stream()), "pnp_snapshot")
        return out

    def restore(self, snap: torch.Tensor, x: torch.Tensor, z: torch.Tensor, u: torch.Tensor,
                t_state: Optional[torch.Tensor] = None) -> None:
        nhw = self.n * self.h * self.w
        self._chk(x, torch.float32, nhw, "x"); self._chk(z, torch.complex64, nhw, "z"); self._chk(u, torch.complex64, nhw, "u")
        if t_state is not None:
            self._chk(t_state, torch.float32, self.n, "t_state")
        if snap.numel() * snap.element_size() != self.lib.pnp_snapshot_bytes(self._h) or not snap.is_contiguous():
            raise ValueError("not a snapshot of this engine")
        _lib.check(self.lib.pnp_restore(self._h, snap.data_ptr(), x.data_ptr(), z.data_ptr(), u.data_ptr(), _ptr(t_state),
                                        self._stream()), "pnp_restore")

    def read_stage(self, which: int) -> torch.Tensor:
        c, hh, ww = C.c_int(), C.c_int(), C.c_int()
        _lib.check(self.lib.pnp_unet_read_stage(self._h, which, None, C.byref(c), C.byref(hh), C.byref(ww), self._stream()),
                   "pnp_unet_read_stage")
        out = torch.empty((self.n, c.value, hh.value, ww.value), dtype=torch.float32, device=self.device)
        _lib.check(self.lib.pnp_unet_read_stage(self._h, which, out.data_ptr(), None, None, None, self._stream()),
                   "pnp_unet_read_stage")
        return out

    def conv_algorithms(self):
        out = (C.c_int32 * _lib.N_LAYERS)()
        _lib.check(self.lib.pnp_conv_algorithms(self._h, out), "pnp_conv_algorithms")
        return list(out)

    def conv_schedules(self):
        out = (C.c_int32 * _lib.N_LAYERS)()
        _lib.check(self.lib.pnp_conv_schedules(self._h, out), "pnp_conv_schedules")
        return list(out)

    def bf16_weight_terms(self) -> int:
        return int(self.lib.pnp_bf16_weight_terms(self._h))

    def profile_reset(self) -> None:
        _lib.check(self.lib.pnp_profile_reset(self._h), "pnp_profile_reset")

    def profile_collect(self) -> Dict[str, Dict[str, float]]:
        ms = (C.c_double * _lib.PROFILE_CLASSES)()
        cnt = (C.c_int64 * _lib.PROFILE_CLASSES)()
        _lib.check(self.lib.pnp_profile_collect(self._h, ms, cnt), "pnp_profile_collect")
        lms = (C.c_double * _lib.N_LAYERS)()
        lcnt = (C.c_int64 * _lib.N_LAYERS)()
        _lib.check(self.lib.pnp_profile_layers(self._h, lms, lcnt), "pnp_profile_layers")
        out = {name: {"ms": ms[i], "launches": int(cnt[i])} for i, name in enumerate(_lib.PROFILE_CLASS_NAMES)}
        out["layers"] = {"ms": list(lms), "launches": [int(v) for v in lcnt]}
        return out
```

Baseline: 132.1.

## Let Winograd F4 workgroups process runs of consecutive tiles per block

Restructures the F4 Winograd conv kernel so that one workgroup can loop over a run of consecutive tiles within its XCD slice instead of handling a single tile. Per-tile staging (buffer descriptors, offsets, halo loads) moves into lambdas that can be re-invoked, and the bias load is hoisted out of the epilogue. The aim is to amortise per-block setup and weight-fragment loads across several tiles with a smaller grid. The planner leaves run length at 1 unless PNP_WINO_F4_RUN=2 is set, because the default rule is hard-coded false. The restructured kernel body, which reads args through the kernarg pointer and adds an LDS exchange buffer, may still change register and LDS usage on the default path.

New measurement: 129.2. 2.2% lower.

```diff
diff --git a/dt4image_restoration_amd/_lib.py b/dt4image_restoration_amd/_lib.py
--- a/dt4image_restoration_amd/_lib.py
+++ b/dt4image_restoration_amd/_lib.py
@@ -159,6 +159,11 @@
 }
 
 
+SIGNATURES_PLAN = {
+    "pnp_conv_tile_runs": (C.c_int, [C.c_void_p, C.POINTER(C.c_int32)]),
+}
+
+
 def toeplitz_size_error(fn: str, h: int, w: int):
     if h <= PNP_TOEPLITZ_MAX_SIDE and w <= PNP_TOEPLITZ_MAX_SIDE:
         return None
@@ -183,6 +188,11 @@
         fn = getattr(lib, name)
         fn.restype = res
         fn.argtypes = args
+    for name, (res, args) in SIGNATURES_PLAN.items():
+        if hasattr(lib, name):
+            fn = getattr(lib, name)
+            fn.restype = res
+            fn.argtypes = args
     _lib = lib
     return lib
 
diff --git a/dt4image_restoration_amd/csrc/conv_kernels.hip b/dt4image_restoration_amd/csrc/conv_kernels.hip
--- a/dt4image_restoration_amd/csrc/conv_kernels.hip
+++ b/dt4image_restoration_amd/csrc/conv_kernels.hip
@@ -669,6 +669,8 @@
     t.no_f4_fused_first = getenv("PNP_NO_F4_FUSED_FIRST") != nullptr;
     if (const char* v = getenv("PNP_WINO_F4_MT16")) t.f4_mt16 = atoi(v);
     if (const char* v = getenv("PNP_WINO_F4_CS")) t.f4_cs = atoi(v);
+    if (const char* v = getenv("PNP_WINO_F4_RUN")) t.f4_run = atoi(v);
+    if (const char* v = getenv("PNP_WINO_F4_RUN_LEN")) t.f4_run_len = atoi(v);
     if (const char* v = getenv("PNP_WINO_F4_ORDER")) t.f4_order = atoi(v) != 0;
     t.bf16_f32_acts = getenv("PNP_BF16_F32_ACTS") != nullptr;
     t.bf16_no_ws = getenv("PNP_BF16_NO_WS") != nullptr;
diff --git a/dt4image_restoration_amd/csrc/pnp_capi.hip b/dt4image_restoration_amd/csrc/pnp_capi.hip
--- a/dt4image_restoration_amd/csrc/pnp_capi.hip
+++ b/dt4image_restoration_amd/csrc/pnp_capi.hip
@@ -3,6 +3,7 @@
 #include "../../include/pnpadmm_toeplitz.h"
 #include "../../include/pnpadmm_dcf.h"
 #include "../../include/pnpadmm_offres.h"
+#include "../../include/pnpadmm_plan.h"
 #include "pnp_internal.h"
 #include "denoiser_plan.h"
 #include "nufft_plan.h"
@@ -2692,6 +2693,21 @@
     PNP_API_END("pnp_conv_schedules")
 }
 
+int pnp_conv_tile_runs(pnp_handle e, int32_t* run28) {
+    PNP_API_BEGIN
+    if (!e || !run28) return fail(PNP_ERR_INVALID, "pnp_conv_tile_runs: null argument");
+    if (e->cfg.flags & PNP_FLAG_NO_DENOISER) return fail(PNP_ERR_STATE, "pnp_conv_tile_runs: handle has no denoiser");
+    for (int i = 0; i < N_LAYERS; ++i) {
+        const int at = e->dplan.launch_of[i];
+        run28[i] = 0;
+        if (at < 0 || e->dplan.family[i] != FAM_WINO4) continue;
+        const WinoPlan& w = e->dplan.launch[at].wino;
+        if (!w.cs && !w.phased) run28[i] = w.run > 1 ? w.run : 1;
+    }
+    return PNP_OK;
+    PNP_API_END("pnp_conv_tile_runs")
+}
+
 int pnp_profile_reset(pnp_handle e) {
     PNP_API_BEGIN
     if (!e) return fail(PNP_ERR_INVALID, "null handle");
diff --git a/dt4image_restoration_amd/csrc/pnp_internal.h b/dt4image_restoration_amd/csrc/pnp_internal.h
--- a/dt4image_restoration_amd/csrc/pnp_internal.h
+++ b/dt4image_restoration_amd/csrc/pnp_internal.h
@@ -24,6 +24,8 @@
     bool bf16_no_holdhi = false;
     bool bf16_w1 = false;
     int f4_cs = 1;
+    int f4_run = 1;
+    int f4_run_len = 0;
     int f4_order = 1;
     int slice128_min_n = 192;
     bool tv_naive = false;
@@ -66,6 +68,7 @@
     int bf16;
     int act16;
     int order;
+    int run;
 #ifdef PNP_STAMPS
     int stamp_slot;
 #endif
@@ -105,7 +108,21 @@
     int phased;
     int cs;
     int order;
-};
+    int run;
+};
+inline long winograd4_grid(int ntiles, int ny, int order, int run) {
+    const long tpx = (ntiles + 7) / 8;
+    return 8 * ny * (order == 1 && run > 1 ? (tpx + run - 1) / run : tpx);
+}
+__host__ __device__ inline void winograd4_run_decode(int bid, int ny, int ntiles, int run, int& cby, int& bt0, int& nrun) {
+    const int xcd = bid & 7, slot = bid >> 3;
+    const int tpx = (ntiles + 7) >> 3;
+    const int rb = slot / ny;
+    cby = slot - rb * ny;
+    const int lt0 = rb * run, lt1 = lt0 + run < tpx ? lt0 + run : tpx;
+    bt0 = xcd * tpx + lt0;
+    nrun = (xcd * tpx + lt1 < ntiles ? xcd * tpx + lt1 : ntiles) - bt0;
+}
 WinoPlan winograd_plan(int N, int H, int W, int Cin, int Cout, int src_mode, const Tuning& t, int Cskip = 0);
 bool upsample_lines_regular(int H);
 size_t winograd4_pack_floats(int cin, int cout);
diff --git a/dt4image_restoration_amd/csrc/winograd4_kernels.hip b/dt4image_restoration_amd/csrc/winograd4_kernels.hip
--- a/dt4image_restoration_amd/csrc/winograd4_kernels.hip
+++ b/dt4image_restoration_amd/csrc/winograd4_kernels.hip
@@ -121,6 +121,14 @@
     }
     return true;
 }
+
+__device__ __forceinline__ const ConvArgs* w4_args(const ConvArgs*) {
+    auto p = (const ConvArgs __attribute__((address_space(4)))*)__builtin_amdgcn_kernarg_segment_ptr();
+    asm volatile("" : "+s"(p));
+    return (const ConvArgs*)p;
+}
+__device__ __forceinline__ int w4_opaque(int v) { asm volatile("" : "+v"(v)); return v; }
+__device__ __forceinline__ int w4_opaque_s(int v) { asm volatile("" : "+s"(v)); return v; }
 
 __device__ __forceinline__ void wino4_decode(int bid, int ny, int ntiles, int order, int& cby, int& bt) {
     if (order == 0) {
@@ -218,11 +226,10 @@
 
 template <int TW, bool STK, int MT = 32, bool FUSE = false>
 __device__ __forceinline__ void wino4_epilogue(const ConvArgs& a, const f32x4 (&acc)[36], int n, int th, int tg, int cl, int cb,
-                                               int tx0, int ty0, bool live, float* xch = nullptr) {
+                                               int tx0, int ty0, bool live, float bias, float* xch = nullptr) {
     constexpr int TC = TW / 4, TR = MT / TC;
     constexpr unsigned OOB = 0x80000000u;
     const int cout0 = cb * 16 + cl;
-    const float bias = a.bias[cout0];
     const int Hp = a.H >> 1, Wp = a.W >> 1;
     auto at6 = [&](v2f m0, v2f m1, v2f m2, v2f m3, v2f m4, v2f m5, v2f* t) {
         const v2f s1 = m1 + m2, d1 = m1 - m2, s2 = m3 + m4, d2 = m3 - m4;
@@ -338,7 +345,7 @@
 }
 
 template <int TW, int SRC, bool STK = false, int WN = 2, int MT = 32>
-__global__ __launch_bounds__(8 * MT * WN, 2) void conv3x3_wino4_kernel(const ConvArgs a) {
+__global__ __launch_bounds__(8 * MT * WN, 2) void conv3x3_wino4_kernel(const ConvArgs a_) {
     constexpr int CK = 8 * WN, CKP = CK, LP = CK, PPP = CK / 4, NT_ = 8 * MT * WN;
     constexpr int CKQ = WN == 2 ? CK + 4 : CK + 2;
     constexpr int HCN = CK / 2;
@@ -377,82 +384,105 @@
     float* const mimg = dimg + (PH + 2) * IW;
     float* const wl = mimg + (PH + 2) * IW;
     float* const bl = wl + 18 * 32;
-#ifdef PNP_STAMPS
-    unsigned long long st_t0 = W4T(), st_setup = 0, st_loop0 = 0, st_commit = 0, st_trans = 0, st_mfma = 0, st_loop1 = 0, st_ew = 0, st_er = 0, st_tmp = 0;
-#endif
-    const int tid = threadIdx.x, lane = tid & 63;
+    constexpr bool FUSE = WN == 1 && MT == 32 && SRC == SRC_PLAIN;
+    float* const xch = V + 36 * PLANE;
+#ifdef PNP_STAMPS
+    unsigned long long st_t0 = W4T(), st_setup = 0, st_commit = 0, st_trans = 0, st_mfma = 0, st_loop = 0, st_epi = 0, st_tmp = 0, st_l0 = 0, st_sets = 0;
+#endif
+    const ConvArgs* pa = w4_args(&a_);
+    int tid = threadIdx.x, lane = tid & 63;
     const int wid = __builtin_amdgcn_readfirstlane(tid >> 6);
     const int cq = wid / (MT / 16), th = wid % (MT / 16);
-    const int tg = lane >> 4, cl = lane & 15;
-
-    const int ny = a.Cout / (32 * WN);
+    int tg = lane >> 4, cl = lane & 15;
+
+    const int ny = pa->Cout / (32 * WN);
     const int bid = blockIdx.x;
-    const int ntl = a.tilesX * a.tilesY * (STK ? (a.N + 1) / 2 : a.N);
-    int cby, bt;
-    wino4_decode(bid, ny, ntl, a.order, cby, bt);
-    if (bt >= ntl) return;
-    const int tx0 = (bt % a.tilesX) * TW;
-    bt /= a.tilesX;
-    const int ty0 = (bt % a.tilesY) * TH;
-    const int n = STK ? 2 * (bt / a.tilesY) : bt / a.tilesY;
-    const int nsl = STK ? (n + 1 < a.N ? 2 : 1) : 1;
-    const bool live0 = !(a.tact != nullptr && a.tact[n] > 0.5f);
-    const bool live1 = STK && nsl == 2 && !(a.tact != nullptr && a.tact[n + 1] > 0.5f);
-    if (!live0 && !live1) return;
+    const int tpi = pa->tilesX * pa->tilesY;
+    const int ntl = tpi * (STK ? (pa->N + 1) / 2 : pa->N);
+    int cby, bt0, nrun;
+    if (!STK && pa->order == 1 && pa->run > 1) {
+        winograd4_run_decode(bid, ny, ntl, pa->run, cby, bt0, nrun);
+    } else {
+        wino4_decode(bid, ny, ntl, pa->order, cby, bt0);
+        nrun = bt0 < ntl ? 1 : 0;
+    }
+    if (nrun <= 0) return;
+    unsigned long long lm0, lm1 = 0;
+    {
+        const int sl = STK ? 2 * ((bt0 + lane) / tpi) : (bt0 + lane) / tpi;
+        bool l0 = lane < nrun, l1 = STK && lane < nrun && sl + 1 < pa->N;
+        if (pa->tact != nullptr) {
+            if (l0) l0 = !(pa->tact[sl] > 0.5f);
+            if (l1) l1 = !(pa->tact[sl + 1] > 0.5f);
+        }
+        lm0 = __ballot(l0);
+        if constexpr (STK) lm1 = __ballot(l1);
+    }
+    unsigned long long todo = lm0 | lm1;
+    if (todo == 0) return;
     const int cb = cby * (2 * WN) + cq;
-    const int nchunks = a.Cin / CK;
-
-    const int Hs = a.H >> 1, Ws = a.W >> 1;
-    const int ylo = UP2 ? ty0 / 2 - 1 : 0;
-    const int xlo = UP2 ? (int)(a.rw * (float)(tx0 > 0 ? tx0 - 1 : 0)) : 0;
-    const int nskip = UP2 ? a.Cskip / CK : 0;
+    const int nchunks = pa->Cin / CK;
+    const float bias = pa->bias[cb * 16 + cl];
+
+    const int nskip = UP2 ? pa->Cskip / CK : 0;
 
     constexpr unsigned OOB = 0x80000000u;
-    const int cs = UP2 ? a.Cskip : a.Cin;
 #ifdef PNP_DIAG
-    const bool hot = (a.diag & 2) != 0;
+    const bool hot = (pa->diag & 2) != 0;
 #else
     constexpr bool hot = false;
 #endif
-    const int ly0 = hot ? 0 : ty0, lx0 = hot ? 0 : tx0, ln = hot ? 0 : n;
-    const __amdgpu_buffer_rsrc_t rsrc0 = __builtin_amdgcn_make_buffer_rsrc(
-        (void*)(a.src0 + (size_t)ln * a.H * a.W * cs), 0, nsl * a.H * a.W * cs * 4, 0x00020000);
+    int qtx0 = 0, qty0 = 0, qn = 0, qylo = 0, qxlo = 0;
+    bool qfi = false;
+    __amdgpu_buffer_rsrc_t rsrc0 = __builtin_amdgcn_make_buffer_rsrc((void*)pa->src0, 0, 0, 0x00020000);
+    __amdgpu_buffer_rsrc_t rsrc1 = rsrc0;
     unsigned voff[NIT];
-#pragma unroll
-    for (int k = 0; k < NIT; ++k) {
-        const int idx = tid + k * NT_;
-        const int part = idx % PPP, pp = idx / PPP;
-        const int py = pp / PW, px = pp % PW;
-        const int sub = STK ? py / SUBH : 0;
-        const int gy = STK ? py % SUBH - 1 : ly0 + py - 1, gx = lx0 + px - 1;
-        voff[k] = (idx < ITEMS && sub < nsl && gy >= 0 && gy < a.H && gx >= 0 && gx < a.W)
-                      ? (unsigned)((((sub * a.H + gy) * a.W + gx) * cs + part * 4) * 4) : OOB;
-    }
-    const int Cup = a.Cin - a.Cskip;
-    const __amdgpu_buffer_rsrc_t rsrc1 = __builtin_amdgcn_make_buffer_rsrc(
-        (void*)(UP2 ? a.src1 + (size_t)ln * Hs * Ws * Cup : a.src0), 0, UP2 ? Hs * Ws * Cup * 4 : 0, 0x00020000);
     unsigned voffL[UP2 ? NITL : 1];
-    if constexpr (UP2) {
-#pragma unroll
-        for (int k = 0; k < NITL; ++k) {
-            const int idx = tid + k * NT_;
+    auto stage_tile = [&](int bt, unsigned (&vo)[NIT], unsigned (&voL)[UP2 ? NITL : 1], bool lowres_too) {
+        const int t_ = w4_opaque((int)threadIdx.x);
+        const int Hs = pa->H >> 1, Ws = pa->W >> 1;
+        const int cs = UP2 ? pa->Cskip : pa->Cin, Cup = pa->Cin - pa->Cskip;
+        qtx0 = (bt % pa->tilesX) * TW;
+        bt /= pa->tilesX;
+        qty0 = (bt % pa->tilesY) * TH;
+        qn = STK ? 2 * (bt / pa->tilesY) : bt / pa->tilesY;
+        const int nsl = STK ? (qn + 1 < pa->N ? 2 : 1) : 1;
+        qylo = UP2 ? qty0 / 2 - 1 : 0;
+        qxlo = UP2 ? (int)(pa->rw * (float)(qtx0 > 0 ? qtx0 - 1 : 0)) : 0;
+        const int ly0 = hot ? 0 : qty0, lx0 = hot ? 0 : qtx0, ln = hot ? 0 : qn;
+        rsrc0 = __builtin_amdgcn_make_buffer_rsrc((void*)(pa->src0 + (size_t)ln * pa->H * pa->W * cs), 0, nsl * pa->H * pa->W * cs * 4, 0x00020000);
+#pragma unroll
+        for (int k = 0; k < NIT; ++k) {
+            const int idx = t_ + k * NT_;
             const int part = idx % PPP, pp = idx / PPP;
-            const int sy = (hot ? -1 : ylo) + pp / LW, sx = (hot ? 0 : xlo) + pp % LW;
-            voffL[k] = (idx < LITEMS && sy >= 0 && sy < Hs && sx < Ws) ? (unsigned)(((sy * Ws + sx) * Cup + part * 4) * 4) : OOB;
-        }
-    }
-    const int ldst = ((tid / PPP) * CKQ + (tid % PPP) * 4);
-    const int ldstL = ((tid / PPP) * LP + (tid % PPP) * 4);
+            const int py = pp / PW, px = pp % PW;
+            const int sub = STK ? py / SUBH : 0;
+            const int gy = STK ? py % SUBH - 1 : ly0 + py - 1, gx = lx0 + px - 1;
+            vo[k] = (idx < ITEMS && sub < nsl && gy >= 0 && gy < pa->H && gx >= 0 && gx < pa->W)
+                          ? (unsigned)((((sub * pa->H + gy) * pa->W + gx) * cs + part * 4) * 4) : OOB;
+        }
+        rsrc1 = __builtin_amdgcn_make_buffer_rsrc((void*)(UP2 ? pa->src1 + (size_t)ln * Hs * Ws * Cup : pa->src0), 0, UP2 ? Hs * Ws * Cup * 4 : 0, 0x00020000);
+        if (UP2 && lowres_too) {
+#pragma unroll
+            for (int k = 0; k < NITL; ++k) {
+                const int idx = t_ + k * NT_;
+                const int part = idx % PPP, pp = idx / PPP;
+                const int sy = (hot ? -1 : qylo) + pp / LW, sx = (hot ? 0 : qxlo) + pp % LW;
+                voL[k] = (idx < LITEMS && sy >= 0 && sy < Hs && sx < Ws) ? (unsigned)(((sy * Ws + sx) * Cup + part * 4) * 4) : OOB;
+            }
+        }
+        if constexpr (FIRST) qfi = qty0 >= 2 && qty0 + TH + 2 <= pa->H && qtx0 >= 2 && qtx0 + TW + 2 <= pa->W;
+    };
     auto put_patch = [&](int off, float4 v) {
         if constexpr (CKQ % 4 == 0) *reinterpret_cast<float4*>(&patch[off]) = v;
         else { *reinterpret_cast<float2*>(&patch[off]) = make_float2(v.x, v.y); *reinterpret_cast<float2*>(&patch[off + 2]) = make_float2(v.z, v.w); }
     };
 
     float4 raw[NRAW];
-    auto issue = [&](int c, int half = 0) {
+    auto issue_from = [&](int c, int half, const unsigned (&voff)[NIT], const unsigned (&voffL)[UP2 ? NITL : 1]) {
         if (UP2 && c >= nskip) {
             if (half != 0) return;
-            const int soff = (c * CK - a.Cskip) * 4;
+            const int soff = (c - nskip) * CK * 4;
 #pragma unroll
             for (int k = 0; k < NITL; ++k)
                 raw[k] = __builtin_bit_cast(float4, __builtin_amdgcn_raw_buffer_load_b128(rsrc1, voffL[k], soff, 0));
@@ -469,7 +499,12 @@
                 raw[k - NH0] = __builtin_bit_cast(float4, __builtin_amdgcn_raw_buffer_load_b128(rsrc0, voff[k], soff, 0));
         }
     };
+    auto issue = [&](int c, int half = 0) { issue_from(c, half, voff, voffL); };
+    unsigned vnext[NIT], vnextL[UP2 ? NITL : 1];
     auto park = [&](int c, int half = 0) {
+        const int tp = w4_opaque((int)threadIdx.x);
+        const int ldst = ((tp / PPP) * CKQ + (tp % PPP) * 4);
+        const int ldstL = ((tp / PPP) * LP + (tp % PPP) * 4);
         if (UP2 && c >= nskip) {
             if (half != 0) return;
 #pragma unroll
@@ -500,41 +535,63 @@
         wino4_interpolate<PH, PW, PPP, LH, LW, LP, NT_ / 64, PW * CKQ>(lowres, rowT, colT, wid, tid,
             [](int y, int x, int part) { return ((y * PW + x) * CKQ) + part * 4; }, [&](int off, float4 v) { put_patch(off, v); });
     };
+    constexpr int NHALO = (PH + 2) * (PW + 2);
+    constexpr int NF = FIRST ? (NHALO + NT_ - 1) / NT_ : 1;
     bool first_interior = false;
     int fbase[FIRST ? NIT : 1];
-    if constexpr (FIRST) {
-        first_interior = ty0 >= 2 && ty0 + TH + 2 <= a.H && tx0 >= 2 && tx0 + TW + 2 <= a.W;
-        const float sg = a.first_sigma[n];
-        for (int i = tid; i < (PH + 2) * (PW + 2); i += NT_) {
-            const int r = i / (PW + 2), q = i % (PW + 2);
-            const int gy = ty0 - 2 + r, gx = tx0 - 2 + q;
-            float d = 0.f, m = 0.f;
-            if (gy >= 0 && gy < a.H && gx >= 0 && gx < a.W) {
-                const size_t qx = ((size_t)n * a.H + gy) * a.W + gx;
-                d = a.last_ximg != nullptr ? a.last_ximg[qx] : (a.last_z[qx].x - a.last_u[qx].x);
-                m = 1.f;
-            }
-            dimg[r * IW + q] = d;
-            mimg[r * IW + q] = m;
-        }
-        for (int i = tid; i < 32 * 18; i += NT_) {
-            const int ch = i / 18, t = i % 18;
-            wl[t * 32 + ch] = a.first_w[i] * (t >= 9 ? sg : 1.f);
-        }
-        if (tid < 32) {
-            float sc = 0.f;
-#pragma unroll
-            for (int t = 9; t < 18; ++t) sc += a.first_w[tid * 18 + t] * sg;
-            bl[tid] = a.first_b[tid];
-            bl[32 + tid] = a.first_b[tid] + sc;
-        }
-#pragma unroll
-        for (int k = 0; k < NIT; ++k) {
-            const int pp = (tid + k * NT_) / PPP;
-            fbase[k] = (tid + k * NT_ < ITEMS) ? (pp / PW) * IW + pp % PW : 0;
-        }
-        __syncthreads();
-    }
+    float fz[NF], fu[NF];
+    auto halo_in = [&](int i) {
+        const int gy = qty0 - 2 + i / (PW + 2), gx = qtx0 - 2 + i % (PW + 2);
+        return i < NHALO && gy >= 0 && gy < pa->H && gx >= 0 && gx < pa->W;
+    };
+    auto halo_issue = [&]() {
+        if constexpr (FIRST) {
+            size_t qx[NF];
+#pragma unroll
+            for (int k = 0; k < NF; ++k) {
+                const int i = tid + k * NT_;
+                const int gy = qty0 - 2 + i / (PW + 2), gx = qtx0 - 2 + i % (PW + 2);
+                qx[k] = halo_in(i) ? ((size_t)qn * pa->H + gy) * pa->W + gx : 0;
+            }
+            if (pa->last_ximg != nullptr) {
+#pragma unroll
+                for (int k = 0; k < NF; ++k) { fz[k] = pa->last_ximg[qx[k]]; fu[k] = 0.f; }
+            } else {
+#pragma unroll
+                for (int k = 0; k < NF; ++k) { fz[k] = pa->last_z[qx[k]].x; fu[k] = pa->last_u[qx[k]].x; }
+            }
+        }
+    };
+    auto halo_park = [&]() {
+        if constexpr (FIRST) {
+#pragma unroll
+            for (int k = 0; k < NF; ++k) {
+                const int i = tid + k * NT_;
+                if (i < NHALO) {
+                    const bool in = halo_in(i);
+                    const float d = pa->last_ximg != nullptr ? fz[k] : (fz[k] - fu[k]);
+                    dimg[(i / (PW + 2)) * IW + i % (PW + 2)] = in ? d : 0.f;
+                    mimg[(i / (PW + 2)) * IW + i % (PW + 2)] = in ? 1.f : 0.f;
+                }
+            }
+        }
+    };
+    auto fill_wl = [&](int sl) {
+        if constexpr (FIRST) {
+            const float sg = pa->first_sigma[sl];
+            for (int i = tid; i < 32 * 18; i += NT_) {
+                const int ch = i / 18, t = i % 18;
+                wl[t * 32 + ch] = pa->first_w[i] * (t >= 9 ? sg : 1.f);
+            }
+            if (tid < 32) {
+                float sc = 0.f;
+#pragma unroll
+                for (int t = 9; t < 18; ++t) sc += pa->first_w[tid * 18 + t] * sg;
+                bl[tid] = pa->first_b[tid];
+                bl[32 + tid] = pa->first_b[tid] + sc;
+            }
+        }
+    };
     auto first_patch = [&](int c) {
         if constexpr (FIRST) {
             const int part = tid % PPP;
@@ -568,129 +625,215 @@
             }
         }
     };
-    if constexpr (UP2) {
-        wino4_upsample_tables<PH, PW, LP>(a, tid, ty0, tx0, ylo, xlo, rowT, colT);
-    }
-    if constexpr (FIRST) first_patch(0);
-    else {
-        issue(0); park(0);
-        if constexpr (SPLIT) { issue(0, 1); park(0, 1); }
-    }
+    auto tables = [&]() {
+        if constexpr (UP2) wino4_upsample_tables<PH, PW, LP>(*pa, w4_opaque((int)threadIdx.x), qty0, qtx0, qylo, qxlo, rowT, colT);
+    };
 
     auto swz = [](int t16, int g) { return WN == 2 ? (g ^ ((4 - (t16 >> 2)) & 3)) : (g ^ ((t16 >> 3) << 1)); };
-    const int hc = tid % HCN, tq = (tid / HCN) % MT;
     const int tj = wid / (NT_ / 128);
-    const int trow = tq / TC;
-    const int wrow = STK ? (trow / (TR / 2)) * SUBH + 4 * (trow % (TR / 2)) : 4 * trow;
-    const int win = (wrow * PW + 4 * (tq % TC)) * CKQ + 2 * hc;
-    const int vout = WN == 2 ? tq * CKP + 4 * swz(tq & 15, hc >> 1) + 2 * (hc & 1)
-                             : tq * CKP + 2 * swz(tq & 15, hc);
-
-    f32x4 acc[36];
-#pragma unroll
-    for (int k = 0; k < 36; ++k) acc[k] = f32x4{0.f, 0.f, 0.f, 0.f};
-
+    int win = 0, vout = 0, aoff = 0, boff = 0;
     typedef typename std::conditional<WN == 2, float4, float2>::type frag_t;
-    const size_t stream = (size_t)nchunks * 36 * 64 + kW4Tail / S;
+    auto wstream = [&]() {
+        const size_t stream = (size_t)nchunks * 36 * 64 + kW4Tail / S;
+        return reinterpret_cast<const frag_t*>(pa->wpack) + (size_t)cb * stream;
+    };
     const __amdgpu_buffer_rsrc_t rB = __builtin_amdgcn_make_buffer_rsrc(
-        (void*)(reinterpret_cast<const frag_t*>(a.wpack) + (size_t)cb * stream), 0, (int)(stream * sizeof(frag_t)), 0x00020000);
-    const int boff = lane * (int)sizeof(frag_t);
-    const frag_t* const bptr = reinterpret_cast<const frag_t*>(a.wpack) + (size_t)cb * stream + lane;
+        (void*)wstream(), 0, (int)(((size_t)nchunks * 36 * 64 + kW4Tail / S) * sizeof(frag_t)), 0x00020000);
+    const frag_t* bptr = nullptr;
+    auto derive = [&]() {
+        tid = w4_opaque((int)threadIdx.x);
+        lane = tid & 63;
+        tg = lane >> 4; cl = lane & 15;
+        const int hc = tid % HCN, tq = (tid / HCN) % MT;
+        const int trow = tq / TC;
+        const int wrow = STK ? (trow / (TR / 2)) * SUBH + 4 * (trow % (TR / 2)) : 4 * trow;
+        win = (wrow * PW + 4 * (tq % TC)) * CKQ + 2 * hc;
+        vout = WN == 2 ? tq * CKP + 4 * swz(tq & 15, hc >> 1) + 2 * (hc & 1)
+                       : tq * CKP + 2 * swz(tq & 15, hc);
+        boff = lane * (int)sizeof(frag_t);
+        bptr = wstream() + lane;
+        aoff = (16 * th + cl) * CKP + S * swz(cl, tg);
+        if constexpr (FIRST) {
+#pragma unroll
+            for (int k = 0; k < NIT; ++k) {
+                const int pp = (tid + k * NT_) / PPP;
+                fbase[k] = (tid + k * NT_ < ITEMS) ? (pp / PW) * IW + pp % PW : 0;
+            }
+        }
+    };
     auto bfrag = [&](const frag_t* bp, int f0, int i) -> frag_t {
         if constexpr (!UP2) return bp[i * 64];
         else if constexpr (WN == 2) return __builtin_bit_cast(frag_t, __builtin_amdgcn_raw_buffer_load_b128(rB, boff, (f0 + i) * (64 * 16), 0));
         else return __builtin_bit_cast(frag_t, __builtin_amdgcn_raw_buffer_load_b64(rB, boff, (f0 + i) * (64 * 8), 0));
     };
     frag_t bq[PF];
+
+    derive();
+    stage_tile(bt0 + __builtin_ctzll(todo), voff, voffL, true);
+    tables();
+    int n = qn;
+    if constexpr (FIRST) {
+        halo_issue();
+        fill_wl(qn);
+        halo_park();
+        first_interior = qfi;
+        __syncthreads();
+        first_patch(0);
+    } else {
+        issue(0); park(0);
+        if constexpr (SPLIT) { issue(0, 1); park(0, 1); }
+    }
 #pragma unroll
     for (int p = 0; p < KEEP; ++p) bq[p] = bfrag(bptr, 0, p);
-    const int aoff = (16 * th + cl) * CKP + S * swz(cl, tg);
 
 #ifdef PNP_STAMPS
     st_setup = W4T();
-    st_loop0 = st_setup;
-#endif
-    for (int c = 0; c < nchunks; ++c) {
+#endif
+    for (;;) {
+#ifdef PNP_STAMPS
+        st_l0 = W4T();
+        st_sets += 1;
+#endif
+        const unsigned long long rest = todo & (todo - 1);
+        const bool hasnext = !STK && rest != 0;
+        pa = w4_args(&a_);
+        f32x4 acc[36];
+#pragma unroll
+        for (int k = 0; k < 36; ++k) acc[k] = f32x4{0.f, 0.f, 0.f, 0.f};
+
+        for (int c = 0; c < nchunks; ++c) {
+            const bool lastc = c + 1 == nchunks;
+            const int cn = lastc ? 0 : c + 1;
+            const bool more = !lastc || hasnext;
+#ifdef PNP_STAMPS
+            st_tmp = W4T();
+#endif
+            __syncthreads();
+            if (UP2 && c >= nskip) {
+                if constexpr (NT_ == 256) __builtin_amdgcn_s_setprio(3);
+                interpolate();
+                if constexpr (NT_ == 256) __builtin_amdgcn_s_setprio(0);
+                __syncthreads();
+            }
+#ifdef PNP_STAMPS
+            { const unsigned long long t = W4T(); st_commit += t - st_tmp; st_tmp = t; }
+#endif
+
+            if constexpr (WN == 1 && !FIRST) {
+                if (lastc) {
+                    if (hasnext) { pa = w4_args(&a_); stage_tile(bt0 + __builtin_ctzll(rest), vnext, vnextL, nskip == 0); tables(); issue_from(0, 0, vnext, vnextL); }
+                } else issue(c + 1);
+            }
+            if constexpr (FIRST) { if (lastc && hasnext) { pa = w4_args(&a_); stage_tile(bt0 + __builtin_ctzll(rest), vnext, vnextL, false); halo_issue(); } }
+            __builtin_amdgcn_sched_barrier(0);
+            if constexpr (NT_ == 256) __builtin_amdgcn_s_setprio(3);
+            if (tj == 0) wino4_input_transform<0, PW, CKQ, PLANE>(patch + win, V + vout);
+            else wino4_input_transform<1, PW, CKQ, PLANE>(patch + win, V + vout);
+            if constexpr (NT_ == 256) __builtin_amdgcn_s_setprio(0);
+            __builtin_amdgcn_sched_barrier(0);
+            const frag_t* bp = bptr + (size_t)c * 36 * 64;
+            const int bf0 = c * 36;
+            if constexpr (WN == 2) {
+                if (lastc && hasnext) { pa = w4_args(&a_); stage_tile(bt0 + __builtin_ctzll(rest), vnext, vnextL, nskip == 0); tables(); }
+                __builtin_amdgcn_sched_barrier(0);
+            }
+#pragma unroll
+            for (int p = KEEP; p < PF; ++p) bq[p] = bfrag(bp, bf0, p);
+            if constexpr (WN == 2) {
+                if (!lastc) issue(c + 1);
+                else if (hasnext) issue_from(0, 0, vnext, vnextL);
+            }
+            __syncthreads();
+#ifdef PNP_STAMPS
+            { const unsigned long long t = W4T(); st_trans += t - st_tmp; st_tmp = t; }
+#endif
+
+            frag_t ar[3];
+            ar[0] = *reinterpret_cast<const frag_t*>(&V[aoff]);
+            ar[1] = *reinterpret_cast<const frag_t*>(&V[PLANE + aoff]);
+#pragma unroll
+            for (int xi = 0; xi < 36; ++xi) {
+                if (xi + 2 < 36) ar[(xi + 2) % 3] = *reinterpret_cast<const frag_t*>(&V[(xi + 2) * PLANE + aoff]);
+                __builtin_amdgcn_sched_barrier(0);
+                const frag_t a0 = ar[xi % 3], b0 = bq[xi % PF];
+                acc[xi] = __builtin_amdgcn_mfma_f32_16x16x4f32(a0.x, b0.x, acc[xi], 0, 0, 0);
+                acc[xi] = __builtin_amdgcn_mfma_f32_16x16x4f32(a0.y, b0.y, acc[xi], 0, 0, 0);
+                if constexpr (WN == 2) {
+                    acc[xi] = __builtin_amdgcn_mfma_f32_16x16x4f32(a0.z, b0.z, acc[xi], 0, 0, 0);
+                    acc[xi] = __builtin_amdgcn_mfma_f32_16x16x4f32(a0.w, b0.w, acc[xi], 0, 0, 0);
+                }
+                __builtin_amdgcn_sched_barrier(0);
+                if constexpr (SPLIT) {
+                    if (xi == 17 && more) {
+                        park(cn, 0);
+                        if (!lastc) issue(c + 1, 1);
+                        else issue_from(0, 1, vnext, vnextL);
+                    }
+                }
+#ifdef PNP_DIAG
+                if ((pa->diag & 4) && (xi & 1)) continue;
+#endif
+                if (xi + PF < 36 + KEEP) bq[xi % PF] = bfrag(bp, bf0, xi + PF);
+            }
+#ifdef PNP_STAMPS
+            { const unsigned long long t = W4T(); st_mfma += t - st_tmp; }
+#endif
+            if (more) {
+                if constexpr (FIRST) {
+                    if (!lastc) first_patch(c + 1);
+                    else { halo_park(); if (qn != n) fill_wl(qn); }
+                } else park(cn, SPLIT ? 1 : 0);
+            }
+        }
 #ifdef PNP_STAMPS
         st_tmp = W4T();
-#endif
-        __syncthreads();
-        if (UP2 && c >= nskip) {
-            if constexpr (NT_ == 256) __builtin_amdgcn_s_setprio(3);
-            interpolate();
-            if constexpr (NT_ == 256) __builtin_amdgcn_s_setprio(0);
+        st_loop += st_tmp - st_l0;
+#endif
+
+        pa = w4_args(&a_);
+        {
+            const int l = w4_opaque((int)threadIdx.x) & 63;
+            tg = l >> 4; cl = l & 15;
+        }
+        {
+            const int j = __builtin_ctzll(todo);
+            int bt = bt0 + j;
+            const int tx0 = (bt % pa->tilesX) * TW;
+            bt /= pa->tilesX;
+            const int ty0 = (bt % pa->tilesY) * TH;
+            const int ne = STK ? 2 * (bt / pa->tilesY) : bt / pa->tilesY;
+            wino4_epilogue<TW, STK, MT, FUSE>(*pa, acc, ne, th, tg, cl, cb, tx0, ty0, STK ? (((th == 0 ? lm0 : lm1) >> j) & 1) != 0 : true, bias, xch);
+        }
+#ifdef PNP_STAMPS
+        st_epi += W4T() - st_tmp;
+#endif
+        if (!hasnext) break;
+        todo = rest;
+        if constexpr (FIRST) n = qn;
+        pa = w4_args(&a_);
+        derive();
+        if constexpr (!FIRST) stage_tile(w4_opaque_s(bt0 + __builtin_ctzll(todo)), voff, voffL, true);
+#pragma unroll
+        for (int p = 0; p < KEEP; ++p) bq[p] = bfrag(bptr, 0, p);
+        if constexpr (FIRST) {
+            first_interior = qfi;
             __syncthreads();
-        }
-#ifdef PNP_STAMPS
-        { const unsigned long long t = W4T(); st_commit += t - st_tmp; st_tmp = t; }
-#endif
-
-        if constexpr (WN == 1 && !FIRST) { if (c + 1 < nchunks) issue(c + 1); }
-        __builtin_amdgcn_sched_barrier(0);
-        if constexpr (NT_ == 256) __builtin_amdgcn_s_setprio(3);
-        if (tj == 0) wino4_input_transform<0, PW, CKQ, PLANE>(patch + win, V + vout);
-        else wino4_input_transform<1, PW, CKQ, PLANE>(patch + win, V + vout);
-        if constexpr (NT_ == 256) __builtin_amdgcn_s_setprio(0);
-        __builtin_amdgcn_sched_barrier(0);
-        const frag_t* bp = bptr + (size_t)c * 36 * 64;
-        const int bf0 = c * 36;
-#pragma unroll
-        for (int p = KEEP; p < PF; ++p) bq[p] = bfrag(bp, bf0, p);
-        if constexpr (WN == 2) { if (c + 1 < nchunks) issue(c + 1); }
-        __syncthreads();
-#ifdef PNP_STAMPS
-        { const unsigned long long t = W4T(); st_trans += t - st_tmp; st_tmp = t; }
-#endif
-
-        frag_t ar[3];
-        ar[0] = *reinterpret_cast<const frag_t*>(&V[aoff]);
-        ar[1] = *reinterpret_cast<const frag_t*>(&V[PLANE + aoff]);
-#pragma unroll
-        for (int xi = 0; xi < 36; ++xi) {
-            if (xi + 2 < 36) ar[(xi + 2) % 3] = *reinterpret_cast<const frag_t*>(&V[(xi + 2) * PLANE + aoff]);
-            __builtin_amdgcn_sched_barrier(0);
-            const frag_t a0 = ar[xi % 3], b0 = bq[xi % PF];
-            acc[xi] = __builtin_amdgcn_mfma_f32_16x16x4f32(a0.x, b0.x, acc[xi], 0, 0, 0);
-            acc[xi] = __builtin_amdgcn_mfma_f32_16x16x4f32(a0.y, b0.y, acc[xi], 0, 0, 0);
-            if constexpr (WN == 2) {
-                acc[xi] = __builtin_amdgcn_mfma_f32_16x16x4f32(a0.z, b0.z, acc[xi], 0, 0, 0);
-                acc[xi] = __builtin_amdgcn_mfma_f32_16x16x4f32(a0.w, b0.w, acc[xi], 0, 0, 0);
-            }
-            __builtin_amdgcn_sched_barrier(0);
-            if constexpr (SPLIT) {
-                if (xi == 17 && c + 1 < nchunks) { park(c + 1, 0); issue(c + 1, 1); }
-            }
-#ifdef PNP_DIAG
-            if ((a.diag & 4) && (xi & 1)) continue;
-#endif
-            if (xi + PF < 36 + KEEP) bq[xi % PF] = bfrag(bp, bf0, xi + PF);
-        }
-#ifdef PNP_STAMPS
-        { const unsigned long long t = W4T(); st_mfma += t - st_tmp; }
-#endif
-        if (c + 1 < nchunks) {
-            if constexpr (FIRST) first_patch(c + 1);
-            else park(c + 1, SPLIT ? 1 : 0);
-        }
-    }
-#ifdef PNP_STAMPS
-    st_loop1 = W4T();
-    st_tmp = st_loop1;
-#endif
-
-    wino4_epilogue<TW, STK, MT, WN == 1 && MT == 32 && SRC == SRC_PLAIN>(a, acc, n, th, tg, cl, cb, tx0, ty0, STK ? (th == 0 ? live0 : live1) : true, smem);
+            first_patch(0);
+        }
+    }
 #ifdef PNP_STAMPS
     {
         const int w = (int)blockIdx.x - (int)(gridDim.x / 2);
-        if (tid == 0 && w >= 0 && w < W4_WGS && a.stamp_slot < W4_SLOTS) {
-            unsigned long long* o = g_w4_stamps + ((size_t)a.stamp_slot * W4_WGS + w) * W4_N;
+        if (tid == 0 && w >= 0 && w < W4_WGS && pa->stamp_slot < W4_SLOTS) {
+            unsigned long long* o = g_w4_stamps + ((size_t)pa->stamp_slot * W4_WGS + w) * W4_N;
             const unsigned long long te = W4T();
-            o[0] = 1; o[1] = st_setup - st_t0; o[2] = st_commit; o[3] = st_trans; o[4] = st_mfma; o[5] = st_loop1 - st_loop0;
-            o[6] = te - st_tmp; o[7] = 0; o[8] = te - st_loop1; o[9] = te - st_t0; o[10] = (unsigned long long)nchunks;
-        }
-    }
-#endif
-}
+            o[0] = 1; o[1] = st_setup - st_t0; o[2] = st_commit; o[3] = st_trans; o[4] = st_mfma; o[5] = st_loop;
+            o[6] = st_epi; o[7] = 0; o[8] = st_epi; o[9] = te - st_t0; o[10] = (unsigned long long)nchunks; o[11] = st_sets;
+        }
+    }
+#endif
+}
+
 
 template <int TW, bool STK>
 __global__ __launch_bounds__(512, 2) void conv3x3_wino4p_kernel(const ConvArgs a) {
@@ -853,7 +996,7 @@
     st_tmp = st_loop1;
 #endif
 
-    wino4_epilogue<TW, STK>(a, acc, n, th, tg, cl, cb, tx0, ty0, STK ? (th == 0 ? live0 : live1) : true);
+    wino4_epilogue<TW, STK>(a, acc, n, th, tg, cl, cb, tx0, ty0, STK ? (th == 0 ? live0 : live1) : true, a.bias[cb * 16 + cl]);
 #ifdef PNP_STAMPS
     {
         const int w = (int)blockIdx.x - (int)(gridDim.x / 2);
@@ -1088,7 +1231,7 @@
     st_tmp = st_loop1;
 #endif
 
-    wino4_epilogue<TW, false, 16>(a, acc, n, 0, tg, cl, cb, tx0, ty0, true);
+    wino4_epilogue<TW, false, 16>(a, acc, n, 0, tg, cl, cb, tx0, ty0, true, a.bias[cb * 16 + cl]);
 #ifdef PNP_STAMPS
     {
         const int w = (int)blockIdx.x - (int)(gridDim.x / 2);
@@ -1141,14 +1284,15 @@
     constexpr size_t patch_f = (((size_t)(STK ? TH + 4 : TH + 2) * (TW + 2) * CKQ + 3) / 4) * 4;
     constexpr size_t lowres_f = SRC == SRC_UPCAT ? (size_t)(TH / 2 + 3) * (TW / 2 + 3) * CK + 4 * (TH + 2 + TW + 2) : 0;
     constexpr size_t first_f = SRC == SRC_FIRST ? (size_t)2 * (TH + 4) * (TW + 5) + 18 * 32 + 64 : 0;
-    constexpr size_t lds = (patch_f + (size_t)36 * MT * CKP + lowres_f + first_f) * sizeof(float);
+    constexpr size_t xch_f = (WN == 1 && MT == 32 && SRC == SRC_PLAIN) ? 512 : 0;
+    constexpr size_t lds = (patch_f + (size_t)36 * MT * CKP + lowres_f + first_f + xch_f) * sizeof(float);
     static_assert(lds <= (WN == 2 && MT == 32 ? 160 : 80) * 1024, "one (8 waves) / two (4 waves) workgroups per CU");
-    if (p.th != TH || p.tw != TW) return hipErrorInvalidValue;
+    if (p.th != TH || p.tw != TW || a.run < 1 || a.run > 64) return hipErrorInvalidValue;
     auto kern = conv3x3_wino4_kernel<TW, SRC, STK, WN, MT>;
     static DeviceOnce cap;
     if (hipError_t e = raise_lds_cap((const void*)kern, (int)lds, cap); e != hipSuccess) return e;
     const int ntiles = p.tiles_x * p.tiles_y * (STK ? (a.N + 1) / 2 : a.N), ny = a.Cout / (32 * WN);
-    dim3 grid((unsigned)(((ntiles + 7) / 8) * 8 * ny));
+    dim3 grid((unsigned)winograd4_grid(ntiles, ny, a.order, a.run));
     hipLaunchKernelGGL(kern, grid, dim3(8 * MT * WN), lds, s, a);
     return hipGetLastError();
 }
@@ -1160,6 +1304,7 @@
     a.tilesX = p.tiles_x;
     a.tilesY = p.tiles_y;
     a.order = p.order;
+    a.run = (p.order == 1 && p.run > 1 && !p.cs && !(p.phased && src_mode == SRC_PLAIN && p.bn == 64 && p.mt == 32)) ? p.run : 1;
 #ifdef PNP_STAMPS
     a.stamp_slot = g_w4_slot++;
 #endif
diff --git a/dt4image_restoration_amd/csrc/winograd_kernels.hip b/dt4image_restoration_amd/csrc/winograd_kernels.hip
--- a/dt4image_restoration_amd/csrc/winograd_kernels.hip
+++ b/dt4image_restoration_amd/csrc/winograd_kernels.hip
@@ -90,7 +90,21 @@
                 f.stack = 0;
                 f.phased = 0;
             }
-            const long blocks = (long)f.tiles_x * f.tiles_y * (f.stack ? (N + 1) / 2 : N) * (Cout / f.bn);
+            const long ntl = (long)f.tiles_x * f.tiles_y * (f.stack ? (N + 1) / 2 : N);
+            const long blocks = ntl * (Cout / f.bn);
+            f.run = 1;
+            if (!f.cs && !f.phased && f.order == 1 && t.f4_run != 0 && ntl < (1L << 30)) {
+                constexpr long kRunRounds = 4;
+                const int ny = Cout / f.bn;
+                const long tpx = (ntl + 7) / 8;
+                const long slots = (f.bn == 32 || f.mt == 16) ? 512 : 256;
+                long run = t.f4_run_len > 0 ? t.f4_run_len : winograd4_grid((int)ntl, ny, 1, 1) / (slots * kRunRounds);
+                run = run < 1 ? 1 : (run > 64 ? 64 : run);
+                if (run > tpx) run = tpx;
+                while (run > 1 && winograd4_grid((int)ntl, ny, 1, (int)run) < t.wino_min_blocks) --run;
+                const bool run_rule = false;
+                if (t.f4_run == 2 || (t.f4_run == 1 && run_rule)) f.run = (int)run;
+            }
             f.use = blocks >= t.wino_min_blocks;
             if (f.use) return f;
         }
diff --git a/dt4image_restoration_amd/engine.py b/dt4image_restoration_amd/engine.py
--- a/dt4image_restoration_amd/engine.py
+++ b/dt4image_restoration_amd/engine.py
@@ -921,6 +921,13 @@
         _lib.check(self.lib.pnp_conv_schedules(self._h, out), "pnp_conv_schedules")
         return list(out)
 
+    def conv_tile_runs(self):
+        if not hasattr(self.lib, "pnp_conv_tile_runs"):
+            raise _lib.PnPError("pnp_conv_tile_runs: not in this library build")
+        out = (C.c_int32 * _lib.N_LAYERS)()
+        _lib.check(self.lib.pnp_conv_tile_runs(self._h, out), "pnp_conv_tile_runs")
+        return list(out)
+
     def bf16_weight_terms(self) -> int:
         return int(self.lib.pnp_bf16_weight_terms(self._h))
 
diff --git a/include/pnpadmm_plan.h b/include/pnpadmm_plan.h
--- /dev/null
+++ b/include/pnpadmm_plan.h
@@ -0,0 +1,16 @@
+#ifndef PNPADMM_PLAN_H
+#define PNPADMM_PLAN_H
+
+#include "pnpadmm.h"
+
+#ifdef __cplusplus
+extern "C" {
+#endif
+
+int pnp_conv_tile_runs(pnp_handle h, int32_t* run28);
+
+#ifdef __cplusplus
+}
+#endif
+
+#endif
```
